# CaptainEven/DenseBox

Measured on AMD Instinct MI355X. Metric: training patches/sec (240x240), higher is better.
Workload: dtype f16; 1 GPU; full training step (fwd + fused dense loss w/ hard-negative mining + bwd + grad all-reduce + SGD) of DenseBoxLMLOC on 240x240 patches; net=DenseBoxLMLOC, batch_per_gpu=64, global_batch=64, patch=240x240, parallelism=dp1, half_neg=11, grad_finite=True

## Files before the change

densebox_amd/_lib.py:

```python
import ctypes as C
import os

_HERE = os.path.dirname(os.path.abspath(__file__))
LIB_PATH = os.environ.get('DBX_LIB') or os.path.join(_HERE, 'csrc', 'libdensebox_hip.so')

F16, BF16, F32 = 0, 1, 2
DTYPE_ID = {'f16': F16, 'bf16': BF16, 'f32': F32}
ESIZE = {F16: 2, BF16: 2, F32: 4}

EPI_BIAS, EPI_RELU, EPI_GATE, EPI_DROPMASK, EPI_ACCUM, EPI_F32_NCHW, EPI_DROPHASH = 1, 2, 4, 8, 16, 32, 64
CONV_WFRAG = 128
K_IGEMM, K_DMA, K_BAND, K_C64, K_C8, K_WS, K_P8 = 1, 2, 3, 4, 5, 6, 7


class View(C.Structure):
    _fields_ = [('ptr', C.c_void_p), ('n', C.c_int32), ('h', C.c_int32), ('w', C.c_int32),
                ('pad', C.c_int32), ('ld', C.c_int32), ('c_off', C.c_int32), ('c', C.c_int32)]


class ConvDesc(C.Structure):
    _fields_ = [('dtype', C.c_int32), ('kh', C.c_int32), ('kw', C.c_int32), ('cpad', C.c_int32),
                ('cin_pad', C.c_int32), ('cout_pad', C.c_int32), ('epilogue', C.c_int32), ('drop_seed', C.c_uint32)]


class ConvPlan(C.Structure):
    _fields_ = [('kernel', C.c_int32), ('tile_m', C.c_int32), ('tile_n', C.c_int32), ('w_frag', C.c_int32),
                ('name', C.c_char * 64)]


class LossDesc(C.Structure):
    _fields_ = [('kind', C.c_int32), ('n', C.c_int32), ('half_neg', C.c_int32),
                ('lambda_loc', C.c_float), ('lambda_det', C.c_float), ('lambda_lm', C.c_float),
                ('use_labels', C.c_int32)]


class LossIO(C.Structure):
    _fields_ = [(k, C.c_void_p) for k in (
        'bbox', 'vertices', 'labels', 'rand_neg', 'lm_rand_neg',
        'score', 'loc', 'lm', 'rf', 'lmloc',
        'd_score', 'd_loc', 'd_lm', 'd_rf', 'd_lmloc',
        'loss', 'mask_cls', 'mask_lm', 'neg_idx', 'lm_neg_idx', 'pos_count')]


class WarpJob(C.Structure):
    _fields_ = [('src', C.c_void_p), ('sh', C.c_int32), ('sw', C.c_int32), ('m9', C.c_double * 9), ('dh', C.c_int32),
                ('dw', C.c_int32), ('x0', C.c_int32), ('y0', C.c_int32), ('oh', C.c_int32), ('ow', C.c_int32),
                ('dst_off', C.c_int64)]


class CropFrame(C.Structure):
    _fields_ = [('src', C.c_void_p), ('sh', C.c_int32), ('sw', C.c_int32)]


class EvalRecord(C.Structure):
    _fields_ = [('score', C.c_double), ('lm_err', C.c_double), ('status', C.c_int32), ('frame', C.c_int32)]


class Track(C.Structure):
    _fields_ = [('box', C.c_double * 4), ('vel', C.c_double * 4), ('score', C.c_double), ('best_score', C.c_double), ('id', C.c_int32),
                ('hits', C.c_int32), ('age', C.c_int32), ('first_frame', C.c_int32), ('last_frame', C.c_int32), ('best_frame', C.c_int32)]


class TrackRecord(C.Structure):
    _fields_ = [('stream', C.c_int32), ('reserved', C.c_int32), ('t', Track)]


class Shot(C.Structure):
    _fields_ = [('key', C.c_double), ('score', C.c_double), ('sharpness', C.c_int64), ('id', C.c_int32), ('frame', C.c_int32),
                ('shots', C.c_int32), ('reserved', C.c_int32)]


class ShotRecord(C.Structure):
    _fields_ = [('stream', C.c_int32), ('slot', C.c_int32), ('shot', Shot)]


class ResizeJob(C.Structure):
    _fields_ = [('src', C.c_void_p), ('sh', C.c_int32), ('sw', C.c_int32), ('cx0', C.c_int32), ('cy0', C.c_int32),
                ('cw', C.c_int32), ('ch', C.c_int32), ('pad_l', C.c_int32), ('pad_t', C.c_int32), ('pad_r', C.c_int32),
                ('pad_b', C.c_int32), ('pad_value', C.c_int32), ('dh', C.c_int32), ('dw', C.c_int32), ('dst_off', C.c_int64)]


class MergeXform(C.Structure):
    _fields_ = [('scale', C.c_double), ('off_x', C.c_double), ('off_y', C.c_double)]


_VP, _I32, _I64, _F, _D = C.c_void_p, C.c_int32, C.c_int64, C.c_float, C.c_double
_PV, _PC = C.POINTER(View), C.POINTER(ConvDesc)

SIGNATURES = {
    'dbx_last_error': (C.c_char_p, []),
    'dbx_version': (C.c_int, []),
    'dbx_device_arch': (C.c_int, [C.c_int]),
    'dbx_conv_packed_elems': (_I64, [_PC]),
    'dbx_conv_forward': (C.c_int, [_PC, _PV, _VP, _VP, _PV, _PV, _VP, _I32, _VP]),
    'dbx_conv_plan': (C.c_int, [_PC, _PV, _PV, C.POINTER(ConvPlan)]),
    'dbx_conv_forward_split': (C.c_int, [_PC, _PV, _VP, _VP, _PV, _PV, _PV, _PV, _I32, _I32, _VP]),
    'dbx_heads_forward_fusable': (C.c_int, [_PC, _PV, _PV, C.POINTER(C.c_int32), _I32]),
    'dbx_heads_forward_fused_scratch_bytes': (_I64, [_I32, _I64]),
    'dbx_heads_forward_fused': (C.c_int, [_PC, _PV, _VP, _VP, _PV, _VP, _VP, C.POINTER(C.c_int32), _I32, _VP, _VP, _VP]),
    'dbx_heads_forward_fused_heads': (C.c_int, [_PC, _PV, _VP, _VP, _PV, _VP, _VP, C.POINTER(C.c_int32), _I32, C.POINTER(C.c_void_p), _VP, _VP]),
    'dbx_dp_unique_id': (C.c_int, [_VP]),
    'dbx_dp_init': (C.c_int, [_VP, _I32, _I32, C.POINTER(C.c_void_p)]),
    'dbx_dp_allreduce_sum_f32': (C.c_int, [_VP, _VP, _I64, _VP]),
    'dbx_dp_destroy': (C.c_int, [_VP]),
    'dbx_conv_dgrad_wgrad1_scratch_bytes': (_I64, []),
    'dbx_conv_dgrad_wgrad1_fusable': (C.c_int, [_PC, _PV, _PV, _PV]),
    'dbx_conv_dgrad_wgrad1': (C.c_int, [_PC, _PV, _VP, _PV, _PV, _I32, _VP, _VP, _VP, _I32, _VP]),
    'dbx_conv_pool_fusable': (C.c_int, [_PC, _PV, _PV]),
    'dbx_conv_forward_pool': (C.c_int, [_PC, _PV, _VP, _VP, _PV, _PV, _I32, _VP]),
    'dbx_conv_forward_pool_idx': (C.c_int, [_PC, _PV, _VP, _VP, _PV, _PV, _I32, _VP, _VP]),
    'dbx_pack_weight': (C.c_int, [_I32, _I32, _VP, _I32, _I32, _I32, _I32, _VP, _I32, _I32, _I32, _I32, _VP]),
    'dbx_fold_heads': (C.c_int, [_VP, _VP, _VP, _VP, _I32, _VP, _VP, _VP]),
    'dbx_fold_refine': (C.c_int, [_VP, _VP, _VP, _VP, _VP, _VP, _I32, _I32, _VP, _VP, _VP, _VP]),
    'dbx_refine_eval': (C.c_int, [_VP, _VP, _I32, _I32, _I32, _VP, _VP, _VP, _VP]),
    'dbx_refine_backward_scratch_bytes': (C.c_int64, [_I32, _I32, _I32]),
    'dbx_refine_backward': (C.c_int, [_VP, _VP, _VP, _I32, _I32, _I32, _VP, _VP, _VP, _VP, _VP, _VP, _I32, _VP, _VP, _VP, _VP, _VP, _VP, _VP, _VP, _VP, _VP, _VP, _VP, _VP, _VP]),
    'dbx_upsample_bilinear_nchw_f32': (C.c_int, [_VP, _I32, _I32, _I32, _VP, _I32, _I32, _VP]),
    'dbx_pack_multi': (C.c_int, [_I32, _VP, _I32, _I64, _VP]),
    'dbx_sgd_pack_step': (C.c_int, [_I32, _VP, _I32, _I64, _VP, _F, _F, _F, _I32, _VP]),
    'dbx_head2_dgrad': (C.c_int, [_I32, _PV, C.POINTER(C.c_void_p), C.POINTER(C.c_int32), _I32, _PV, _VP, _I32, _I32, C.c_uint32, _VP]),
    'dbx_head2_wgrad_scratch_bytes': (_I64, [_I32, _I32]),
    'dbx_head2_wgrad': (C.c_int, [_I32, _PV, _PV, C.POINTER(C.c_int32), _I32, C.POINTER(C.c_void_p), C.POINTER(C.c_void_p), _VP, _VP]),
    'dbx_head2_backward': (C.c_int, [_I32, _PV, _PV, C.POINTER(C.c_void_p), C.POINTER(C.c_int32), _I32, _PV, _VP, _I32, _I32, C.c_uint32,
                                     C.POINTER(C.c_void_p), C.POINTER(C.c_void_p), _VP, _VP]),
    'dbx_head2_backward_up': (C.c_int, [_I32, _PV, _PV, C.POINTER(C.c_void_p), C.POINTER(C.c_int32), _I32, _PV, _VP, _I32, _I32, C.c_uint32,
                                        C.POINTER(C.c_void_p), C.POINTER(C.c_void_p), _VP, _PV, _VP]),
    'dbx_perspective_matrix': (C.c_int, [_VP, _VP, _VP]),
    'dbx_warp_perspective_u8': (C.c_int, [_VP, _I32, _I32, _I32, _VP, _VP, _I32, _I32, _VP]),
    'dbx_warp_batch_workspace_bytes': (_I64, [_I32]),
    'dbx_warp_perspective_batch_u8': (C.c_int, [C.POINTER(WarpJob), _I32, _I32, _VP, _VP, _VP]),
    'dbx_plate_crops_batch': (C.c_int, [_VP, _I32, _I32, _VP, _I64, _I64, _VP, _I32, _I32, _I32, _VP, _VP, _VP, _VP]),
    'dbx_match_gt_batch': (C.c_int, [_VP, _I32, _I64, _VP, _VP, _I32, _I32, _VP, _I32, _VP, _VP, _I32, _D, _VP, _VP, _VP, _VP, _VP, _VP]),
    'dbx_eval_append': (C.c_int, [_VP, _I32, _I64, _VP, _VP, _I32, _I32, _VP, _VP, _VP, _VP, _I64, _VP, _VP]),
    'dbx_track_update_batch': (C.c_int, [_VP, _I32, _I64, _VP, _VP, _I32, _I32, _VP, _VP, _I32, _I32, _I32, _D, _I32, _D, _D, _D, _VP, _VP, _VP,
                                         _VP, _VP, _VP]),
    'dbx_track_append': (C.c_int, [_VP, _VP, _I32, _I32, _I32, _VP, _I64, _VP, _VP]),
    'dbx_crop_sharpness': (C.c_int, [_VP, _I64, _I32, _I32, _I32, _VP, _VP]),
    'dbx_track_gallery_update': (C.c_int, [_VP, _VP, _VP, _VP, _VP, _VP, _VP, _VP, _VP, _VP, _VP, _VP, _VP, _I32, _I32, _I32, _I32, _I32, _I32,
                                           _I32, _I32, _I64, _I32, _D, _I32, _VP]),
    'dbx_resize_batch_workspace_bytes': (_I64, [_I32]),
    'dbx_resize_cubic_batch_u8': (C.c_int, [C.POINTER(ResizeJob), _I32, _I32, _VP, _VP, _VP]),
    'dbx_conv_wgrad_scratch_bytes': (_I64, [_I32, _PV, _PV, _I32, _I32]),
    'dbx_conv_wgrad': (C.c_int, [_I32, _PV, _PV, _I32, _I32, _I32, _I32, _I32, _VP, _VP, _VP, _I32, _VP]),
    'dbx_conv_wgrad_slice': (C.c_int, [_I32, _PV, _PV, _I32, _I32, _I32, _I32, _I32, _VP, _I32, _I32, _VP, _VP, _I32, _VP]),
    'dbx_conv_wgrad_pool_dz_ok': (C.c_int, [_I32, _PV, _PV, _I32, _I32]),
    'dbx_conv_wgrad_pool_dz': (C.c_int, [_I32, _PV, _VP, _I32, _PV, _PV, _I32, _I32, _I32, _I32, _I32, _VP, _VP, _VP, _I32, _I32, _VP]),
    'dbx_head2_backward_up_fused': (C.c_int, [_I32, _PV, _PV]),
    'dbx_heads1_wgrad_gen_ok': (C.c_int, [_I32, _PV, _I32]),
    'dbx_heads1_dgrad_gen': (C.c_int, [_I32, _PV, C.POINTER(C.c_void_p), C.POINTER(C.c_int32), _I32, _I32, C.c_uint32, _VP, _PV, _PV, _VP]),
    'dbx_heads1_wgrad_gen': (C.c_int, [_I32, _PV, _PV, C.POINTER(C.c_void_p), C.POINTER(C.c_int32), _I32, _I32, C.c_uint32, _I32, _VP, _I32, _I32,
                             _VP, _VP, _VP]),
    'dbx_conv_wgrad_plan': (C.c_int, [_I32, _PV, _PV, _I32, _I32, C.c_char_p, _I32, C.POINTER(C.c_int32)]),
    'dbx_nchw_to_framed': (C.c_int, [_I32, _VP, _I32, _PV, _VP]),
    'dbx_u8hwc_to_framed': (C.c_int, [_I32, _VP, _PV, C.POINTER(C.c_float), C.POINTER(C.c_float), _VP]),
    'dbx_nchw_to_framed_ch': (C.c_int, [_I32, _VP, _I32, _PV, _I32, _VP]),
    'dbx_nchw_to_framed_slots': (C.c_int, [_I32, _VP, _VP, _I32, _I32, _PV, _VP]),
    'dbx_framed_to_nchw_f32': (C.c_int, [_I32, _PV, _VP, _VP]),
    'dbx_framed_add_ch': (C.c_int, [_I32, _PV, _I32, _I32, _PV, _I32, _VP]),
    'dbx_maxpool2x2': (C.c_int, [_I32, _PV, _PV, _VP]),
    'dbx_maxpool2x2_bwd': (C.c_int, [_I32, _PV, _PV, _PV, _I32, _I32, _VP]),
    'dbx_maxpool_idx_bytes': (C.c_int64, [_I32, _I32, _I32, _I32]),
    'dbx_maxpool2x2_idx': (C.c_int, [_I32, _PV, _PV, _VP, _VP]),
    'dbx_maxpool2x2_bwd_idx': (C.c_int, [_I32, _VP, _PV, _PV, _I32, _I32, _VP]),
    'dbx_upsample_bilinear': (C.c_int, [_I32, _PV, _PV, _VP]),
    'dbx_upsample_bilinear_bwd': (C.c_int, [_I32, _PV, _PV, _PV, _VP]),
    'dbx_loss_scratch_bytes': (C.c_int64, [_I32]),
    'dbx_loss_forward_backward': (C.c_int, [C.POINTER(LossDesc), C.POINTER(LossIO), _VP, _VP]),
    'dbx_count_positives': (C.c_int, [_VP, _VP, _I32, _VP, _VP]),
    'dbx_init_score_map': (C.c_int, [_VP, _VP, _I32, _VP, _VP]),
    'dbx_init_offset_map': (C.c_int, [_VP, _VP, _I32, _I32, _VP, _VP]),
    'dbx_init_lm_heatmap': (C.c_int, [_VP, _VP, _I32, _I32, _VP, _VP]),
    'dbx_mask_by_sel': (C.c_int, [_VP, _I32, _VP, _I64, _VP, _I32, _VP]),
    'dbx_mask_gray_zone_cls': (C.c_int, [_VP, _VP, _VP, _I32, _VP]),
    'dbx_mask_gray_zone_lm': (C.c_int, [_VP, _I32, _VP, _I64, _VP]),
    'dbx_sgd_step': (C.c_int, [_VP, _VP, _I32, _I64, _F, _F, _F, _I32, _VP]),
    'dbx_grad_guard': (C.c_int, [_VP, _I64, _VP, _I32, _VP]),
    'dbx_sgd_step_guarded': (C.c_int, [_VP, _VP, _I32, _I64, _F, _F, _F, _I32, _VP, _I32, _VP]),
    'dbx_sgd_pack_step_guarded': (C.c_int, [_I32, _VP, _I32, _I64, _VP, _F, _F, _F, _I32, _VP, _I32, _VP]),
    'dbx_detect_scratch_bytes': (_I64, [_I32, _I32, _I32]),
    'dbx_detect': (C.c_int, [_VP, _VP, _VP, _VP, _I32, _I32, _I32, _D, _VP, _I32, _VP, _VP, _VP, _VP]),
    'dbx_detect_batch_scratch_bytes': (_I64, [_I32, _I32, _I32, _I32]),
    'dbx_detect_batch': (C.c_int, [_VP, _VP, _VP, _VP, _I32, _I32, _I32, _I32, _D, _VP, _I32, _VP, _VP, _VP, _VP]),
    'dbx_nms': (C.c_int, [_VP, _I32, _I32, _D, _VP, _VP, _VP]),
    'dbx_detect_thresh_batch_scratch_bytes': (_I64, [_I32, _I32, _I32, _I32]),
    'dbx_detect_thresh_batch': (C.c_int, [_VP, _VP, _VP, _VP, _I32, _I32, _I32, _F, _I32, _D, _VP, _I32, _VP, _VP, _VP, _VP, _VP]),
    'dbx_thresh_rows_batch_scratch_bytes': (_I64, [_I32, _I32, _I32, _I32]),
    'dbx_thresh_rows_batch': (C.c_int, [_VP, _VP, _VP, _VP, _I32, _I32, _I32, _F, _I32, _VP, _I32, _VP, _VP, _VP, _VP]),
    'dbx_nms_large_scratch_bytes': (_I64, [_I32]),
    'dbx_nms_large': (C.c_int, [_VP, _I32, _I32, _D, _VP, _VP, _VP]),
    'dbx_merge_nms_batch_workspace_bytes': (_I64, [_I32, _I32, _I32]),
    'dbx_merge_nms_batch': (C.c_int, [C.POINTER(C.c_void_p), C.POINTER(MergeXform), _I32, _I32, _I32, _I32, _D, _VP, _VP, _VP, _VP]),
    'dbx_merge_nms_thresh_batch_workspace_bytes': (_I64, [_I32, _I32, _I32]),
    'dbx_merge_nms_thresh_batch': (C.c_int, [C.POINTER(C.c_void_p), C.POINTER(C.c_void_p), C.POINTER(MergeXform), _I32, _I32, _I32, _I32, _D,
                                             _VP, _VP, _VP, _VP, _VP]),
}

ABI_VERSION = 13
_lib = None
MISSING = []


def lib():
    global _lib
    if _lib is None:
        if not os.path.exists(LIB_PATH):
            raise RuntimeError('libdensebox_hip.so is not built (%s). Run `python -c "import __graft_entry__ as g; '
                               'g.build()"`; densebox_amd has no fallback path.' % LIB_PATH)
        L = C.CDLL(LIB_PATH)
        for name, (res, args) in SIGNATURES.items():
            try:
                fn = getattr(L, name)
            except AttributeError:
                MISSING.append(name)
                continue
            fn.restype = res
            fn.argtypes = args
        if 'dbx_version' not in MISSING and L.dbx_version() != ABI_VERSION:
            raise RuntimeError('libdensebox_hip.so at %s has ABI version %d, this binding needs %d (struct layouts / scratch '
                               'contracts differ): rebuild it' % (LIB_PATH, L.dbx_version(), ABI_VERSION))
        _lib = L
    return _lib


def check(rc):
    if rc != 0:
        raise RuntimeError('libdensebox_hip: %s (status %d)' % (lib().dbx_last_error().decode(), rc))


def ptr(t):
    return C.c_void_p(t.data_ptr()) if t is not None else None


def stream_ptr():
    import torch
    return C.c_void_p(torch.cuda.current_stream().cuda_stream)
```

densebox_amd/csrc/aux_ops.hip:

```cpp
#include "common.hpp"
#include <mutex>

static thread_local char g_err[512] = "";
void dbx_set_error(const char* fmt, ...) {
    va_list ap;
    va_start(ap, fmt);
    vsnprintf(g_err, sizeof(g_err), fmt, ap);
    va_end(ap);
}
extern "C" const char* dbx_last_error(void) { return g_err; }
extern "C" int dbx_version(void) { return DBX_ABI_VERSION; }
extern "C" int dbx_device_arch(int device) {
    hipDeviceProp_t p;
    if (hipGetDeviceProperties(&p, device) != hipSuccess) { dbx_set_error("hipGetDeviceProperties failed"); return DBX_ERR_HIP; }
    int arch = 0;
    const char* s = p.gcnArchName;
    if (s[0] == 'g' && s[1] == 'f' && s[2] == 'x') arch = (int)strtol(s + 3, nullptr, 16) == 0x950 ? 950 : (int)strtol(s + 3, nullptr, 10);
    return arch;
}

template <typename T> struct Vec { static constexpr int N = 16 / sizeof(T); };

template <typename T> __device__ __forceinline__ void load_vec(const T* p, float (&v)[16 / sizeof(T)]) {
    const u32x4 raw = *(const u32x4*)p;
    const T* e = (const T*)&raw;
#pragma unroll
    for (int i = 0; i < 16 / (int)sizeof(T); ++i) v[i] = to_f32(e[i]);
}
template <typename T> __device__ __forceinline__ void store_vec(T* p, const float (&v)[16 / sizeof(T)]) {
    u32x4 raw;
    T* e = (T*)&raw;
#pragma unroll
    for (int i = 0; i < 16 / (int)sizeof(T); ++i) e[i] = from_f32<T>(v[i]);
    *(u32x4*)p = raw;
}

static inline int grid_for(int64_t work, int block = 256) {
    int64_t b = (work + block - 1) / block;
    return (int)(b < 1 ? 1 : (b > 8192 ? 8192 : b));
}

#define VIEW_VEC_CHECK(T, v, name)                                                                             \
    DBX_REQUIRE(((size_t)(v)->ptr % 16) == 0 && ((v)->ld * sizeof(T)) % 16 == 0 && ((v)->c_off * sizeof(T)) % 16 == 0 && \
                    ((v)->c * sizeof(T)) % 16 == 0, name ": view must be 16-byte aligned/strided")

template <typename T>
__global__ void nchw_to_framed_kernel(const float* __restrict__ x, int csrc, FrameGeo y) {
    constexpr int V = Vec<T>::N;
    const int cg = y.c / V;
    const int64_t total = (int64_t)y.n * y.h * y.w * cg;
    for (int64_t i = blockIdx.x * (int64_t)blockDim.x + threadIdx.x; i < total; i += (int64_t)gridDim.x * blockDim.x) {
        const int px = (int)(i % y.w);
        const int g = (int)((i / y.w) % cg);
        const int py = (int)((i / ((int64_t)y.w * cg)) % y.h);
        const int n = (int)(i / ((int64_t)y.w * cg * y.h));
        float v[V];
#pragma unroll
        for (int j = 0; j < V; ++j) {
            const int c = g * V + j;
            v[j] = c < csrc ? x[(((int64_t)n * csrc + c) * y.h + py) * y.w + px] : 0.f;
        }
        store_vec<T>((T*)y.base + geo_pix(y, n, py, px) + g * V, v);
    }
}
template <typename T> static int nchw_to_framed_t(const float* x, int csrc, const dbx_view* y, hipStream_t s) {
    VIEW_VEC_CHECK(T, y, "nchw_to_framed");
    FrameGeo g = make_geo<T>(y);
    const int64_t total = (int64_t)y->n * y->h * y->w * (y->c / Vec<T>::N);
    hipLaunchKernelGGL(nchw_to_framed_kernel<T>, dim3(grid_for(total)), dim3(256), 0, s, x, csrc, g);
    DBX_LAUNCH_CHECK();
    return DBX_OK;
}
extern "C" int dbx_nchw_to_framed(int32_t dtype, const float* x_nchw, int32_t c_src, const dbx_view* y, void* stream) {
    DBX_DISPATCH_DTYPE(dtype, nchw_to_framed_t, x_nchw, c_src, y, (hipStream_t)stream);
}

struct SlotSrc { const float* x[4]; int k[4]; };
template <typename T>
__global__ void nchw_to_framed_slots_kernel(SlotSrc src, int nslots, int slot, FrameGeo y) {
    constexpr int V = Vec<T>::N;
    const int gps = slot / V, cg = nslots * gps;
    const int64_t total = (int64_t)y.n * y.h * y.w * cg;
    for (int64_t i = blockIdx.x * (int64_t)blockDim.x + threadIdx.x; i < total; i += (int64_t)gridDim.x * blockDim.x) {
        const int px = (int)(i % y.w);
        const int g = (int)((i / y.w) % cg);
        const int py = (int)((i / ((int64_t)y.w * cg)) % y.h);
        const int n = (int)(i / ((int64_t)y.w * cg * y.h));
        const int si = g / gps, c0 = (g % gps) * V;
        const float* x = si == 0 ? src.x[0] : si == 1 ? src.x[1] : si == 2 ? src.x[2] : src.x[3];
        const int k = si == 0 ? src.k[0] : si == 1 ? src.k[1] : si == 2 ? src.k[2] : src.k[3];
        float v[V];
#pragma unroll
        for (int j = 0; j < V; ++j) {
            const int c = c0 + j;
            v[j] = (x && c < k) ? x[(((int64_t)n * k + c) * y.h + py) * y.w + px] : 0.f;
        }
        store_vec<T>((T*)y.base + geo_pix(y, n, py, px) + si * slot + c0, v);
    }
}
template <typename T> static int nchw_to_framed_slots_t(const float* const* xs, const int32_t* ks, int nslots, int slot, const dbx_view* y, hipStream_t s) {
    VIEW_VEC_CHECK(T, y, "nchw_to_framed_slots");
    DBX_REQUIRE(nslots >= 1 && nslots <= 4 && slot % Vec<T>::N == 0 && y->c == nslots * slot, "nchw_to_framed_slots: 1..4 slots of a multiple of the vector width, view of nslots * slot channels");
    SlotSrc src;
    for (int i = 0; i < 4; ++i) {
        src.x[i] = i < nslots ? xs[i] : nullptr; src.k[i] = i < nslots ? ks[i] : 0;
        if (i < nslots) DBX_REQUIRE(ks[i] >= 0 && ks[i] <= slot, "nchw_to_framed_slots: k must fit its slot");
    }
    FrameGeo g = make_geo<T>(y);
    const int64_t total = (int64_t)y->n * y->h * y->w * (y->c / Vec<T>::N);
    hipLaunchKernelGGL(nchw_to_framed_slots_kernel<T>, dim3(grid_for(total)), dim3(256), 0, s, src, nslots, slot, g);
    DBX_LAUNCH_CHECK();
    return DBX_OK;
}
extern "C" int dbx_nchw_to_framed_slots(int32_t dtype, const float* const* x_nchw, const int32_t* k, int32_t nslots, int32_t slot, const dbx_view* y,
                                        void* stream) {
    if (!x_nchw || !k || !y) { dbx_set_error("nchw_to_framed_slots: null argument"); return DBX_ERR_ARG; }
    DBX_DISPATCH_DTYPE(dtype, nchw_to_framed_slots_t, x_nchw, k, nslots, slot, y, (hipStream_t)stream);
}

template <typename T>
__global__ void framed_to_nchw_kernel(FrameGeo x, float* __restrict__ y) {
    const int64_t total = (int64_t)x.n * x.c * x.h * x.w;
    for (int64_t i = blockIdx.x * (int64_t)blockDim.x + threadIdx.x; i < total; i += (int64_t)gridDim.x * blockDim.x) {
        const int px = (int)(i % x.w);
        const int py = (int)((i / x.w) % x.h);
        const int c = (int)((i / ((int64_t)x.w * x.h)) % x.c);
        const int n = (int)(i / ((int64_t)x.w * x.h * x.c));
        y[i] = to_f32(((const T*)x.base)[geo_pix(x, n, py, px) + c]);
    }
}
template <typename T> static int framed_to_nchw_t(const dbx_view* x, float* y, hipStream_t s) {
    FrameGeo g = make_geo<T>(x);
    const int64_t total = (int64_t)x->n * x->c * x->h * x->w;
    hipLaunchKernelGGL(framed_to_nchw_kernel<T>, dim3(grid_for(total)), dim3(256), 0, s, g, y);
    DBX_LAUNCH_CHECK();
    return DBX_OK;
}
extern "C" int dbx_framed_to_nchw_f32(int32_t dtype, const dbx_view* x, float* y_nchw, void* stream) {
    DBX_DISPATCH_DTYPE(dtype, framed_to_nchw_t, x, y_nchw, (hipStream_t)stream);
}

template <typename T> struct IdxWord { typedef unsigned int type; };
template <> struct IdxWord<float> { typedef unsigned short type; };
template <typename T>
__global__ void maxpool_kernel(FrameGeo x, FrameGeo y, unsigned char* __restrict__ idx) {
    constexpr int V = Vec<T>::N;
    const int cg = y.c / V;
    const int64_t total = (int64_t)y.n * y.h * y.w * cg;
    for (int64_t i = blockIdx.x * (int64_t)blockDim.x + threadIdx.x; i < total; i += (int64_t)gridDim.x * blockDim.x) {
        const int g = (int)(i % cg);
        const int px = (int)((i / cg) % y.w);
        const int py = (int)((i / ((int64_t)cg * y.w)) % y.h);
        const int n = (int)(i / ((int64_t)cg * y.w * y.h));
// ... 1049 lines not shown
#pragma unroll
        for (int d = 0; d < D; ++d) {
            const int r = r0 + d;
            float gj[KJ], h[V];
            {
                const T* ge = (const T*)&graw[d];
                const T* he = (const T*)&hraw[d];
#pragma unroll
                for (int j = 0; j < KJ; ++j) gj[j] = to_f32(ge[j]);
#pragma unroll
                for (int i = 0; i < V; ++i) h[i] = to_f32(he[i]);
            }
            fetch(d);
            if (r < R) {
                int y0, y1; float ly0, ly1;
                bilin_coef(oy, sy, dg.h, y0, y1, ly0, ly1);
                while (y0 > cur) {
                    finalize(cur, va);
#pragma unroll
                    for (int i = 0; i < V / 2; ++i) { va[i] = vb[i]; vb[i] = (f32x2){0.f, 0.f}; }
                    ++cur;
                }
                const float wa = (y0 == cur ? ly0 : 0.f) + (y1 == cur ? ly1 : 0.f);
                const float wb = (y0 == cur + 1 ? ly0 : 0.f) + (y1 == cur + 1 ? ly1 : 0.f);
                {
                    f32x2 o2[V / 2];
#pragma unroll
                    for (int i = 0; i < V / 2; ++i) o2[i] = (f32x2){0.f, 0.f};
#pragma unroll
                    for (int j = 0; j < KJ; ++j) {
                        bs[j] += gj[j];
                        const f32x2 g2 = {gj[j], gj[j]};
#pragma unroll
                        for (int i = 0; i < V / 2; ++i) acc[j][i] = g2 * (f32x2){h[2 * i], h[2 * i + 1]} + acc[j][i];
#pragma unroll
                        for (int i = 0; i < V / 2; ++i) o2[i] = g2 * w2[j][i] + o2[i];
                    }
                    float o[V];
#pragma unroll
                    for (int i = 0; i < V / 2; ++i) { o[2 * i] = o2[i].x; o[2 * i + 1] = o2[i].y; }
                    const long long pc0 = ((long long)n * H + oy) * W;
                    if (mask) {
                        unsigned char mb[V];
                        *(u32x2*)mb = *(const u32x2*)(mask + (size_t)pc0 * mask_ld + lo_mask);
#pragma unroll
                        for (int i = 0; i < V; ++i) o[i] = mb[i] ? o[i] : 0.f;
                    } else if (use_hash) {
                        const unsigned kb8 = dbx_drop_hash32(drop_seed, (unsigned)pc0 + (unsigned)px, (unsigned)(hd * 512 + c0) >> 5) >> ((unsigned)c0 & 31u);
#pragma unroll
                        for (int i = 0; i < V; ++i)
                            o[i] = __builtin_bit_cast(float, __builtin_bit_cast(int, o[i]) & ((int)(kb8 << (31 - i)) >> 31));
                    }
                    u32x4 raw;
                    T* oe = (T*)&raw;
#pragma unroll
                    for (int i = 0; i < V; ++i) oe[i] = from_f32<T>(o[i]);
                    if (owner && !nostore) *(u32x4*)((T*)dhid.base + row_of(dhid, n, oy) + lo_dhid) = raw;
                    const f32x2 wa2 = {wa, wa}, wb2 = {wb, wb};
#pragma unroll
                    for (int i = 0; i < V / 2; ++i) {
                        const f32x2 dv = {to_f32(oe[2 * i]), to_f32(oe[2 * i + 1])};
                        va[i] = wa2 * dv + va[i]; vb[i] = wb2 * dv + vb[i];
                    }
                }
                if (++oy == H) {
                    finalize(cur, va);
                    if (cur + 1 < dg.h) finalize(cur + 1, vb);
                    if (pend) flush();
#pragma unroll
                    for (int i = 0; i < V / 2; ++i) va[i] = vb[i] = (f32x2){0.f, 0.f};
                    cur = 0; oy = 0; n += G;
                }
            }
        }
    }
    if (!owner) {
#pragma unroll
        for (int j = 0; j < KJ; ++j) {
            bs[j] = 0.f;
#pragma unroll
            for (int i = 0; i < V / 2; ++i) acc[j][i] = (f32x2){0.f, 0.f};
        }
    }
    const int lane = threadIdx.x & 63, wv = threadIdx.x >> 6;
#pragma unroll
    for (int j = 0; j < KJ; ++j) {
#pragma unroll
        for (int i = 0; i < V; ++i) {
            float a = acc[j][i >> 1][i & 1];
            a += __shfl_xor(a, 8); a += __shfl_xor(a, 16); a += __shfl_xor(a, 32);
            acc[j][i >> 1][i & 1] = a;
        }
        float bsum = bs[j];
        bsum += __shfl_xor(bsum, 8); bsum += __shfl_xor(bsum, 16); bsum += __shfl_xor(bsum, 32);
        bs[j] = bsum;
    }
    __syncthreads();
    float* red = s_v;
    if (lane < LPP) {
#pragma unroll
        for (int j = 0; j < KJ; ++j) {
            *(f32x4*)&red[(wv * 8 + j) * CS + lane * V] = (f32x4){acc[j][0][0], acc[j][0][1], acc[j][1][0], acc[j][1][1]};
            *(f32x4*)&red[(wv * 8 + j) * CS + lane * V + 4] = (f32x4){acc[j][2][0], acc[j][2][1], acc[j][3][0], acc[j][3][1]};
        }
#pragma unroll
        for (int j = KJ; j < 8; ++j) {
            *(f32x4*)&red[(wv * 8 + j) * CS + lane * V] = (f32x4){0.f, 0.f, 0.f, 0.f};
            *(f32x4*)&red[(wv * 8 + j) * CS + lane * V + 4] = (f32x4){0.f, 0.f, 0.f, 0.f};
        }
        if (lane == 0) {
#pragma unroll
            for (int j = 0; j < 8; ++j) red[4 * 8 * CS + wv * 8 + j] = j < KJ ? bs[j < KJ ? j : 0] : 0.f;
        }
    }
    __syncthreads();
    {
        const size_t blk = (size_t)grp * plan.halves + half;
        const int c = threadIdx.x % CS;
#pragma unroll
        for (int jj = 0; jj < 2; ++jj) {
            const int j = threadIdx.x / CS + 4 * jj;
            float o = 0.f;
#pragma unroll
            for (int q = 0; q < 4; ++q) o += red[(q * 8 + j) * CS + c];
            partial[(blk * nhl * 8 + (hd - hd0) * 8 + j) * 512 + cbase + c] = o;
        }
        if (cbase == 0 && threadIdx.x < 8) {
            float bsum = 0.f;
#pragma unroll
            for (int q = 0; q < 4; ++q) bsum += red[4 * 8 * CS + q * 8 + threadIdx.x];
            bpartial[blk * 32 + (hd - hd0) * 8 + threadIdx.x] = bsum;
        }
    }
}
static bool h2u_plan(int W, int ws, float sx, H2UPlan& p) {
    if (W > 64 || ws > 32 || W < 1 || ws < 1) return false;
    int x0[64];
    for (int ox = 0; ox < W; ++ox) { int v = (int)(sx * (float)ox); x0[ox] = v > ws - 1 ? ws - 1 : v; }
    if (W <= 32 && ws <= 16) { p.halves = 1; p.h[0] = p.h[1] = H2UHalf{0, W, 0, W, 0, ws}; return true; }
    const int S = ws / 2;
    if (S < 1 || S > 16 || ws - S > 16) return false;
    int hiL = -1, loR = W;
    for (int ox = 0; ox < W; ++ox) { if (x0[ox] <= S - 1) hiL = ox; if (x0[ox] >= S - 1 && ox < loR) loR = ox; }
    if (hiL + 1 > 32 || W - loR > 32 || loR > hiL + 1) return false;
    const int P = (loR + hiL + 1) / 2;
    p.halves = 2;
    p.h[0] = H2UHalf{0, hiL + 1, 0, P, 0, S};
    p.h[1] = H2UHalf{loR, W - loR, P, W, S, ws - S};
    return true;
}
template <typename T>
static int head2_backward_up_t(const dbx_view* dout, const dbx_view* hid, const float* const* w2, const int32_t* k, int nh, const dbx_view* dhid,
                               const uint8_t* mask, int mask_ld, int use_hash, unsigned drop_seed, float* const* dw, float* const* db,
                               void* scratch, const dbx_view* dg, hipStream_t s) {
    VIEW_VEC_CHECK(T, dg, "head2_backward_up d_g44");
    DBX_REQUIRE(dg->n == hid->n && dg->c == hid->c, "head2_backward_up: d_g44 has the hidden map's batch and channels");
    const float sy = ac_scale(dg->h, hid->h), sx = ac_scale(dg->w, hid->w);
    H2UPlan plan;
    bool fused = sizeof(T) == 2 && sy > 0.f && sy < 1.f && sx > 0.45f && sx < 1.f && hid->c % 64 == 0 && hid->h >= 2 && h2u_plan(hid->w, dg->w, sx, plan);
    if (const char* e = getenv("DBX_HEAD2_UP")) fused = fused && atoi(e) != 0;
    const bool nostore = dhid->ptr == nullptr;
    DBX_REQUIRE(!nostore || (fused && !mask), "head2_backward_up without d_hid: needs the one-pass kernel (dbx_head2_backward_up_fused) and hash / no dropout");
    if (!fused) {
        const int rc = head2_wgrad_t<T>(dout, hid, k, nh, dw, db, scratch, s, w2, dhid, mask, mask_ld, use_hash, drop_seed);
        return rc != DBX_OK ? rc : upsample_bwd_t<T>(dhid, dg, nullptr, s);
    }
    if constexpr (sizeof(T) == 2) {
        VIEW_VEC_CHECK(T, hid, "head2_backward_up hid");
        if (!nostore) VIEW_VEC_CHECK(T, dhid, "head2_backward_up d_hid");
        DBX_REQUIRE(nh >= 1 && nh <= 4 && hid->c == 512 * nh && dout->c % nh == 0 && dout->c / nh >= 8, "head2_backward_up: nh in 1..4, hid of 512*nh channels, d_out of nh slots >= 8 channels");
        DBX_REQUIRE(dout->n == hid->n && dout->h == hid->h && dout->w == hid->w && dhid->n == hid->n && dhid->h == hid->h && dhid->w == hid->w && dhid->c == hid->c,
                    "head2_backward_up: shape mismatch");
        DBX_REQUIRE(((size_t)dout->ptr % 16) == 0 && (dout->ld * sizeof(T)) % 16 == 0 && (dout->c_off * sizeof(T)) % 16 == 0 &&
                        ((dout->c / nh) * sizeof(T)) % 16 == 0, "head2_backward_up: d_out alignment");
        Head2Out o;
        Head2Args ha;
        ha.nh = nh; ha.slot = dout->c / nh;
        for (int i = 0; i < 4; ++i) {
            o.dw[i] = i < nh ? dw[i] : nullptr; o.db[i] = (i < nh && db) ? db[i] : nullptr; o.k[i] = i < nh ? k[i] : 0;
            ha.w2[i] = i < nh ? w2[i] : nullptr; ha.k[i] = i < nh ? k[i] : 0;
            if (i < nh) DBX_REQUIRE(k[i] >= 1 && k[i] <= 8 && dw[i] && w2[i] && ((size_t)w2[i] % 16) == 0, "head2_backward_up: k in 1..8, 16-byte aligned weights");
        }
        constexpr size_t smem = (size_t)2 * H2U_NB * 32 * 64 * 4;
        static_assert(smem >= (4 * 8 * 64 + 32) * 4 && 2 * smem + 4096 <= 160 * 1024, "LDS budget of two workgroups per CU");
        static DbxDevOnce attr_once; int attr_dev = 0;
        if (attr_once.pending(&attr_dev)) {
            DBX_HIP(hipFuncSetAttribute((const void*)head2_backward_up_kernel<T, 1>, hipFuncAttributeMaxDynamicSharedMemorySize, (int)smem));
            DBX_HIP(hipFuncSetAttribute((const void*)head2_backward_up_kernel<T, 2>, hipFuncAttributeMaxDynamicSharedMemorySize, (int)smem));
            DBX_HIP(hipFuncSetAttribute((const void*)head2_backward_up_kernel<T, 4>, hipFuncAttributeMaxDynamicSharedMemorySize, (int)smem));
            DBX_HIP(hipFuncSetAttribute((const void*)head2_backward_up_kernel<T, 8>, hipFuncAttributeMaxDynamicSharedMemorySize, (int)smem));
            attr_once.mark(attr_dev);
        }
        static int split = -1;
        if (split < 0) { const char* e = getenv("DBX_HEAD2_UP_SPLIT"); split = e ? atoi(e) : 1; }
        auto kup = [&](int kk) { return !split ? 8 : kk <= 1 ? 1 : kk <= 2 ? 2 : kk <= 4 ? 4 : 8; };
        float* const pbase = (float*)scratch;
        long long pused = 0;
        int blocks_max = 0;
        for (int h0 = 0; h0 < nh;) {
            int h1 = h0 + 1;
            while (h1 < nh && kup(k[h1]) == kup(k[h0])) ++h1;
            const int nhl = h1 - h0, nsl = nhl * 8, kj = kup(k[h0]);
            int groups = H2U_WGS / (nsl * plan.halves);
            groups = groups < 1 ? 1 : groups > hid->n ? hid->n : groups;
            const int blocks = groups * plan.halves;
            float* partial = pbase + pused;
            float* bpartial = partial + (size_t)blocks * nhl * 8 * 512;
            for (int i = h0; i < h1; ++i) { o.poff[i] = pused; o.boff[i] = pused + (long long)blocks * nhl * 8 * 512; o.nblk[i] = blocks; o.nhl[i] = nhl; o.hl[i] = i - h0; }
            pused += (long long)blocks * (nhl * 8 * 512 + 32);
            blocks_max = blocks > blocks_max ? blocks : blocks_max;
#define H2U_LAUNCH(KJ)                                                                                                              \
            hipLaunchKernelGGL((head2_backward_up_kernel<T, KJ>), dim3(blocks * nsl), dim3(256), smem, s, make_geo<T>(dout), make_geo<T>(hid),    \
                               make_geo<T>(nostore ? hid : dhid), make_geo<T>(dg), h0, nhl, dout->c / nh, ha, partial, bpartial, mask, mask_ld,    \
                               use_hash, drop_seed, sy, sx, plan, nostore ? 1 : 0)
            if (kj == 1) H2U_LAUNCH(1); else if (kj == 2) H2U_LAUNCH(2); else if (kj == 4) H2U_LAUNCH(4); else H2U_LAUNCH(8);
#undef H2U_LAUNCH
            DBX_LAUNCH_CHECK();
            h0 = h1;
        }
        for (int i = nh; i < 4; ++i) { o.poff[i] = 0; o.boff[i] = 0; o.nblk[i] = 0; o.nhl[i] = 1; o.hl[i] = 0; }
        float* partial = pbase; float* bpartial = pbase;
        const int blocks = blocks_max;
        const int total = nh * 8 * 512 + nh * 8;
        hipLaunchKernelGGL(head2_wgrad_reduce_kernel, dim3((total + 63) / 64), dim3(1024), 0, s, partial, bpartial, blocks, nh, o);
        DBX_LAUNCH_CHECK();
    }
    return DBX_OK;
}
template <typename T> static int head2_up_fused_t(const dbx_view* hid, const dbx_view* dg) {
    const float sy = ac_scale(dg->h, hid->h), sx = ac_scale(dg->w, hid->w);
    H2UPlan plan;
    bool fused = sizeof(T) == 2 && sy > 0.f && sy < 1.f && sx > 0.45f && sx < 1.f && hid->c % 64 == 0 && hid->h >= 2 && h2u_plan(hid->w, dg->w, sx, plan);
    if (const char* e = getenv("DBX_HEAD2_UP")) fused = fused && atoi(e) != 0;
    return fused ? 1 : 0;
}
extern "C" int dbx_head2_backward_up_fused(int32_t dtype, const dbx_view* hid, const dbx_view* d_g44) {
    if (!hid || !d_g44) return 0;
    switch (dtype) { case DBX_F16: return head2_up_fused_t<_Float16>(hid, d_g44); case DBX_BF16: return head2_up_fused_t<__bf16>(hid, d_g44); default: return 0; }
}
extern "C" int dbx_head2_backward_up(int32_t dtype, const dbx_view* d_out, const dbx_view* hid, const float* const* w2, const int32_t* k,
                                     int32_t nh, const dbx_view* d_hid, const uint8_t* dropmask, int32_t dropmask_ld, int32_t use_hash,
                                     uint32_t drop_seed, float* const* dw, float* const* db, void* scratch, const dbx_view* d_g44, void* stream) {
    if (!d_out || !hid || !w2 || !k || !d_hid || !dw || !scratch || !d_g44) { dbx_set_error("head2_backward_up: null argument"); return DBX_ERR_ARG; }
    DBX_DISPATCH_DTYPE(dtype, head2_backward_up_t, d_out, hid, w2, k, nh, d_hid, dropmask, dropmask_ld, use_hash, (unsigned)drop_seed, dw, db,
                       scratch, d_g44, (hipStream_t)stream);
}

struct PackJob { const float* src; void* dst; int co, ci, taps, mode; long long ktot; int cin_pad, row_off, k_off, rows_lim; };
template <typename T>
__global__ void pack_multi_kernel(const PackJob* __restrict__ jobs) {
    const PackJob j = jobs[blockIdx.y];
    const int total = j.co * j.ci * j.taps, taps = j.taps, ci = j.ci;
    T* wp = (T*)j.dst;
    const bool fwd = j.mode == 0 || j.mode == 4;
    const int rl = j.mode >= 4 ? (int)j.ktot : j.rows_lim;
    if (sizeof(T) == 2 && j.mode != 2 && (fwd ? ci : j.co) % 8 == 0 && (j.k_off & 7) == 0 && (j.cin_pad & 7) == 0 && taps <= 25) {
        __shared__ float tile[8][32 * 25];
        const int ot = (j.co + 7) / 8, ctn = (ci + 31) / 32, ntiles = ot * ctn, row_f = 32 * taps;
        for (int tl = blockIdx.x; tl < ntiles; tl += gridDim.x) {
            const int o0 = (tl / ctn) * 8, c0 = (tl % ctn) * 32;
            const int cw = min(32, ci - c0), ow = min(8, j.co - o0);
            __syncthreads();
            for (int e = threadIdx.x; e < 8 * row_f; e += blockDim.x) {
                const int r = e / row_f, f = e - r * row_f;
                tile[r][f] = (r < ow && f < cw * taps) ? j.src[((o0 + r) * ci + c0) * taps + f] : 0.f;
            }
            __syncthreads();
            const int nch = fwd ? 8 * taps * 4 : 32 * taps;
            for (int q = threadIdx.x; q < nch; q += blockDim.x) {
                int row, col, tap;
                float v[8];
                if (fwd) {
                    const int k8 = q & 3, t = (q >> 2) % taps, r = (q >> 2) / taps;
                    if (r >= ow || 8 * k8 >= cw) continue;
                    row = j.row_off + o0 + r; col = j.k_off + c0 + 8 * k8; tap = t;
#pragma unroll
                    for (int e = 0; e < 8; ++e) v[e] = tile[r][(8 * k8 + e) * taps + t];
                } else {
                    const int c = q % 32, t = q / 32;
                    if (c >= cw) continue;
                    row = j.row_off + c0 + c; col = j.k_off + o0; tap = taps - 1 - t;
#pragma unroll
                    for (int e = 0; e < 8; ++e) v[e] = tile[e][c * taps + t];
                }
                if (row < 0 || col < 0 || col + 8 > j.cin_pad || (rl > 0 && row >= rl)) continue;
                u32x4 raw;
                T* e8 = (T*)&raw;
#pragma unroll
                for (int e = 0; e < 8; ++e) e8[e] = from_f32<T>(v[e]);
                const long long di = j.mode >= 4 ? (long long)dbx_frag_index(row, tap, col, j.cin_pad, (int)j.ktot, taps)
                                                 : (long long)row * j.ktot + (long long)tap * j.cin_pad + col;
                *(u32x4*)(wp + di) = raw;
            }
        }
        return;
    }
    for (int i = blockIdx.x * blockDim.x + threadIdx.x; i < total; i += gridDim.x * blockDim.x) {
        const float v = j.src[i];
        if (j.mode == 2) { ((float*)j.dst)[j.row_off + i] = v; continue; }
        const int q = i / taps, t = i - q * taps;
        const int o = q / ci, c = q - o * ci;
        {
            const int row = j.row_off + (fwd ? o : c), col = j.k_off + (fwd ? c : o);
            if (row < 0 || col < 0 || col >= j.cin_pad || (rl > 0 && row >= rl)) continue;
        }
        if (j.mode == 0) wp[(long long)(j.row_off + o) * j.ktot + (long long)t * j.cin_pad + j.k_off + c] = from_f32<T>(v);
        else if (j.mode == 1) wp[(long long)(j.row_off + c) * j.ktot + (long long)(taps - 1 - t) * j.cin_pad + j.k_off + o] = from_f32<T>(v);
        else if (j.mode == 4) wp[dbx_frag_index(j.row_off + o, t, j.k_off + c, j.cin_pad, (int)j.ktot, taps)] = from_f32<T>(v);
        else wp[dbx_frag_index(j.row_off + c, taps - 1 - t, j.k_off + o, j.cin_pad, (int)j.ktot, taps)] = from_f32<T>(v);
    }
}
template <typename T> static int pack_multi_t(const void* jobs, int count, long long max_elems, hipStream_t s) {
    int bx = (int)((max_elems + 255) / 256);
    bx = bx < 1 ? 1 : (bx > 256 ? 256 : bx);
    hipLaunchKernelGGL(pack_multi_kernel<T>, dim3(bx, count), dim3(256), 0, s, (const PackJob*)jobs);
    DBX_LAUNCH_CHECK();
    return DBX_OK;
}
extern "C" int dbx_pack_multi(int32_t dtype, const void* jobs, int32_t count, int64_t max_elems, void* stream) {
    DBX_REQUIRE(jobs && count > 0, "pack_multi: empty job table");
    DBX_DISPATCH_DTYPE(dtype, pack_multi_t, jobs, count, (long long)max_elems, (hipStream_t)stream);
}

struct PackDst { void* dst; long long ktot; int mode, cin_pad, row_off, k_off, rows_lim, pad_; };
struct SgdPackJob { float* p; int pidx, co, ci, taps, ndst, tiled; PackDst d[4]; };
template <typename T>
__device__ __forceinline__ void pack_scatter_elem(const PackDst& d, int o, int c, int t, int i, int taps, float v) {
    if (d.mode == 2) { ((float*)d.dst)[d.row_off + i] = v; return; }
    const bool fwd = d.mode == 0 || d.mode == 4;
    const int rl = d.mode >= 4 ? (int)d.ktot : d.rows_lim;
    const int row = d.row_off + (fwd ? o : c), col = d.k_off + (fwd ? c : o), tap = fwd ? t : taps - 1 - t;
    if (row < 0 || col < 0 || col >= d.cin_pad || (rl > 0 && row >= rl)) return;
    T* wp = (T*)d.dst;
    if (d.mode >= 4) wp[dbx_frag_index(row, tap, col, d.cin_pad, (int)d.ktot, taps)] = from_f32<T>(v);
    else wp[(long long)row * d.ktot + (long long)tap * d.cin_pad + col] = from_f32<T>(v);
}
template <typename T>
__global__ __launch_bounds__(256) void sgd_pack_kernel(const SgdPackJob* __restrict__ jobs, float* const* __restrict__ ptrs, float lr, float mu,
                                                       float wd, int first, int* __restrict__ guard, int step_id) {
    if (guard && guard[0] == step_id) {
        if (blockIdx.x == 0 && blockIdx.y == 0 && threadIdx.x == 0) atomicAdd(guard + 1, 1);
        return;
    }
    const SgdPackJob& j = jobs[blockIdx.y];
    float* p = j.p;
    const int pidx = j.pidx, taps = j.taps, ci = j.ci, co = j.co, ndst = j.ndst;
    const float* g = pidx >= 0 ? ptrs[3 * pidx + 1] : nullptr;
    float* b = pidx >= 0 ? ptrs[3 * pidx + 2] : nullptr;
    const int total = co * ci * taps;
    if (j.tiled && sizeof(T) == 2) {
        __shared__ float tile[8][32 * 25];
        const int CW = taps == 1 ? 256 : 32, nk8 = CW / 8;
        const int ot = (co + 7) / 8, ctn = (ci + CW - 1) / CW, ntiles = ot * ctn, row_f = CW * taps;
        constexpr int U = 3;
        for (int tl = blockIdx.x; tl < ntiles; tl += gridDim.x) {
            const int o0 = (tl / ctn) * 8, c0 = (tl % ctn) * CW;
            const int cw = min(CW, ci - c0), ow = min(8, co - o0);
            __syncthreads();
            int r = 0, f = threadIdx.x;
            while (f >= row_f) { f -= row_f; ++r; }
            for (int e = threadIdx.x; e < 8 * row_f; e += U * 256) {
                float pv[U], gv[U], bv[U];
                int ii[U], rr[U], ff[U];
#pragma unroll
                for (int u = 0; u < U; ++u) {
                    rr[u] = r; ff[u] = f;
                    const bool ok = r < ow && f < cw * taps;
                    ii[u] = ok ? ((o0 + r) * ci + c0) * taps + f : -1;
                    pv[u] = ok ? p[ii[u]] : 0.f;
                    if (g && ok) { gv[u] = g[ii[u]]; bv[u] = first ? 0.f : b[ii[u]]; }
                    f += 256;
                    while (f >= row_f) { f -= row_f; ++r; }
                }
#pragma unroll
                for (int u = 0; u < U; ++u) {
                    if (g && ii[u] >= 0) {
                        float bb = bv[u];
                        pv[u] = dbx_sgd_update(pv[u], gv[u], &bb, lr, mu, wd, first);
                        b[ii[u]] = bb; p[ii[u]] = pv[u];
                    }
                    if (rr[u] < 8) tile[rr[u]][ff[u]] = pv[u];
                }
            }
            __syncthreads();
            for (int di = 0; di < ndst; ++di) {
                const PackDst& d = j.d[di];
                T* wp = (T*)d.dst;
                const bool fwd = d.mode == 0 || d.mode == 4;
                const int rl = d.mode >= 4 ? (int)d.ktot : d.rows_lim;
                const int nch = fwd ? 8 * taps * nk8 : CW * taps;
                for (int q = threadIdx.x; q < nch; q += blockDim.x) {
                    int row, col, tap;
                    float v[8];
                    if (fwd) {
                        const int k8 = q % nk8, q2 = q / nk8, t = q2 % taps, r2 = q2 / taps;
                        if (r2 >= ow || 8 * k8 >= cw) continue;
                        row = d.row_off + o0 + r2; col = d.k_off + c0 + 8 * k8; tap = t;
#pragma unroll
// ... 240 lines not shown
```

densebox_amd/csrc/loss.hip:

```cpp
#include "common.hpp"

#define HWD 60
#define NPIX 3600
#define LOSS_THREADS 1024

__device__ __forceinline__ int norm_idx(int v) {
    if (v < 0) { v += HWD; if (v < 0) v = 0; }
    else if (v > HWD) v = HWD;
    return v;
}
struct Span { int a, b; };
__device__ __forceinline__ Span py_slice(int start, int stop) {
    Span s; s.a = norm_idx(start); s.b = norm_idx(stop); if (s.b < s.a) s.b = s.a; return s;
}
__device__ __forceinline__ void rect_axis(float c0, float c2, double border, int& org, int& end) {
    const double centre = (double)(c0 + c2) * 0.5;
    const float w = c2 - c0;
    const float rw = 0.3f * w;
    const float half = rw * 0.5f;
    if (border == 0.0) {
        org = (int)(centre - (double)half + 0.5);
        end = (int)((double)org + (double)rw + 0.5);
    } else {
        org = (int)(centre - (double)half - border + 0.5);
// ... 160 lines not shown
        }
        __syncthreads();
        for (int i = tid; i < NPIX; i += LOSS_THREADS) {
            const int y = i / HWD, x = i - y * HWD;
            if (in_span(box.coy, y) && in_span(box.cox, x)) mask[i] = 1;
        }
        __syncthreads();
    }

    int lmx[4] = {0, 0, 0, 0}, lmy[4] = {0, 0, 0, 0};
    if (kind != 0) {
        const float* vt = io.vertices + 8 * n;
        const int clamp = a.d.use_labels;
        for (int j = 0; j < 4; ++j) { lmx[j] = lm_coord(vt[2 * j], clamp); lmy[j] = lm_coord(vt[2 * j + 1], clamp); }
        for (int j = 0; j < 4; ++j) {
            const float* lm = io.lm + ((size_t)n * 4 + j) * NPIX;
            const int pidx = lmy[j] * HWD + lmx[j];
            for (int i = tid; i < NPIX; i += LOSS_THREADS) {
                const float gt = (valid && i == pidx) ? 1.f : 0.f;
                const float d = lm[i] - gt;
                negl[i] = d * d * (1.f - gt);
                lmask[j][i] = gt != 0.f;
            }
            __syncthreads();
            const int hard = block_argmax(negl, red_v, red_i);
            if (tid == 0) {
                const long long r = io.lm_rand_neg[((size_t)j * N + n)];
                lmask[j][hard] = 1;
                if (r >= 0 && r < NPIX) lmask[j][(int)r] = 1;
                if (io.lm_neg_idx) { io.lm_neg_idx[((size_t)j * N + n) * 2] = hard; io.lm_neg_idx[((size_t)j * N + n) * 2 + 1] = r; }
            }
            __syncthreads();
            if (valid) {
                const Span sy = py_slice(lmy[j] - 2, lmy[j] + 3), sx = py_slice(lmx[j] - 2, lmx[j] + 3);
                for (int i = tid; i < 25; i += LOSS_THREADS) {
                    const int y = sy.a + i / 5, x = sx.a + i % 5;
                    if (y < sy.b && x < sx.b) lmask[j][y * HWD + x] = 0;
                }
                __syncthreads();
                if (tid == 0) lmask[j][pidx] = 1;
                __syncthreads();
            }
        }
    }

    unsigned char* mb = a.maskbuf + (size_t)n * 5 * NPIX;
    for (int i = tid; i < NPIX; i += LOSS_THREADS) {
        mb[i] = mask[i];
        if (kind != 0) {
#pragma unroll
            for (int j = 0; j < 4; ++j) mb[(1 + j) * NPIX + i] = lmask[j][i];
        }
    }
}

__global__ __launch_bounds__(LOSS_APPLY_THREADS) void loss_apply_kernel(const LossArgs a) {
    __shared__ double red_d[LOSS_APPLY_THREADS / 64];
    const int n = blockIdx.y, tid = threadIdx.x, i = blockIdx.x * LOSS_APPLY_THREADS + tid;
    const int kind = a.d.kind;
    const dbx_loss_io& io = a.io;
    const float* bb = io.bbox + 4 * n;
    const int valid = (a.d.use_labels && io.labels) ? (io.labels[n] != 0.f) : 1;
    const Box box = make_box(bb, valid);
    const float* score = io.score + (size_t)n * NPIX;
    const unsigned char* mb = a.maskbuf + (size_t)n * 5 * NPIX;
    int lmx[4] = {0, 0, 0, 0}, lmy[4] = {0, 0, 0, 0};
    if (kind != 0) {
        const float* vt = io.vertices + 8 * n;
        const int clamp = a.d.use_labels;
        for (int j = 0; j < 4; ++j) { lmx[j] = lm_coord(vt[2 * j], clamp); lmy[j] = lm_coord(vt[2 * j + 1], clamp); }
    }
    const float l_loc = a.d.lambda_loc, l_det = (kind == 0) ? 1.f : a.d.lambda_det, l_lm = a.d.lambda_lm;
    double s_cls = 0, s_loc = 0, s_lm = 0, s_lmloc = 0, s_rf = 0;
    if (i < NPIX) {
        const int y = i / HWD, x = i - y * HWD;
        const float m = (float)mb[i];
        const float gt = (valid && in_span(box.py, y) && in_span(box.px, x)) ? 1.f : 0.f;
        if (io.mask_cls) io.mask_cls[(size_t)n * NPIX + i] = m;
        {
            const float d = score[i] - gt;
            s_cls += (double)(m * (d * d));
            if (io.d_score) io.d_score[(size_t)n * NPIX + i] = 2.f * l_det * m * d;
        }
        const float mg = m * gt;
        const float fx = (float)x, fy = (float)y;
#pragma unroll
        for (int c = 0; c < 4; ++c) {
            const float tgt = valid ? ((c & 1) ? fy : fx) - bb[c] : 0.f;
            const size_t o = ((size_t)n * 4 + c) * NPIX + i;
            const float d = io.loc[o] - tgt;
            s_loc += (double)(mg * (d * d));
            if (io.d_loc) io.d_loc[o] = 2.f * l_det * l_loc * mg * d;
        }
        if (kind != 0) {
            const float d = io.rf[(size_t)n * NPIX + i] - gt;
            s_rf += (double)(m * (d * d));
            if (io.d_rf) io.d_rf[(size_t)n * NPIX + i] = 2.f * m * d;
#pragma unroll
            for (int j = 0; j < 4; ++j) {
                const float ml = (float)mb[(1 + j) * NPIX + i];
                const float hg = (valid && i == lmy[j] * HWD + lmx[j]) ? 1.f : 0.f;
                const size_t o = ((size_t)n * 4 + j) * NPIX + i;
                const float dl = io.lm[o] - hg;
                s_lm += (double)(ml * (dl * dl));
                if (io.d_lm) io.d_lm[o] = 2.f * l_lm * ml * dl;
                if (io.mask_lm) io.mask_lm[o] = ml;
            }
            if (kind == 2) {
                const float* vt = io.vertices + 8 * n;
#pragma unroll
                for (int c = 0; c < 8; ++c) {
                    const float tgt = valid ? ((c & 1) ? fy : fx) - vt[c] : 0.f;
                    const size_t o = ((size_t)n * 8 + c) * NPIX + i;
                    const float d = io.lmloc[o] - tgt;
                    s_lmloc += (double)(mg * (d * d));
                    if (io.d_lmloc) io.d_lmloc[o] = 2.f * mg * d;
                }
            }
        }
    }
    double mine = (double)l_det * (s_cls + (double)l_loc * s_loc) + (double)l_lm * s_lm + s_lmloc + s_rf;
#pragma unroll
    for (int off = 32; off > 0; off >>= 1) mine += __shfl_down(mine, off);
    if ((tid & 63) == 0) red_d[tid >> 6] = mine;
    __syncthreads();
    if (tid == 0) {
        double t = 0.0;
        for (int w = 0; w < LOSS_APPLY_THREADS / 64; ++w) t += red_d[w];
        a.partial[(size_t)n * LOSS_APPLY_BLOCKS + blockIdx.x] = t;
    }
}

__global__ __launch_bounds__(256) void loss_finish_kernel(const double* partial, int n, int per, float* loss) {
    __shared__ double psum[256];
    double run = 0.0;
    for (int base = 0; base < n; base += 256) {
        const int p = base + threadIdx.x;
        double t = 0.0;
        if (p < n) for (int i = 0; i < per; ++i) t += partial[(size_t)p * per + i];
        psum[threadIdx.x] = t;
        __syncthreads();
        if (threadIdx.x == 0) {
            const int cnt = n - base < 256 ? n - base : 256;
            for (int i = 0; i < cnt; ++i) run += psum[i];
        }
        __syncthreads();
    }
    if (threadIdx.x == 0) loss[0] = (float)run;
}

extern "C" int64_t dbx_loss_scratch_bytes(int32_t n) {
    return (int64_t)n * LOSS_APPLY_BLOCKS * 8 + (int64_t)n * 5 * NPIX + 64;
}
extern "C" int dbx_loss_forward_backward(const dbx_loss_desc* d, const dbx_loss_io* io, void* scratch, void* stream) {
    DBX_REQUIRE(d && io && scratch, "loss: null argument");
    DBX_REQUIRE(d->kind >= 0 && d->kind <= 2 && d->n > 0, "loss: bad kind/n");
    DBX_REQUIRE(d->half_neg >= 0 && d->half_neg <= NPIX, "loss: half_neg out of range");
    DBX_REQUIRE(io->bbox && io->score && io->loc && io->loss && (d->half_neg == 0 || io->rand_neg), "loss: missing tensors");
    if (d->kind != 0) DBX_REQUIRE(io->vertices && io->lm && io->rf && io->lm_rand_neg, "loss: landmark tensors missing");
    if (d->kind == 2) DBX_REQUIRE(io->lmloc != nullptr, "loss: lm_loc missing");
    LossArgs a; a.d = *d; a.io = *io; a.partial = (double*)scratch;
    a.maskbuf = (unsigned char*)scratch + (size_t)d->n * LOSS_APPLY_BLOCKS * sizeof(double);
    hipLaunchKernelGGL(loss_kernel, dim3(d->n), dim3(LOSS_THREADS), 0, (hipStream_t)stream, a);
    DBX_LAUNCH_CHECK();
    hipLaunchKernelGGL(loss_apply_kernel, dim3(LOSS_APPLY_BLOCKS, d->n), dim3(LOSS_APPLY_THREADS), 0, (hipStream_t)stream, a);
    DBX_LAUNCH_CHECK();
    hipLaunchKernelGGL(loss_finish_kernel, dim3(1), dim3(256), 0, (hipStream_t)stream, (const double*)scratch, d->n, LOSS_APPLY_BLOCKS, io->loss);
    DBX_LAUNCH_CHECK();
    return DBX_OK;
}

__global__ void count_positives_kernel(const float* bbox, const float* labels, int n, int* out) {
    const int i = blockIdx.x * blockDim.x + threadIdx.x;
    if (i >= n) return;
    const int valid = labels ? labels[i] != 0.f : 1;
    const Box b = make_box(bbox + 4 * i, valid);
    out[i] = valid ? (b.py.b - b.py.a) * (b.px.b - b.px.a) : 0;
}
extern "C" int dbx_count_positives(const float* bbox, const float* labels, int32_t n, int32_t* out, void* stream) {
    hipLaunchKernelGGL(count_positives_kernel, dim3((n + 63) / 64), dim3(64), 0, (hipStream_t)stream, bbox, labels, n, out);
    DBX_LAUNCH_CHECK();
    return DBX_OK;
}

__global__ void init_score_map_kernel(const float* bbox, const float* labels, float* out) {
    const int n = blockIdx.x;
    const int valid = labels ? labels[n] != 0.f : 1;
    const Box b = make_box(bbox + 4 * n, valid);
    for (int i = threadIdx.x; i < NPIX; i += blockDim.x) {
        const int y = i / HWD, x = i - y * HWD;
        out[(size_t)n * NPIX + i] = (valid && in_span(b.py, y) && in_span(b.px, x)) ? 1.f : 0.f;
    }
}
extern "C" int dbx_init_score_map(const float* bbox, const float* labels, int32_t n, float* out, void* stream) {
    hipLaunchKernelGGL(init_score_map_kernel, dim3(n), dim3(256), 0, (hipStream_t)stream, bbox, labels, out);
    DBX_LAUNCH_CHECK();
    return DBX_OK;
}

__global__ void init_offset_map_kernel(const float* coords, const float* labels, int c, float* out) {
    const int n = blockIdx.x;
    const int valid = labels ? labels[n] != 0.f : 1;
    for (int i = threadIdx.x; i < c * NPIX; i += blockDim.x) {
        const int ch = i / NPIX, p = i - ch * NPIX;
        const int y = p / HWD, x = p - y * HWD;
        out[(size_t)n * c * NPIX + i] = valid ? ((ch & 1) ? (float)y : (float)x) - coords[n * c + ch] : 0.f;
    }
}
extern "C" int dbx_init_offset_map(const float* coords, const float* labels, int32_t n, int32_t c, float* out, void* stream) {
    hipLaunchKernelGGL(init_offset_map_kernel, dim3(n), dim3(256), 0, (hipStream_t)stream, coords, labels, c, out);
    DBX_LAUNCH_CHECK();
    return DBX_OK;
}

__global__ void init_lm_heatmap_kernel(const float* vert, const float* labels, int clamp, float* out, int* err) {
    const int n = blockIdx.x;
    const int valid = labels ? labels[n] != 0.f : 1;
    for (int i = threadIdx.x; i < 4 * NPIX; i += blockDim.x) out[(size_t)n * 4 * NPIX + i] = 0.f;
    __syncthreads();
    if (threadIdx.x < 4 && valid) {
        const int j = threadIdx.x;
        int x = lm_coord(vert[8 * n + 2 * j], clamp), y = lm_coord(vert[8 * n + 2 * j + 1], clamp);
        if (x >= HWD || y >= HWD) { if (err) atomicAdd(err, 1); x = min(x, HWD - 1); y = min(y, HWD - 1); }
        out[((size_t)n * 4 + j) * NPIX + y * HWD + x] = 1.f;
    }
}
extern "C" int dbx_init_lm_heatmap(const float* vertices, const float* labels, int32_t n, int32_t clamp, float* out, void* stream) {
    hipLaunchKernelGGL(init_lm_heatmap_kernel, dim3(n), dim3(256), 0, (hipStream_t)stream, vertices, labels, clamp, out, (int*)nullptr);
    DBX_LAUNCH_CHECK();
    return DBX_OK;
}

__global__ void mask_by_sel_kernel(float* mask, int n, const long long* pos, long long npos, const long long* neg, int nneg) {
    const long long total = npos + (long long)n * nneg;
    for (long long i = blockIdx.x * (long long)blockDim.x + threadIdx.x; i < total; i += (long long)gridDim.x * blockDim.x) {
        if (i < npos) {
            const long long* p = pos + 4 * i;
            mask[((size_t)p[0] + p[1]) * NPIX + p[2] * HWD + p[3]] = 1.f;
        } else {
            const long long j = i - npos;
            const long long id = neg[j];
            if (id >= 0 && id < NPIX) mask[(size_t)(j / nneg) * NPIX + id] = 1.f;
        }
    }
}
extern "C" int dbx_mask_by_sel(float* mask, int32_t n, const int64_t* pos_idx, int64_t n_pos, const int64_t* neg_idx,
                               int32_t n_neg, void* stream) {
    const long long total = n_pos + (long long)n * n_neg;
    if (total == 0) return DBX_OK;
    hipLaunchKernelGGL(mask_by_sel_kernel, dim3((unsigned)((total + 255) / 256)), dim3(256), 0, (hipStream_t)stream, mask, n,
                       (const long long*)pos_idx, (long long)n_pos, (const long long*)neg_idx, n_neg);
    DBX_LAUNCH_CHECK();
    return DBX_OK;
}

__global__ void mask_gray_zone_cls_kernel(float* mask, const float* bbox, const float* labels) {
    const int n = blockIdx.x;
    const int valid = labels ? labels[n] != 0.f : 1;
    if (!valid) return;
    const Box b = make_box(bbox + 4 * n, valid);
    for (int i = threadIdx.x; i < NPIX; i += blockDim.x) {
        const int y = i / HWD, x = i - y * HWD;
        float v = mask[(size_t)n * NPIX + i];
        if (in_span(b.gzy, y) && in_span(b.gzx, x)) v = 0.f;
        if (in_span(b.coy, y) && in_span(b.cox, x)) v = 1.f;
        mask[(size_t)n * NPIX + i] = v;
    }
}
extern "C" int dbx_mask_gray_zone_cls(float* mask, const float* bbox, const float* labels, int32_t n, void* stream) {
    hipLaunchKernelGGL(mask_gray_zone_cls_kernel, dim3(n), dim3(256), 0, (hipStream_t)stream, mask, bbox, labels);
    DBX_LAUNCH_CHECK();
    return DBX_OK;
}

__global__ void mask_gray_zone_lm_kernel(float* mask, const long long* pos, long long npos) {
    const long long p = blockIdx.x;
    if (p >= npos) return;
    const long long n = pos[4 * p];
    const int y = (int)pos[4 * p + 2], x = (int)pos[4 * p + 3];
    const Span sy = py_slice(y - 2, y + 3), sx = py_slice(x - 2, x + 3);
    const int i = threadIdx.x;
    if (i < 25) {
        const int yy = sy.a + i / 5, xx = sx.a + i % 5;
        if (yy < sy.b && xx < sx.b) mask[(size_t)n * NPIX + yy * HWD + xx] = 0.f;
    }
    __syncthreads();
    if (i == 0) mask[(size_t)n * NPIX + y * HWD + x] = 1.f;
}
extern "C" int dbx_mask_gray_zone_lm(float* mask, int32_t n, const int64_t* pos_idx, int64_t n_pos, void* stream) {
    if (n_pos == 0) return DBX_OK;
    hipLaunchKernelGGL(mask_gray_zone_lm_kernel, dim3((unsigned)n_pos), dim3(64), 0, (hipStream_t)stream, mask,
                       (const long long*)pos_idx, (long long)n_pos);
    DBX_LAUNCH_CHECK();
    return DBX_OK;
}
```

densebox_amd/dist.py:

```python
import contextlib
import json
import os
import sys
import threading
from datetime import timedelta

import torch
import torch.distributed as dist


def rendezvous_timeout_s():
    return float(os.environ.get('DBX_DIST_RENDEZVOUS_S', '120'))


def dist_timeout_s():
    return float(os.environ.get('DBX_DIST_TIMEOUT_S', '1800'))


def rccl_info():
    env = {k: v for k, v in os.environ.items()
           if k.startswith(('NCCL_', 'RCCL_', 'HSA_ENABLE_IPC', 'MASTER_', 'DBX_DIST_')) or k in ('RANK', 'WORLD_SIZE', 'LOCAL_RANK')}
    info = {'backend': dist.get_backend() if dist.is_initialized() else None,
            'world': dist.get_world_size() if dist.is_initialized() else int(os.environ.get('WORLD_SIZE', '1')),
            'timeout_s': dist_timeout_s(), 'rendezvous_timeout_s': rendezvous_timeout_s(), 'env': env,
# ... 77 lines not shown
        self.bucket_elems = max(1, bucket_bytes // 4)
        self._ready_hi = 0
        self._sent_hi = 0
        self._works = []

    def grad_view(self, name):
        return self.views[name]

    def region(self, names):
        lo, hi = self.range[names[0]][0], self.range[names[-1]][1]
        assert hi - lo == sum(self.range[n][1] - self.range[n][0] for n in names), 'parameters are not adjacent'
        return self.flat[lo:hi]

    in_step = False

    def begin(self):
        self._ready_hi = self._sent_hi = 0
        self._works = []

    def ready(self, names):
        if not self.in_step:
            return
        for n in names:
            self._ready_hi = max(self._ready_hi, self.range[n][1])
        if self.collective and self._ready_hi - self._sent_hi >= self.bucket_elems:
            self._send(self._ready_hi)

    def _send(self, hi):
        if hi > self._sent_hi:
            self._works.append(dist.all_reduce(self.flat[self._sent_hi:hi], op=dist.ReduceOp.SUM, group=self.group,
                                               async_op=True))
            self._sent_hi = hi

    def finish(self):
        if self.collective:
            self._send(self.flat.numel())
            for w in self._works:
                w.wait()
        self._works = []


class DataParallel:

    def __init__(self, net, optimizer, bucket_bytes=8 << 20, always_reduce=False):
        self.net, self.opt = net, optimizer
        self.world = dist.get_world_size() if dist.is_initialized() else 1
        self.rank = dist.get_rank() if dist.is_initialized() else 0
        self.ctl = None
        self.collective = self.world > 1 or (always_reduce and dist.is_initialized())
        if self.collective:
            for p in net.parameters():
                dist.broadcast(p.data, src=0)
            self.ctl = dist.new_group(backend='gloo', timeout=timedelta(seconds=dist_timeout_s())) if dist.get_backend() != 'gloo' \
                else dist.group.WORLD
        eng = net.engine()
        self.reducer = GradReducer(net.named_parameters(), eng.grad_order(), bucket_bytes, always_reduce=always_reduce)
        eng.grad_sink = self.reducer
        self._pf = None
        self.guard_f16 = os.environ.get('DBX_F16_GUARD', '1') != '0' and hasattr(optimizer, 'enable_guard')

    def close(self):
        eng = self.net.engine()
        if eng.grad_sink is self.reducer:
            eng.grad_sink = None

    def prefetch_positive_num(self, bbox, labels=None):
        from . import labels as LB
        if self._pf is not None:
            self._consume_prefetch()
        p = int(LB.positive_count(bbox, labels).sum())
        if self.collective:
            t = torch.tensor([p], dtype=torch.int64)
            self._pf = (p, t, dist.all_reduce(t, op=dist.ReduceOp.SUM, group=self.ctl, async_op=True))
        else:
            self._pf = (p, None, None)

    def drain_prefetch(self):
        if self._pf is not None:
            self._consume_prefetch()

    def _consume_prefetch(self):
        p, t, w = self._pf
        self._pf = None
        if w is not None:
            w.wait()
            return p, int(t.item())
        return p, p

    def global_positive_num(self, bbox, labels=None):
        from . import labels as LB
        p = int(LB.positive_count(bbox, labels).sum())
        if self._pf is not None:
            local, total = self._consume_prefetch()
            if local != p:
                raise RuntimeError('prefetch_positive_num() was given another batch than this step (local positives %d != %d)' % (local, p))
            return total
        if self.collective:
            t = torch.tensor([p], dtype=torch.int64)
            dist.all_reduce(t, op=dist.ReduceOp.SUM, group=self.ctl)
            p = int(t.item())
        return p

    def skipped_steps(self):
        return self.opt.skipped_steps() if hasattr(self.opt, 'skipped_steps') else 0

    def _stage(self, dev, items):
        import numpy as np
        host = []
        for t, dt in items:
            if t is None or (torch.is_tensor(t) and t.is_cuda):
                host.append(None)
            else:
                host.append(torch.as_tensor(np.ascontiguousarray(t) if isinstance(t, np.ndarray) else t).to(dt).contiguous())
        nbytes = sum((h.numel() * h.element_size() + 15) // 16 * 16 for h in host if h is not None)
        if nbytes == 0:
            return [t for t, _ in items]
        st = self.__dict__.get('_stage_buf')
        if st is None or st[0].numel() < nbytes:
            st = (torch.empty(2 * nbytes, dtype=torch.uint8).pin_memory(), torch.empty(2 * nbytes, dtype=torch.uint8, device=dev),
                  torch.cuda.Event())
            self._stage_buf = st
        pin, dbuf, ev = st
        ev.synchronize()
        out, off = [], 0
        for (t, dt), h in zip(items, host):
            if h is None:
                out.append(t); continue
            nb = h.numel() * h.element_size()
            pin[off:off + nb].view(dt).view(h.shape).copy_(h)
            out.append(dbuf[off:off + nb].view(dt).view(h.shape))
            off += (nb + 15) // 16 * 16
        dbuf[:off].copy_(pin[:off], non_blocking=True)
        ev.record()
        return out

    def step(self, x, bbox, vertices=None, labels=None, rand_neg_indices=None, lm_rand_neg_indices=None,
             positive_num_global=None, **loss_kw):
        net = self.net
        n_global = x.size(0) * self.world
        if positive_num_global is None:
            positive_num_global = self.global_positive_num(bbox, labels if net.KIND == 'DenseBoxLMLOC' else None)
        if x.is_cuda:
            import numpy as np
            from . import labels as LB
            n = x.size(0)
            rs = loss_kw.get('rng') or np.random
            _, half = LB.neg_counts(int(positive_num_global), n_global)
            if rand_neg_indices is None:
                rand_neg_indices = np.stack([rs.choice(3600, half, replace=False) for _ in range(n)]) if half else \
                    np.zeros((n, 0), np.int64)
            if net.KIND != 'DenseBox' and lm_rand_neg_indices is None:
                lm_rand_neg_indices = np.stack([np.stack([rs.choice(3600, 1, replace=False) for _ in range(n)])
                                                for _ in range(4)])
            bbox, vertices, labels, rand_neg_indices, lm_rand_neg_indices = self._stage(
                x.device, [(bbox, torch.float32), (vertices, torch.float32), (labels, torch.float32),
                           (rand_neg_indices, torch.int64), (lm_rand_neg_indices, torch.int64)])
        if self.guard_f16:
            self.opt.enable_guard(self.reducer.flat, on=net.resolved_dtype(True) == 'f16')
        self.opt.zero_grad(set_to_none=True)
        self.reducer.begin()
        net.engine().sample_offset = self.rank * x.size(0)
        self.reducer.in_step = True
        try:
            outs = net(x)
            loss = net.loss(outs, bbox, vertices, labels, rand_neg_indices, lm_rand_neg_indices,
                            batch_global=n_global, positive_num_global=positive_num_global, **loss_kw)
            direct = getattr(loss, '_dbx_direct', None)
            if direct is not None and all(t.requires_grad for t in direct[0]):
                torch.autograd.backward(direct[0], direct[1])
            else:
                loss.backward()
        finally:
            self.reducer.in_step = False
        self.reducer.finish()
        for name, p in net.named_parameters():
            p.grad = self.reducer.views.get(name)
        self.opt.step()
        return loss
```

densebox_amd/engine.py:

```python
import ctypes as C
import os
import weakref

import torch

from . import _lib
from ._lib import View, ConvDesc, check, ptr, stream_ptr

_BACKBONE = [('conv1_1_1', 3, 64), ('conv1_2_1', 64, 64), ('conv2_1_1', 64, 128), ('conv2_2_1', 128, 128),
             ('conv3_1_1', 128, 256), ('conv3_2_1', 256, 256), ('conv3_4_1', 256, 256),
             ('conv4_1_1', 256, 512), ('conv4_2_1', 512, 512), ('conv4_3_1', 512, 512), ('conv4_4_1', 512, 512)]

_HEADS = {
    'DenseBox': [('det', 1), ('loc', 4)],
    'DenseBoxLM': [('det', 1), ('loc', 4), ('landmark', 4)],
    'DenseBoxLMLOC': [('det', 1), ('loc', 4), ('landmark', 4), ('lmloc', 8)],
}


_FWD_IO = {'conv1_1_1': ('x0', 'a11'), 'conv1_2_1': ('a11', 'a12'), 'conv2_1_1': ('p1', 'a21'), 'conv2_2_1': ('a21', 'a22'),
           'conv3_1_1': ('p2', 'a31'), 'conv3_2_1': ('a31', 'a32'), 'conv3_4_1': ('a32', 'c34'), 'conv4_1_1': ('p3', 'a41'),
           'conv4_2_1': ('a41', 'a42'), 'conv4_3_1': ('a42', 'a43'), 'conv4_4_1': ('a43', 'a44')}
_BWD_IO = {'conv4_4_1': ('d_a44', 'd_a43'), 'conv4_3_1': ('d_a43', 'd_a42'), 'conv4_2_1': ('d_a42', 'd_a41'),
           'conv4_1_1': ('d_a41', 'd_p3'), 'conv3_4_1': ('d_c34', 'd_a32'), 'conv3_2_1': ('d_a32', 'd_a31'),
           'conv3_1_1': ('d_a31', 'd_p2'), 'conv2_2_1': ('d_a22', 'd_a21'), 'conv2_1_1': ('d_a21', 'd_p1'),
           'conv1_2_1': ('d_a12', 'd_a11')}
_CH = {s: (ci, co) for s, ci, co in [('conv1_1_1', 3, 64), ('conv1_2_1', 64, 64), ('conv2_1_1', 64, 128), ('conv2_2_1', 128, 128),
                                     ('conv3_1_1', 128, 256), ('conv3_2_1', 256, 256), ('conv3_4_1', 256, 256),
                                     ('conv4_1_1', 256, 512), ('conv4_2_1', 512, 512), ('conv4_3_1', 512, 512),
                                     ('conv4_4_1', 512, 512)]}


def _align(x, a=256):
    return (x + a - 1) // a * a


class Buf:

    def __init__(self, name, n, h, w, c, pad, dtype_id):
        self.name, self.n, self.h, self.w, self.c, self.pad = name, n, h, w, c, pad
        self.dtype_id = dtype_id
        self.es = _lib.ESIZE[dtype_id]
        self.hp, self.wp = h + 2 * pad, w + 2 * pad
        self.bytes = n * self.hp * self.wp * c * self.es
        self.guard = _align(max(4 * (self.wp + 2), 576 + 4 * self.wp) * c * self.es)
        self.base = None

    def view(self, c_off=0, c=None):
        return View(C.c_void_p(self.base), self.n, self.h, self.w, self.pad, self.c, c_off,
                    self.c - c_off if c is None else c)


class Plan:

    @staticmethod
    def env_flags():
        return tuple(os.environ.get(k, '1') != '0' for k in ('DBX_LIN_BWD', 'DBX_REFINE_LINEAR', 'DBX_POOL_IDX', 'DBX_HEADS_GEN')) + \
            (os.environ.get('DBX_F32_LIN', '0') == '1',)

    def __init__(self, kind, n, h, w, dtype_id, device, train):
        self.kind, self.n, self.h, self.w, self.dtype_id, self.train = kind, n, h, w, dtype_id, train
        self.flags = Plan.env_flags()
        lin_bwd, lin_refine, use_idx, heads_gen, f32_lin = self.flags
        lin_bwd = lin_bwd and (dtype_id != _lib.F32 or f32_lin)
        es = _lib.ESIZE[dtype_id]
        self.cin0 = 16 // es
        self.rdt = dtype_id
        self.crf = 8 if _lib.ESIZE[self.rdt] == 2 else 32
        nh = len(_HEADS[kind])
        h2, w2, h4, w4, h8, w8 = h // 2, w // 2, h // 4, w // 4, h // 8, w // 8
        self.h4, self.w4 = h4, w4
        B = {}

        def add(name, hh, ww, c, pad=1, dt=None):
            B[name] = Buf(name, n, hh, ww, c, pad, dtype_id if dt is None else dt)
        add('x0', h, w, self.cin0)
        self.a12_alias = es == 2 and h % 2 == 0 and w % 2 == 0 and (not train or use_idx)
        add('a11', h, w, 64)
        if not self.a12_alias:
            add('a12', h, w, 64)
        add('p1', h2, w2, 64)
        add('a21', h2, w2, 128); add('a22', h2, w2, 128); add('p2', h4, w4, 128)
        add('a31', h4, w4, 256); add('a32', h4, w4, 256)
        add('fusion', h4, w4, 768)
        add('p3', h8, w8, 256)
        add('a41', h8, w8, 512); add('a42', h8, w8, 512); add('a43', h8, w8, 512); add('a44', h8, w8, 512)
        add('hid', h4, w4, 512 * nh, pad=0)
        rf_convs = kind != 'DenseBox' and train and not lin_refine
        if rf_convs:
            add('rf_in', h4, w4, self.crf, pad=0, dt=self.rdt)
            add('rf_p', h8, w8, self.crf, pad=1, dt=self.rdt)
            add('rf_1', h8 - 2, w8 - 2, 64, pad=2, dt=self.rdt)
            add('rf_2', h8 - 6, w8 - 6, 64, pad=0, dt=self.rdt)
            add('rf_u', h4, w4, 64, pad=0, dt=self.rdt)
        if train:
            for nm in ('a11', 'a21', 'a22', 'a31', 'a32', 'a41', 'a42', 'a43', 'a44'):
                add('d_' + nm, B[nm].h, B[nm].w, B[nm].c)
            add('d_a12', h, w, 64)
            add('d_c34', h4, w4, 256)
            if not lin_bwd:
                add('d_ups', h4, w4, 512, pad=0)
            add('d_p1', h2, w2, 64, pad=0); add('d_p2', h4, w4, 128, pad=0); add('d_p3', h8, w8, 256, pad=0)
            add('d_g44', h8, w8, 512 * nh, pad=1)
            add('d_out', h4, w4, self.crf * nh, pad=0)
            L = _lib.lib()
            gen_fits = n * h4 * w4 < (1 << 24) and n * h4 * w4 * self.crf * nh * es < (1 << 31) and self.crf <= 8
            if dtype_id == _lib.F32:
                self.heads_gen = bool(heads_gen and lin_bwd)
            else:
                self.heads_gen = bool(heads_gen and lin_bwd and gen_fits and
                                      L.dbx_head2_backward_up_fused(dtype_id, C.byref(B['hid'].view()), C.byref(B['d_g44'].view())) and
                                      L.dbx_heads1_wgrad_gen_ok(dtype_id, C.byref(B['fusion'].view(512, 256)), nh))
            if not self.heads_gen or dtype_id == _lib.F32:
                add('d_hid', h4, w4, 512 * nh, pad=1)
            if rf_convs:
                add('d_rfo', h4, w4, self.crf, pad=0)
                add('d_rf_u', h4, w4, 64, pad=0)
                add('d_rf_2', h8 - 6, w8 - 6, 64, pad=4)
                add('d_rf_1', h8 - 2, w8 - 2, 64, pad=2)
                add('d_rf_p', h8, w8, self.crf, pad=0)
                add('d_rf_in', h4, w4, self.crf, pad=0)
        off = 0
        for b in B.values():
            off += b.guard
            b.off = off
            off += _align(b.bytes) + b.guard
        self.total = off
        if not train:
            self.heads_gen = False
        self.drop_active = self.drop_hash = False
        self.frag = {}
        self.drop_seed = 0
        self.mask_buf = None
        self.ws = torch.zeros(off, dtype=torch.uint8, device=device)
        self.pool_idx = None
        if train and os.environ.get('DBX_POOL_IDX', '1') != '0':
            self.pool_idx = {k: torch.empty(n * (hh // 2) * (ww // 2) * (c // 2) + 16, dtype=torch.uint8, device=device)
                             for k, (hh, ww, c) in {'a12': (h, w, 64), 'a22': (h2, w2, 128), 'fusion': (h4, w4, 256)}.items()}
        base = self.ws.data_ptr()
        assert base % 256 == 0
        for b in B.values():
            b.base = base + b.off
        if self.a12_alias:
            B['a12'] = B['a11']
        self.B = B


_PARAM_ENGINE = {}


def register_params(engine, params):
    if len(_PARAM_ENGINE) > 4096:
        for k in [k for k, (rp, re_) in _PARAM_ENGINE.items() if rp() is None or re_() is None]:
            del _PARAM_ENGINE[k]
    re_ = weakref.ref(engine)
    for p in params:
        ent = _PARAM_ENGINE.get(id(p))
        if ent is None or ent[0]() is not p or ent[1]() is not engine:
            _PARAM_ENGINE[id(p)] = (weakref.ref(p), re_)


def engine_of(params):
    eng = None
    for p in params:
        ent = _PARAM_ENGINE.get(id(p))
        if ent is None or ent[0]() is not p:
            return None
        e = ent[1]()
        if e is None or (eng is not None and e is not eng):
            return None
        eng = e
    return eng


class Engine:
    def __init__(self, net):
        self.net = net
        self.kind = net.KIND
        self.L = _lib.lib()
        self.plans = {}
        self.wcache = {}
        self.bias_cache = {}
        self.last_plan = None
        self.grad_sink = None
        self.profile = None
        self._defer = None
        self._defer_keep = []
        self._table_keys = set()
        self._tables = {}
        self._wsig = None
        self._plans_conv = {}
        self.act_hook = None

    def grad_order(self):
        heads = _HEADS[self.kind]
        names = []
        if self.kind != 'DenseBox':
            for s_ in ('conv6_3_det', 'conv6_2_det', 'conv6_1_det'):
                names += [s_ + '.weight', s_ + '.bias']
        for s_, _ in heads:
            names += ['conv5_2_%s.weight' % s_, 'conv5_2_%s.bias' % s_]
        names += ['conv5_1_%s.weight' % s_ for s_, _ in heads] + ['conv5_1_%s.bias' % s_ for s_, _ in heads]
        for s_, _, _ in reversed(_BACKBONE):
            names += [s_ + '.weight', s_ + '.bias']
        return names

    def _param(self, name):
        mod, attr = name.rsplit('.', 1)
        return getattr(getattr(self.net, mod), attr)

    def _packed(self, key, builder, versions):
        ent = self.wcache.get(key)
        if ent is not None and (ent[0] == versions or key in self._table_keys):
            return ent[1]
        t = builder(ent[1] if ent is not None else None)
        self.wcache[key] = (versions, t)
        return t

    def _pack(self, dt, mode, w, rows_pad, cin_pad, kh, kw, out=None, row_off=0, k_off=0):
        d = ConvDesc(dt, kh, kw, 0, cin_pad, rows_pad, 0, 0)
        elems = self.L.dbx_conv_packed_elems(C.byref(d))
        if out is None:
            out = torch.zeros(elems * _lib.ESIZE[dt], dtype=torch.uint8, device=w.device)
        co, ci = w.shape[0], w.shape[1]
        if self._defer is not None:
            es = _lib.ESIZE[dt]
            ktot = (kh * kw * cin_pad * es + 127) // 128 * 128 // es
            self._defer.append((w.data_ptr(), out.data_ptr(), co, ci, kh * kw, mode, rows_pad if mode >= 4 else ktot, cin_pad,
                                row_off, k_off, rows_pad))
            self._defer_keep.append(out)
            return out
        check(self.L.dbx_pack_weight(dt, mode, ptr(w.detach()), co, ci, kh, kw, ptr(out), rows_pad, cin_pad,
                                     row_off, k_off, stream_ptr()))
        return out

    def _bias(self, names, pad_to):
        ps = [self._param(n + '.bias') for n in names]
        key = tuple(names)
        ver = tuple((p._version, p.data_ptr()) for p in ps)
        ent = self.bias_cache.get(key)
        if ent is not None and (ent[0] == ver or key in self._table_keys):
            return ent[1]
        b = ent[1] if ent is not None else torch.zeros(pad_to, dtype=torch.float32, device=ps[0].device)
        o = 0
        for p in ps:
            if self._defer is not None:
                self._defer.append((p.data_ptr(), b.data_ptr(), p.numel(), 1, 1, 2, 0, 0, o, 0, 0))
            else:
                b[o:o + p.numel()].copy_(p.detach())
            o += p.numel()
        if self._defer is not None:
            self._defer_keep.append(b)
        self.bias_cache[key] = (ver, b)
        return b

    def _w_fwd(self, dt, stem, cin_pad, cout_pad, frag=False):
        w = self._param(stem + '.weight')
        mode = 4 if frag else 0
        return self._packed((stem, mode, dt),
                            lambda old: self._pack(dt, mode, w, cout_pad, cin_pad, w.shape[2], w.shape[3], out=old),
                            (w._version, w.data_ptr()))

    def conv_plan(self, dt, x, y, kh, kw, cpad, cin_pad, cout_pad, epi):
        key = (dt, x.n, x.h, x.w, x.pad, x.ld, x.c_off, x.c, y.pad, y.ld, y.c_off, y.c, kh, kw, cpad, cin_pad, cout_pad,
               epi & ~_lib.CONV_WFRAG)
        ent = self._plans_conv.get(key)
        if ent is None:
            d = ConvDesc(dt, kh, kw, cpad, cin_pad, cout_pad, epi & ~_lib.CONV_WFRAG, 0)
            out = _lib.ConvPlan()
            check(self.L.dbx_conv_plan(C.byref(d), C.byref(x), C.byref(y), C.byref(out)))
            ent = (out.kernel, out.name.decode(), bool(out.w_frag))
            self._plans_conv[key] = ent
        return ent

    def _w_heads1(self, dt, frag=False):
        heads = _HEADS[self.kind]
        ws = [self._param('conv5_1_%s.weight' % s) for s, _ in heads]
        mode = 4 if frag else 0

        def build(out):
            for i, w in enumerate(ws):
                out = self._pack(dt, mode, w, 512 * len(ws), 768, 1, 1, out=out, row_off=512 * i)
# ... 458 lines not shown
            else:
                self._conv(dt, B['fusion'].view(), yv, wp, bf, 1, 1, 0, 768, 64, _lib.EPI_BIAS | _lib.EPI_F32_NCHW)
            o = 0
            for stem, k in heads:
                outs[stem] = big[:, o:o + k].contiguous()
                o += k
        else:
            epi = _lib.EPI_BIAS
            dm = None
            P.drop_active = bool(self._dropout_p() > 0.0)
            P.drop_hash = P.drop_active and self.net.dropout_masks is None
            if P.drop_hash:
                P.drop_seed = self._next_drop_seed()
                epi |= _lib.EPI_DROPHASH
            elif P.drop_active:
                dm = self._fill_dropout(P, heads)
                epi |= _lib.EPI_DROPMASK
            hfrag = (epi & _lib.EPI_DROPMASK) == 0 and self._frag_heads(P, dt, 'f')
            ktot = sum(k for _, k in heads)
            big = None
            b1 = self._bias(['conv5_1_' + s_ for s_, _ in heads], 512 * nh)
            b2 = self._bias(['conv5_2_' + s_ for s_, _ in heads], 64)
            fk = self._heads_fused(P, dt) if (P.drop_hash and not (epi & _lib.EPI_DROPMASK)) else 0
            if fk == 1 and not hfrag:
                fk = 0
            if fk:
                need = L.dbx_heads_forward_fused_scratch_bytes(nh, n * h4 * w4)
                if getattr(self, '_hf_scratch', None) is None or self._hf_scratch.numel() < need:
                    self._hf_scratch = torch.empty(int(need), dtype=torch.uint8, device=dev)
                d = ConvDesc(dt, 1, 1, 0, 768, 512 * nh, epi | (_lib.CONV_WFRAG if fk == 1 else 0), P.drop_seed)
                prof = self.profile
                if prof is not None:
                    ev0, ev1 = torch.cuda.Event(enable_timing=True), torch.cuda.Event(enable_timing=True)
                    ev0.record()
                for stem, k in heads:
                    outs[stem] = torch.empty((n, k, h4, w4), dtype=torch.float32, device=dev)
                check(L.dbx_heads_forward_fused_heads(C.byref(d), C.byref(B['fusion'].view()), ptr(self._w_heads1(dt, frag=fk == 1)), ptr(b1),
                                                      C.byref(B['hid'].view()), ptr(self._w_heads2_frag(dt) if fk == 1 else self._w_heads2_rows0(dt)), ptr(b2),
                                                      (C.c_int32 * nh)(*[k for _, k in heads]), nh,
                                                      (C.c_void_p * nh)(*[outs[stem].data_ptr() for stem, _ in heads]), ptr(self._hf_scratch), s))
                if prof is not None:
                    ev1.record()
                    prof.append({'kernel': ('conv3x3_ws_kernel<%s,1,1,2>' if fk == 1 else 'conv3x3_p8_kernel<%s,1,1>') % ('f16', 'bf16', 'f32')[dt],
                                 'flops': 2.0 * n * h4 * w4 * (768 * 512 * nh + 512 * ktot), 'start': ev0, 'end': ev1})
            else:
                self._conv(dt, B['fusion'].view(), B['hid'].view(), self._w_heads1(dt, frag=hfrag), b1, 1, 1, 0, 768, 512 * nh,
                           epi | (_lib.CONV_WFRAG if hfrag else 0),
                           dropmask=dm, dm_ld=512 * nh, drop_seed=P.drop_seed if P.drop_hash else 0)
                big = torch.empty((n, ktot, h4, w4), dtype=torch.float32, device=dev)
                yv = View(C.c_void_p(big.data_ptr()), n, h4, w4, 0, ktot, 0, ktot)
                self._conv(dt, B['hid'].view(), yv, self._w_heads2(dt), b2, 1, 1, 0,
                           512 * nh, 64, _lib.EPI_BIAS | _lib.EPI_F32_NCHW, alg_ci=512)
            o = 0
            for stem, k in heads:
                if big is not None:
                    outs[stem] = big[:, o:o + k].contiguous()
                o += k
        lin_rf = os.environ.get('DBX_REFINE_LINEAR', '1') != '0'
        P.refine_fwd = None
        if kind != 'DenseBox' and (not train or lin_rf):
            wf7, bf7, vf7 = self._w_refine_folded()
            lmk, det = outs['landmark'], outs['det']
            if not lmk.is_contiguous():
                lmk = lmk.contiguous()
            if not det.is_contiguous():
                det = det.contiguous()
            small = torch.empty((n, 1, h4 // 2 - 6, w4 // 2 - 6), dtype=torch.float32, device=dev)
            check(L.dbx_refine_eval(ptr(lmk), ptr(det), n, h4, w4, ptr(wf7), ptr(bf7), ptr(small), s))
            o = torch.empty((n, 1, h4, w4), dtype=torch.float32, device=dev)
            check(L.dbx_upsample_bilinear_nchw_f32(ptr(small), n, h4 // 2 - 6, w4 // 2 - 6, ptr(o), h4, w4, s))
            outs['refine'] = o
            if train:
                P.refine_fwd = (lmk, det, wf7, vf7)
        elif kind != 'DenseBox':
            rdt = P.rdt
            saved, self._defer = self._defer, None
            w61, w62, w63 = (self._w_fwd(rdt, 'conv6_1_det', P.crf, 64), self._w_fwd(rdt, 'conv6_2_det', 64, 64),
                             self._w_fwd(rdt, 'conv6_3_det', 64, 64))
            self._defer = saved
            rin = B['rf_in'].view()
            check(L.dbx_nchw_to_framed_ch(rdt, ptr(outs['landmark']), 4, C.byref(rin), 0, s))
            check(L.dbx_nchw_to_framed_ch(rdt, ptr(outs['det']), 1, C.byref(rin), 4, s))
            check(L.dbx_maxpool2x2(rdt, C.byref(rin), C.byref(B['rf_p'].view()), s))
            self._conv(rdt, B['rf_p'].view(), B['rf_1'].view(), w61,
                       self._bias(['conv6_1_det'], 64), 3, 3, 0, P.crf, 64, _lib.EPI_BIAS, alg_ci=5)
            self._conv(rdt, B['rf_1'].view(), B['rf_2'].view(), w62,
                       self._bias(['conv6_2_det'], 64), 5, 5, 0, 64, 64, _lib.EPI_BIAS)
            check(L.dbx_upsample_bilinear(rdt, C.byref(B['rf_2'].view()), C.byref(B['rf_u'].view()), s))
            o = torch.empty((n, 1, h4, w4), dtype=torch.float32, device=dev)
            yv = View(C.c_void_p(o.data_ptr()), n, h4, w4, 0, 1, 0, 1)
            self._conv(rdt, B['rf_u'].view(), yv, w63,
                       self._bias(['conv6_3_det'], 64), 1, 1, 0, 64, 64, _lib.EPI_BIAS | _lib.EPI_F32_NCHW)
            outs['refine'] = o
        return outs

    def _dropout_p(self):
        drops = [m for m in self.net.modules() if isinstance(m, torch.nn.Dropout)]
        p = drops[0].p if drops else 0.0
        if p not in (0.0, 0.5):
            raise RuntimeError('densebox_amd: the head Dropout supports p=0.5 (reference) or p=0, got %r' % p)
        return p

    def _fill_dropout(self, P, heads):
        nh = len(heads)
        inj = self.net.dropout_masks
        dev = P.ws.device
        m = torch.empty((P.n, P.h4, P.w4, nh, 512), dtype=torch.uint8, device=dev)
        for i, (stem, _) in enumerate(heads):
            m[:, :, :, i, :] = inj[stem].to(dev).permute(0, 2, 3, 1).to(torch.uint8)
        P.mask_buf = m
        return m.data_ptr()

    def read_activation(self, name, c_off=0, c=None):
        P = self.last_plan
        b = P.B[name]
        v = b.view(c_off, c)
        out = torch.empty((b.n, v.c, b.h, b.w), dtype=torch.float32, device=P.ws.device)
        check(self.L.dbx_framed_to_nchw_f32(P.dtype_id, C.byref(v), ptr(out), stream_ptr()))
        return out

    def _w_bwd(self, dt, stem, rows_pad, cin_pad, frag=False):
        w = self._param(stem + '.weight')
        mode = 5 if frag else 1
        return self._packed((stem, mode, dt),
                            lambda old: self._pack(dt, mode, w, rows_pad, cin_pad, w.shape[2], w.shape[3], out=old),
                            (w._version, w.data_ptr()))

    def _w_heads1_bwd(self, dt, frag=False):
        heads = _HEADS[self.kind]
        ws = [self._param('conv5_1_%s.weight' % s) for s, _ in heads]
        mode = 5 if frag else 1

        def build(out):
            for i, w in enumerate(ws):
                out = self._pack(dt, mode, w, 768, 512 * len(ws), 1, 1, out=out, k_off=512 * i)
            return out
        return self._packed(('heads1', mode, dt), build, tuple((w._version, w.data_ptr()) for w in ws))

    def _w_heads1_bwd_part(self, dt, part, frag=False):
        heads = _HEADS[self.kind]
        ws = [self._param('conv5_1_%s.weight' % s) for s, _ in heads]
        mode = 5 if frag else 1
        rows, roff = (512, 0) if part == 'a' else (256, -512)

        def build(out):
            for i, w in enumerate(ws):
                out = self._pack(dt, mode, w, rows, 512 * len(ws), 1, 1, out=out, row_off=roff, k_off=512 * i)
            return out
        return self._packed(('heads1_' + part, mode, dt), build, tuple((w._version, w.data_ptr()) for w in ws))

    def _lin_bwd(self, dt):
        return (dt != _lib.F32 or os.environ.get('DBX_F32_LIN', '0') == '1') and os.environ.get('DBX_LIN_BWD', '1') != '0'

    def _d_hid(self, P):
        b = P.B.get('d_hid')
        if b is None:
            hb = P.B['hid']
            b = Buf('d_hid', hb.n, hb.h, hb.w, hb.c, 1, hb.dtype_id)
            P._d_hid_store = torch.zeros(2 * b.guard + _align(b.bytes) + 256, dtype=torch.uint8, device=P.ws.device)
            b.base = _align(P._d_hid_store.data_ptr() + b.guard)
            P.B['d_hid'] = b
        return b

    def _wgrad(self, dt, dz, x, kh, kw, cpad, co, ci, dw, db, accumulate=0, ci_total=None, ci_off=0, gen=None, pool=None):
        need = self.L.dbx_conv_wgrad_scratch_bytes(dt, C.byref(dz), C.byref(x), kh, kw)
        if getattr(self, '_wg_scratch', None) is None or self._wg_scratch.numel() < need:
            self._wg_scratch = torch.empty(int(need * 1.25) + 1024, dtype=torch.uint8, device=dw.device)
        prof = self.profile
        if prof is not None:
            ev0, ev1 = torch.cuda.Event(enable_timing=True), torch.cuda.Event(enable_timing=True)
            ev0.record()
        if pool is not None:
            dyv, nib, nch, write_dz = pool
            check(self.L.dbx_conv_wgrad_pool_dz(dt, C.byref(dyv), ptr(nib), nch, C.byref(dz), C.byref(x), kh, kw, cpad, co, ci, ptr(dw), ptr(db),
                                                ptr(self._wg_scratch), accumulate, write_dz, stream_ptr()))
        elif gen is not None:
            dov, w2p, ks, nh, use_hash, seed = gen
            check(self.L.dbx_heads1_wgrad_gen(dt, C.byref(dov), C.byref(x), w2p, ks, nh, use_hash, seed, ci, ptr(dw), ci_total, ci_off, ptr(db),
                                              ptr(self._wg_scratch), stream_ptr()))
        elif ci_total is None:
            check(self.L.dbx_conv_wgrad(dt, C.byref(dz), C.byref(x), kh, kw, cpad, co, ci, ptr(dw), ptr(db),
                                        ptr(self._wg_scratch), accumulate, stream_ptr()))
        else:
            check(self.L.dbx_conv_wgrad_slice(dt, C.byref(dz), C.byref(x), kh, kw, cpad, co, ci, ptr(dw), ci_total, ci_off, ptr(db),
                                              ptr(self._wg_scratch), accumulate, stream_ptr()))
        if prof is not None:
            ev1.record()
            buf = C.create_string_buffer(64)
            check(self.L.dbx_conv_wgrad_plan(dt, C.byref(dz), C.byref(x), kh, kw, buf, 64, None))
            name = buf.value.decode()
            if gen is not None:
                name = name.replace('>', ',gen>')
            if pool is not None:
                name = name.replace('>', ',pool+dz>' if pool[3] else ',pool>')
            prof.append({'kernel': name, 'flops': 2.0 * dz.n * dz.h * dz.w * kh * kw * ci * co, 'start': ev0, 'end': ev1})

    def backward_raw(self, grad_outs):
        L, kind = self.L, self.kind
        P = self.last_plan
        assert P is not None and P.train, 'backward needs a preceding training-mode forward'
        B, dt, n = P.B, P.dtype_id, P.n
        s = stream_ptr()
        dev = P.ws.device
        heads = _HEADS[kind]
        nh = len(heads)
        h4, w4 = P.h4, P.w4
        G = {}

        sink = self.grad_sink

        def new_grad(name):
            p = self._param(name)
            g = sink.grad_view(name) if sink is not None else torch.empty_like(p, dtype=torch.float32)
            G[name] = g
            return g

        def gout(name, k):
            g = grad_outs.get(name)
            if g is None:
                return torch.zeros((n, k, h4, w4), dtype=torch.float32, device=dev)
            return g.to(torch.float32).contiguous()

        main = torch.cuda.current_stream()
        side = None
        multi = sink is not None and getattr(sink, 'world', 1) > 1
        if self.profile is None and not multi and os.environ.get('DBX_SIDE_STREAM', '0') == '1':
            if getattr(self, '_side', None) is None:
                self._side = torch.cuda.Stream(device=dev)
            side = self._side

        def on_side(fn):
            if side is None:
                return fn()
            ev = torch.cuda.Event()
            ev.record(main)
            side.wait_event(ev)
            with torch.cuda.stream(side):
                return fn()

        def conv_bwd(stem, dz, x, kh, kw, cpad, co, ci):
            dw, db = new_grad(stem + '.weight'), new_grad(stem + '.bias')
            pool = None
            if stem == 'conv1_2_1' and pool12:
                pool = (B['d_p1'].view(), P.pool_idx['a12'], 64, 1 if pool12 == 1 else 0)

            def run():
                self._wgrad(dt, dz, x, kh, kw, cpad, co, ci, dw, db, pool=pool)
                if sink is not None:
                    sink.ready([stem + '.weight', stem + '.bias'])
            on_side(run)

        def dgrad(stem, src, dst, kh, kw, cpad, rows_pad, cin_pad, gate=None, epi=0, dropmask=None):
            frag = stem in _BWD_IO and kh == 3 and self._frag(P, dt, stem, 'b')
            wp = self._w_bwd(dt, stem, rows_pad, cin_pad, frag=frag)
            e = epi | (_lib.EPI_GATE if gate is not None else 0) | (_lib.CONV_WFRAG if frag else 0)
            self._conv(dt, src, dst, wp, None, kh, kw, cpad, cin_pad, rows_pad, e, gate=gate, dropmask=dropmask,
                       dm_ld=512 * nh)

        override = {}
        if kind != 'DenseBox' and P.refine_fwd is not None:
            lmk, det, wf7, vf7 = P.refine_fwd
            pn = ['conv6_1_det.weight', 'conv6_1_det.bias', 'conv6_2_det.weight', 'conv6_2_det.bias', 'conv6_3_det.weight', 'conv6_3_det.bias']
            ps = [self._param(nm).detach() for nm in pn]
            gs = [new_grad(nm) for nm in pn]

            def f32c(t):
                return None if t is None else t.to(torch.float32).contiguous()
            g_lm, g_det = f32c(grad_outs.get('landmark')), f32c(grad_outs.get('det'))
            o_lm = torch.empty((n, 4, h4, w4), dtype=torch.float32, device=dev)
            o_det = torch.empty((n, 1, h4, w4), dtype=torch.float32, device=dev)
            need = L.dbx_refine_backward_scratch_bytes(n, h4, w4)
            if getattr(self, '_rf_scratch', None) is None or self._rf_scratch.numel() < need:
                self._rf_scratch = torch.empty(int(need), dtype=torch.uint8, device=dev)
            d_rf = gout('refine', 1)
            check(L.dbx_refine_backward(ptr(d_rf), ptr(lmk), ptr(det), n, h4, w4, *[ptr(p) for p in ps], ps[0].shape[0], ptr(wf7), ptr(vf7),
                                        ptr(g_lm), ptr(g_det), ptr(o_lm), ptr(o_det), *[ptr(g_) for g_ in gs], ptr(self._rf_scratch), s))
            if sink is not None:
                sink.ready(pn)
            override = {'landmark': o_lm, 'det': o_det}
        elif kind != 'DenseBox' and os.environ.get('DBX_REFINE_LINEAR', '1') != '0':
            raise RuntimeError('densebox_amd: backward of the refine branch without its forward state (no training-mode forward on this plan)')
        elif kind != 'DenseBox':
            d_rfo = B['d_rfo'].view()
            check(L.dbx_nchw_to_framed(dt, ptr(gout('refine', 1)), 1, C.byref(d_rfo), s))
            conv_bwd('conv6_3_det', d_rfo, B['rf_u'].view(), 1, 1, 0, 1, 64)
            dgrad('conv6_3_det', d_rfo, B['d_rf_u'].view(), 1, 1, 0, 64, P.crf)
            check(L.dbx_upsample_bilinear_bwd(dt, C.byref(B['d_rf_u'].view()), C.byref(B['d_rf_2'].view()), None, s))
            conv_bwd('conv6_2_det', B['d_rf_2'].view(), B['rf_1'].view(), 5, 5, 0, 64, 64)
            dgrad('conv6_2_det', B['d_rf_2'].view(), B['d_rf_1'].view(), 5, 5, 4, 64, 64)
            conv_bwd('conv6_1_det', B['d_rf_1'].view(), B['rf_p'].view(), 3, 3, 0, 64, 5)
            dgrad('conv6_1_det', B['d_rf_1'].view(), B['d_rf_p'].view(), 3, 3, 2, 64, 64)
            check(L.dbx_maxpool2x2_bwd(dt, C.byref(B['rf_in'].view()), C.byref(B['d_rf_p'].view()),
                                       C.byref(B['d_rf_in'].view()), 0, 0, s))

        slot = {}
        srcs = []
        for i, (stem, k) in enumerate(heads):
            slot[stem] = B['d_out'].view(P.crf * i, P.crf)
            src = override.get(stem)
            srcs.append(src if src is not None else gout(stem, k))
        if override or kind == 'DenseBox':
            check(L.dbx_nchw_to_framed_slots(dt, (C.c_void_p * nh)(*[t.data_ptr() for t in srcs]), (C.c_int32 * nh)(*[k for _, k in heads]), nh, P.crf,
                                             C.byref(B['d_out'].view()), s))
        else:
            for (stem, k), t in zip(heads, srcs):
                check(L.dbx_nchw_to_framed(dt, ptr(t), k, C.byref(slot[stem]), s))
        if kind != 'DenseBox' and not override:
            check(L.dbx_framed_add_ch(dt, C.byref(B['d_rf_in'].view()), 0, 4, C.byref(slot['landmark']), 0, s))
            check(L.dbx_framed_add_ch(dt, C.byref(B['d_rf_in'].view()), 4, 1, C.byref(slot['det']), 0, s))

        hv = B['hid'].view()
        need = L.dbx_head2_wgrad_scratch_bytes(nh, hv.n * hv.h)
        if getattr(self, '_h2_scratch', None) is None or self._h2_scratch.numel() < need:
            self._h2_scratch = torch.empty(int(need), dtype=torch.uint8, device=dev)
        dw2 = [new_grad('conv5_2_%s.weight' % st) for st, _ in heads]
        db2 = [new_grad('conv5_2_%s.bias' % st) for st, _ in heads]
        prof = self.profile
        if prof is not None:
            ev0, ev1 = torch.cuda.Event(enable_timing=True), torch.cuda.Event(enable_timing=True)
            ev0.record()
        w2s = [self._param('conv5_2_%s.weight' % st).detach() for st, _ in heads]
        ks = (C.c_int32 * nh)(*[k for _, k in heads])
        h2_names = ['conv5_2_%s.weight' % st for st, _ in heads] + ['conv5_2_%s.bias' % st for st, _ in heads]
        mask_p = C.c_void_p(P.mask_buf.data_ptr()) if (P.drop_active and not P.drop_hash) else None
        hash_on, hash_seed = (1 if P.drop_hash else 0), (P.drop_seed if P.drop_hash else 0)
        lin = self._lin_bwd(dt)
        up_done = False
        gen = bool(getattr(P, 'heads_gen', False) and lin and side is None and mask_p is None)
        if gen and dt != _lib.F32:
            dhid_v = View(None, hv.n, hv.h, hv.w, 1, 512 * nh, 0, 512 * nh)
        else:
            dhid_v = self._d_hid(P).view()
        w2p = (C.c_void_p * nh)(*[w.data_ptr() for w in w2s])
        if side is not None:
            def run_h2():
                check(L.dbx_head2_wgrad(dt, C.byref(B['d_out'].view()), C.byref(hv), ks, nh,
                                        (C.c_void_p * nh)(*[t.data_ptr() for t in dw2]), (C.c_void_p * nh)(*[t.data_ptr() for t in db2]),
                                        ptr(self._h2_scratch), stream_ptr()))
                if sink is not None:
                    sink.ready(h2_names)
            on_side(run_h2)
            check(L.dbx_head2_dgrad(dt, C.byref(B['d_out'].view()), (C.c_void_p * nh)(*[w.data_ptr() for w in w2s]), ks, nh,
                                    C.byref(dhid_v), mask_p, 512 * nh, hash_on, hash_seed, s))
        elif lin:
            check(L.dbx_head2_backward_up(dt, C.byref(B['d_out'].view()), C.byref(hv), (C.c_void_p * nh)(*[w.data_ptr() for w in w2s]), ks, nh,
                                          C.byref(dhid_v), mask_p, 512 * nh, hash_on, hash_seed,
                                          (C.c_void_p * nh)(*[t.data_ptr() for t in dw2]), (C.c_void_p * nh)(*[t.data_ptr() for t in db2]),
                                          ptr(self._h2_scratch), C.byref(B['d_g44'].view()), s))
            up_done = True
            if gen and dt == _lib.F32:
                bh = P.B['d_hid']
                P.ws[bh.off:bh.off + bh.bytes].view(torch.float32).fill_(float('nan'))
        else:
            check(L.dbx_head2_backward(dt, C.byref(B['d_out'].view()), C.byref(hv), (C.c_void_p * nh)(*[w.data_ptr() for w in w2s]), ks, nh,
                                       C.byref(dhid_v), mask_p, 512 * nh, hash_on, hash_seed,
                                       (C.c_void_p * nh)(*[t.data_ptr() for t in dw2]), (C.c_void_p * nh)(*[t.data_ptr() for t in db2]),
                                       ptr(self._h2_scratch), s))
            if sink is not None:
                sink.ready(h2_names)
        if prof is not None:
            ev1.record()
            prof.append({'kernel': ('head2_backward_up_kernel<%s>' if up_done else 'head2_wgrad_kernel<%s>') % ('f16', 'bf16', 'f32')[dt],
                         'flops': 2.0 * hv.n * hv.h * hv.w * 512 * sum(k for _, k in heads) * (1 if side is not None else 2), 'start': ev0, 'end': ev1})
        w1n = ['conv5_1_%s.weight' % st for st, _ in heads]
        b1n = ['conv5_1_%s.bias' % st for st, _ in heads]
        if sink is not None:
            dw1, db1 = sink.region(w1n).view(512 * nh, 768, 1, 1), sink.region(b1n)
        else:
            dw1 = torch.empty((512 * nh, 768, 1, 1), dtype=torch.float32, device=dev)
            db1 = torch.empty((512 * nh,), dtype=torch.float32, device=dev)
        c34 = B['fusion'].view(512, 256)
        if lin and not up_done:
            check(L.dbx_upsample_bilinear_bwd(dt, C.byref(dhid_v), C.byref(B['d_g44'].view()), None, s))

        def run_h1():
            if lin:
                self._wgrad(dt, B['d_g44'].view(), B['a44'].view(), 1, 1, 0, 512 * nh, 512, dw1, None, ci_total=768, ci_off=0)
                if gen:
                    self._wgrad(dt, dhid_v, c34, 1, 1, 0, 512 * nh, 256, dw1, db1, ci_total=768, ci_off=512,
                                gen=(B['d_out'].view(), w2p, ks, nh, hash_on, hash_seed))
                else:
                    self._wgrad(dt, dhid_v, c34, 1, 1, 0, 512 * nh, 256, dw1, db1, ci_total=768, ci_off=512)
            else:
                self._wgrad(dt, dhid_v, B['fusion'].view(), 1, 1, 0, 512 * nh, 768, dw1, db1)
            if sink is not None:
                sink.ready(w1n + b1n)
        on_side(run_h1)
        for i, (stem, _) in enumerate(heads):
            G['conv5_1_%s.weight' % stem] = dw1[512 * i:512 * (i + 1)]
            G['conv5_1_%s.bias' % stem] = db1[512 * i:512 * (i + 1)]
        row_bytes = 512 * nh * _lib.ESIZE[dt]
        if lin:
            fa, fc = self._frag_heads(P, dt, 'ba'), self._frag_heads(P, dt, 'bc')
            self._conv(dt, B['d_g44'].view(), B['d_a44'].view(), self._w_heads1_bwd_part(dt, 'a', frag=fa), None, 1, 1, 0, 512 * nh, 512,
                       _lib.EPI_GATE | (_lib.CONV_WFRAG if fa else 0), gate=B['a44'].view())
            if gen:
                if prof is not None:
                    ev0, ev1 = torch.cuda.Event(enable_timing=True), torch.cuda.Event(enable_timing=True)
                    ev0.record()
                check(L.dbx_heads1_dgrad_gen(dt, C.byref(B['d_out'].view()), w2p, ks, nh, hash_on, hash_seed,
                                             ptr(self._w_heads1_bwd_part(dt, 'c', frag=dt != _lib.F32)), C.byref(B['d_c34'].view()), C.byref(c34), s))
                if prof is not None:
                    ev1.record()
                    prof.append({'kernel': 'heads1_dgrad_gen_kernel<%s>' % ('f16', 'bf16', 'f32')[dt],
                                 'flops': 2.0 * hv.n * hv.h * hv.w * 512 * nh * (256 + 8), 'start': ev0, 'end': ev1})
            else:
                if fc and getattr(P, 'heads_gen', False):
                    fc = self.conv_plan(dt, dhid_v, B['d_c34'].view(), 1, 1, 0, 512 * nh, 256, _lib.EPI_GATE)[2]
                self._conv(dt, dhid_v, B['d_c34'].view(), self._w_heads1_bwd_part(dt, 'c', frag=fc), None, 1, 1, 0, 512 * nh, 256,
                           _lib.EPI_GATE | (_lib.CONV_WFRAG if fc else 0), gate=c34)
        elif dt != _lib.F32:
            bfrag = self._frag_heads(P, dt, 'b')
            w1t = self._w_heads1_bwd(dt, frag=bfrag)
            d = ConvDesc(dt, 1, 1, 0, 512 * nh, 768, _lib.CONV_WFRAG if bfrag else 0, 0)
            prof = self.profile
            if prof is not None:
                ev0, ev1 = torch.cuda.Event(enable_timing=True), torch.cuda.Event(enable_timing=True)
                ev0.record()
            check(L.dbx_conv_forward_split(C.byref(d), C.byref(dhid_v), ptr(w1t), None, C.byref(B['d_ups'].view()), None,
                                           C.byref(B['d_c34'].view()), C.byref(c34), 512, _lib.EPI_GATE, s))
            if prof is not None:
                ev1.record()
                hv = dhid_v
                dv = B['d_ups'].view()
                both = View(dv.ptr, dv.n, dv.h, dv.w, dv.pad, 768, 0, 768)
                prof.append({'kernel': self.conv_plan(dt, hv, both, 1, 1, 0, 512 * nh, 768, 0)[1] if bfrag else
                             'conv_igemm_dma_kernel<%s,256,256>' % ('f16', 'bf16', 'f32')[dt],
                             'flops': 2.0 * hv.n * hv.h * hv.w * 512 * nh * 768, 'start': ev0, 'end': ev1})
        else:
            w1t = self._w_heads1_bwd(dt, frag=False)
            self._conv(dt, dhid_v, B['d_ups'].view(), w1t, None, 1, 1, 0, 512 * nh, 512, 0)
            self._conv(dt, dhid_v, B['d_c34'].view(), w1t[512 * row_bytes:], None, 1, 1, 0, 512 * nh, 256,
                       _lib.EPI_GATE, gate=c34)
        if not lin:
            check(L.dbx_upsample_bilinear_bwd(dt, C.byref(B['d_ups'].view()), C.byref(B['d_a44'].view()),
                                              C.byref(B['a44'].view()), s))

        chain = [
            ('conv4_4_1', 'd_a44', 'a43', 512, 512, 'd_a43', 'a43'),
            ('conv4_3_1', 'd_a43', 'a42', 512, 512, 'd_a42', 'a42'),
            ('conv4_2_1', 'd_a42', 'a41', 512, 512, 'd_a41', 'a41'),
            ('conv4_1_1', 'd_a41', 'p3', 256, 512, 'd_p3', None),
            ('pool', 'fusion', 'd_p3', 'd_c34', 1),
            ('conv3_4_1', 'd_c34', 'a32', 256, 256, 'd_a32', 'a32'),
            ('conv3_2_1', 'd_a32', 'a31', 256, 256, 'd_a31', 'a31'),
            ('conv3_1_1', 'd_a31', 'p2', 128, 256, 'd_p2', None),
            ('pool', 'a22', 'd_p2', 'd_a22', 0),
            ('conv2_2_1', 'd_a22', 'a21', 128, 128, 'd_a21', 'a21'),
            ('conv2_1_1', 'd_a21', 'p1', 64, 128, 'd_p1', None),
            ('pool', 'a12', 'd_p1', 'd_a12', 0),
            ('conv1_2_1', 'd_a12', 'a11', 64, 64, 'd_a11', 'a11'),
            ('conv1_1_1', 'd_a11', 'x0', 3, 64, None, None),
        ]
        fused11 = False
        pool12 = 0
        if P.pool_idx is not None and os.environ.get('DBX_POOL_WGRAD', '1') != '0' and \
                L.dbx_conv_wgrad_pool_dz_ok(dt, C.byref(B['d_a12'].view()), C.byref(B['a11'].view()), 3, 3):
            pool12 = 2 if (os.environ.get('DBX_POOL_WGRAD') == '2' or side is not None) else 1
        for item in chain:
            if item[0] == 'conv1_1_1' and fused11:
                continue
            if item[0] == 'conv1_2_1':
                stem, dzn, xn, cin, cout, dxn, gaten = item
                d12 = ConvDesc(dt, 3, 3, 1, 64, 64, _lib.EPI_GATE, 0)
                dzv, gv, x0v = B[dzn].view(), B[gaten].view(), B['x0'].view()
                if side is None and os.environ.get('DBX_FUSE_WG1', '1') != '0' and L.dbx_conv_dgrad_wgrad1_fusable(C.byref(d12), C.byref(dzv), C.byref(gv), C.byref(x0v)):
                    conv_bwd(stem, dzv, B[xn].view(), 3, 3, 1, cout, cin)
                    need = L.dbx_conv_dgrad_wgrad1_scratch_bytes()
                    if getattr(self, '_wg1_scratch', None) is None or self._wg1_scratch.numel() < need:
                        self._wg1_scratch = torch.empty(int(need), dtype=torch.uint8, device=dev)
                    dw1, db1 = new_grad('conv1_1_1.weight'), new_grad('conv1_1_1.bias')
                    if prof is not None:
                        ev0, ev1 = torch.cuda.Event(enable_timing=True), torch.cuda.Event(enable_timing=True)
                        ev0.record()
                    check(L.dbx_conv_dgrad_wgrad1(C.byref(d12), C.byref(dzv), ptr(self._w_bwd(dt, stem, 64, 64, frag=False)),
                                                  C.byref(gv), C.byref(x0v), 3, ptr(dw1), ptr(db1), ptr(self._wg1_scratch), 0, s))
                    if prof is not None:
                        ev1.record()
                        prof.append({'kernel': self.conv_plan(dt, dzv, B[dxn].view(), 3, 3, 1, 64, 64, _lib.EPI_GATE)[1],
                                     'flops': 2.0 * dzv.n * dzv.h * dzv.w * 9 * 64 * (64 + 3), 'start': ev0, 'end': ev1})
                    if sink is not None:
                        sink.ready(['conv1_1_1.weight', 'conv1_1_1.bias'])
                    fused11 = True
                    continue
            if item[0] == 'pool':
                _, xname, dyname, dxname, acc = item
                if xname == 'a12' and pool12 == 1:
                    continue
                if P.pool_idx is not None:
                    check(L.dbx_maxpool2x2_bwd_idx(dt, ptr(P.pool_idx[xname]), C.byref(B[dyname].view()), C.byref(B[dxname].view()),
                                                   acc, 1, s))
                    continue
                xv = c34 if xname == 'fusion' else B[xname].view()
                check(L.dbx_maxpool2x2_bwd(dt, C.byref(xv), C.byref(B[dyname].view()), C.byref(B[dxname].view()),
                                           acc, 1, s))
                continue
            stem, dzn, xn, cin, cout, dxn, gaten = item
            conv_bwd(stem, B[dzn].view(), B[xn].view(), 3, 3, 1, cout, cin)
            if dxn is not None:
                dgrad(stem, B[dzn].view(), B[dxn].view(), 3, 3, 1, max(64, cin), cout,
                      gate=B[gaten].view() if gaten else None)
        if side is not None:
            main.wait_stream(side)
        return G
```

densebox_amd/labels.py:

```python
import ctypes as C

import numpy as np
import torch

from . import _lib
from ._lib import check, ptr, stream_ptr

HW = 60


def _dev(t, device=None, dtype=torch.float32):
    if t is None:
        return None
    t = torch.as_tensor(t)
    if not t.is_cuda:
        t = t.to(device or 'cuda')
    return t.to(dtype).contiguous()


def init_score_map(bbox, batch_size=None, ratio=0.3, labels=None):
    assert ratio == 0.3, 'the kernels hard-code the reference ratio 0.3'
    bbox = _dev(bbox)
    n = bbox.size(0)
    assert batch_size is None or batch_size == n
    out = torch.empty((n, 1, HW, HW), dtype=torch.float32, device=bbox.device)
    lab = _dev(labels, bbox.device)
    check(_lib.lib().dbx_init_score_map(ptr(bbox), ptr(lab), n, ptr(out), stream_ptr()))
    return out


def init_score(bboxes, labels, ratio=0.3):
    assert bboxes.size(0) == labels.size(0) and tuple(labels.shape) == (labels.size(0), 1)
    return init_score_map(bboxes, ratio=ratio, labels=labels)


def _offset(coords, c, labels):
    coords = _dev(coords)
    n = coords.size(0)
    assert tuple(coords.shape) == (n, c)
    out = torch.empty((n, c, HW, HW), dtype=torch.float32, device=coords.device)
    lab = _dev(labels, coords.device)
    check(_lib.lib().dbx_init_offset_map(ptr(coords), ptr(lab), n, c, ptr(out), stream_ptr()))
    return out


def init_loc_map(bboxes, batch_size=None):
    return _offset(bboxes, 4, None)


def init_loc(bboxes, labels):
    return _offset(bboxes, 4, labels)


def init_lm_locmap(vertices, batch_size=None):
    return _offset(vertices, 8, None)


def init_lm_locmap_pn(vertices, labels):
    return _offset(vertices, 8, labels)


def _heat(vertices, labels, clamp):
    v = _dev(vertices)
    n = v.size(0)
    assert tuple(v.shape) == (n, 8)
    out = torch.empty((n, 4, HW, HW), dtype=torch.float32, device=v.device)
    lab = _dev(labels, v.device)
    check(_lib.lib().dbx_init_lm_heatmap(ptr(v), ptr(lab), n, clamp, ptr(out), stream_ptr()))
    return out


def init_lm_heatmap(vertices, batch_size=None):
    v = torch.as_tensor(vertices).float()
    if bool(((v + 0.5).to(torch.int64) >= HW).any()):
        raise IndexError('landmark index 60 is out of bounds for dimension with size 60')
    return _heat(vertices, None, 0)


def init_lm_heatmap_pn(vertices, labels):
    return _heat(vertices, labels, 1)


def mask_by_sel(loss_mask, pos_indices, neg_indices):
    assert tuple(loss_mask.shape) == (loss_mask.size(0), 1, HW, HW) and loss_mask.is_cuda and loss_mask.is_contiguous()
    pos = _dev(pos_indices, loss_mask.device, torch.int64)
    neg = _dev(neg_indices, loss_mask.device, torch.int64)
    check(_lib.lib().dbx_mask_by_sel(ptr(loss_mask), loss_mask.size(0), ptr(pos), pos.size(0), ptr(neg),
                                     neg.size(1) if neg.dim() == 2 else 0, stream_ptr()))


def mask_gray_zone_cls(loss_mask, bboxes, ratio=0.3, gray_border=2.0):
    assert ratio == 0.3 and gray_border == 2.0
    assert loss_mask.is_cuda and loss_mask.is_contiguous() and tuple(loss_mask.shape[1:]) == (1, HW, HW)
    bb = _dev(bboxes, loss_mask.device)
    check(_lib.lib().dbx_mask_gray_zone_cls(ptr(loss_mask), ptr(bb), None, loss_mask.size(0), stream_ptr()))


def mask_gray_zone_cls_pn(loss_mask, bboxes, labels, ratio=0.3, gray_border=2.0):
    assert ratio == 0.3 and gray_border == 2.0
    assert loss_mask.is_cuda and loss_mask.is_contiguous() and tuple(loss_mask.shape[1:]) == (1, HW, HW)
    bb, lab = _dev(bboxes, loss_mask.device), _dev(labels, loss_mask.device)
    check(_lib.lib().dbx_mask_gray_zone_cls(ptr(loss_mask), ptr(bb), ptr(lab), loss_mask.size(0), stream_ptr()))


def mask_gray_zone_lm(loss_mask, pos_indices, lm_id=0, gray_border=2.0):
    assert lm_id in (0, 1, 2, 3)
    assert loss_mask.is_cuda and loss_mask.is_contiguous() and tuple(loss_mask.shape[1:]) == (1, HW, HW)
    pos = _dev(pos_indices, loss_mask.device, torch.int64)
    check(_lib.lib().dbx_mask_gray_zone_lm(ptr(loss_mask), loss_mask.size(0), ptr(pos), pos.size(0), stream_ptr()))


def gen_neg_loss(loss_orig, map_gt):
    assert loss_orig.size() == map_gt.size()
    return loss_orig * (1.0 - map_gt)


def positive_count(bbox, labels=None):
    b = np.asarray(torch.as_tensor(bbox).detach().cpu(), np.float32)
    n = b.shape[0]
    lab = None if labels is None else np.asarray(torch.as_tensor(labels).detach().cpu(), np.float32).reshape(n)
    out = np.zeros(n, np.int64)
    for i in range(n):
        if lab is not None and lab[i] == 0.0:
            continue
        ext = []
        for c0, c2 in ((b[i, 0], b[i, 2]), (b[i, 1], b[i, 3])):
            centre = float(np.float32(c0 + c2)) * 0.5
            rw = np.float32(np.float32(0.3) * np.float32(c2 - c0))
            org = int(centre - float(np.float32(rw * np.float32(0.5))) + 0.5)
            end = int(float(org) + float(rw) + 0.5)
            lo, hi = org, end + 1
            lo = max(lo + HW, 0) if lo < 0 else min(lo, HW)
            hi = max(hi + HW, 0) if hi < 0 else min(hi, HW)
            ext.append(max(0, hi - lo))
        out[i] = ext[0] * ext[1]
    return out


def neg_counts(positive_num, batch):
    neg_num = int(float(positive_num) / float(batch) + 0.5)
    return neg_num, int(neg_num * 0.5 + 0.5)
```

densebox_amd/loss.py:

```python
import ctypes as C

import numpy as np
import torch

from . import _lib, labels as LB
from ._lib import LossDesc, LossIO, check, ptr, stream_ptr

_KIND_ID = {'DenseBox': 0, 'DenseBoxLM': 1, 'DenseBoxLMLOC': 2}


class _LossFn(torch.autograd.Function):
    @staticmethod
    def forward(ctx, loss, n_out, *outs_and_grads):
        outs, grads = outs_and_grads[:n_out], outs_and_grads[n_out:]
        ctx.grads = grads
        return loss.clone()

    @staticmethod
    def backward(ctx, g):
        return (None, None) + tuple(d * g for d in ctx.grads) + (None,) * len(ctx.grads)


def densebox_loss(kind, outputs, bbox, vertices=None, labels=None, rand_neg_indices=None, lm_rand_neg_indices=None,
                  lambda_loc=3.0, lambda_det=1.0, lambda_lm=0.5, batch_global=None, positive_num_global=None,
                  return_debug=False, rng=None):
    kid = _KIND_ID[kind]
    if kind == 'DenseBox':
        score, loc = outputs
        lm = rf = lmloc = None
    elif kind == 'DenseBoxLM':
        score, loc, lm, rf = outputs
        lmloc = None
    else:
        score, rf, loc, lm, lmloc = outputs
    dev = score.device
    n = score.size(0)
    assert tuple(score.shape[1:]) == (1, 60, 60), 'the dense loss is defined on the 60x60 training grid'
    use_labels = kind == 'DenseBoxLMLOC'
    P = int(LB.positive_count(bbox, labels if use_labels else None).sum()) if positive_num_global is None \
        else int(positive_num_global)
    _, half = LB.neg_counts(P, n if batch_global is None else batch_global)
    rs = rng if rng is not None else np.random
    if rand_neg_indices is None:
        rand_neg_indices = np.stack([rs.choice(3600, half, replace=False) for _ in range(n)]) if half else \
            np.zeros((n, 0), np.int64)
    if kid != 0 and lm_rand_neg_indices is None:
        lm_rand_neg_indices = np.stack([np.stack([rs.choice(3600, 1, replace=False) for _ in range(n)])
                                        for _ in range(4)])
    rn = LB._dev(rand_neg_indices, dev, torch.int64).reshape(n, half)
    lrn = LB._dev(lm_rand_neg_indices, dev, torch.int64).reshape(4, n, 1) if kid != 0 else None
    bb = LB._dev(bbox, dev)
    vt = LB._dev(vertices, dev) if kid != 0 else None
    lb = LB._dev(labels, dev) if use_labels else None

    def c32(t):
        return None if t is None else t.detach().to(torch.float32).contiguous()
    o = [c32(t) for t in (score, loc, lm, rf, lmloc)]
    g = [None if t is None else torch.empty_like(t) for t in o]
    loss = torch.empty(1, dtype=torch.float32, device=dev)
    scratch = torch.empty((_lib.lib().dbx_loss_scratch_bytes(n) + 7) // 8, dtype=torch.float64, device=dev)
    dbg = {}
    if return_debug:
        dbg['mask_cls'] = torch.empty((n, 1, 60, 60), dtype=torch.float32, device=dev)
        dbg['neg_idx'] = torch.empty((n, 2 * half), dtype=torch.int64, device=dev)
        dbg['pos_count'] = torch.empty(n, dtype=torch.int32, device=dev)
        if kid != 0:
            dbg['mask_lm'] = torch.empty((n, 4, 60, 60), dtype=torch.float32, device=dev)
            dbg['lm_neg_idx'] = torch.empty((4, n, 2), dtype=torch.int64, device=dev)
    d = LossDesc(kid, n, half, lambda_loc, lambda_det, lambda_lm, 1 if use_labels else 0)
    io = LossIO()
    for name, t in (('bbox', bb), ('vertices', vt), ('labels', lb), ('rand_neg', rn), ('lm_rand_neg', lrn),
                    ('score', o[0]), ('loc', o[1]), ('lm', o[2]), ('rf', o[3]), ('lmloc', o[4]),
                    ('d_score', g[0]), ('d_loc', g[1]), ('d_lm', g[2]), ('d_rf', g[3]), ('d_lmloc', g[4]),
                    ('loss', loss), ('mask_cls', dbg.get('mask_cls')), ('mask_lm', dbg.get('mask_lm')),
                    ('neg_idx', dbg.get('neg_idx')), ('lm_neg_idx', dbg.get('lm_neg_idx')),
                    ('pos_count', dbg.get('pos_count'))):
        setattr(io, name, t.data_ptr() if t is not None else None)
    check(_lib.lib().dbx_loss_forward_backward(C.byref(d), C.byref(io), ptr(scratch), stream_ptr()))
    live = [(t, gg) for t, gg in zip((score, loc, lm, rf, lmloc), g) if t is not None]
    out = _LossFn.apply(loss[0], len(live), *[t for t, _ in live], *[gg for _, gg in live])
    out._dbx_direct = ([t for t, _ in live], [gg for _, gg in live])
    if return_debug:
        dbg['half'] = half
        dbg['grads'] = {k: gg for k, gg in zip(('score', 'loc', 'lm', 'rf', 'lmloc'), g) if gg is not None}
        return out, dbg
    return out
```

include/densebox_hip.h:

```cpp
#ifndef DENSEBOX_HIP_H
#define DENSEBOX_HIP_H

#include <stdint.h>

#ifdef __cplusplus
extern "C" {
#endif

enum dbx_status {
    DBX_OK = 0,
    DBX_ERR_ARG = -1,
    DBX_ERR_HIP = -2,
    DBX_ERR_DTYPE = -3
};

enum dbx_dtype { DBX_F16 = 0, DBX_BF16 = 1, DBX_F32 = 2 };

const char* dbx_last_error(void);
#define DBX_ABI_VERSION 13
int dbx_version(void);
int dbx_device_arch(int device);

typedef struct dbx_view {
    void*   ptr;
    int32_t n, h, w;
    int32_t pad;
    int32_t ld;
    int32_t c_off;
    int32_t c;
} dbx_view;

enum dbx_epilogue {
    DBX_EPI_BIAS     = 1,
    DBX_EPI_RELU     = 2,
    DBX_EPI_GATE     = 4,
    DBX_EPI_DROPMASK = 8,
    DBX_EPI_ACCUM    = 16,
    DBX_EPI_F32_NCHW = 32,
    DBX_EPI_DROPHASH = 64,
    DBX_CONV_WFRAG   = 128
};

typedef struct dbx_conv_desc {
    int32_t dtype;
    int32_t kh, kw;
    int32_t cpad;
    int32_t cin_pad;
    int32_t cout_pad;
    int32_t epilogue;
    uint32_t drop_seed;
} dbx_conv_desc;

int64_t dbx_conv_packed_elems(const dbx_conv_desc* d);
int dbx_conv_forward(const dbx_conv_desc* d, const dbx_view* x, const void* w_packed, const float* bias,
                     const dbx_view* y, const dbx_view* gate, const uint8_t* dropmask, int32_t dropmask_ld,
                     void* stream);
enum dbx_conv_kernel { DBX_K_IGEMM = 1, DBX_K_DMA = 2, DBX_K_BAND = 3, DBX_K_C64 = 4, DBX_K_C8 = 5, DBX_K_WS = 6, DBX_K_P8 = 7 };
typedef struct dbx_conv_plan_t {
    int32_t kernel;
    int32_t tile_m, tile_n;
    int32_t w_frag;
    char    name[64];
} dbx_conv_plan_t;
int dbx_conv_plan(const dbx_conv_desc* d, const dbx_view* x, const dbx_view* y, dbx_conv_plan_t* out);

int dbx_heads_forward_fusable(const dbx_conv_desc* d, const dbx_view* x, const dbx_view* hid, const int32_t* k, int32_t nh);
int64_t dbx_heads_forward_fused_scratch_bytes(int32_t nh, int64_t pixels);
int dbx_heads_forward_fused(const dbx_conv_desc* d, const dbx_view* x, const void* w1_frag, const float* bias1, const dbx_view* hid,
                            const void* w2_frag, const float* bias2, const int32_t* k, int32_t nh, float* out_nchw, void* scratch,
                            void* stream);
int dbx_heads_forward_fused_heads(const dbx_conv_desc* d, const dbx_view* x, const void* w1_frag, const float* bias1, const dbx_view* hid,
                                  const void* w2_frag, const float* bias2, const int32_t* k, int32_t nh, float* const* outs, void* scratch,
                                  void* stream);

int dbx_conv_forward_split(const dbx_conv_desc* d, const dbx_view* x, const void* w_packed, const float* bias,
                           const dbx_view* y, const dbx_view* gate, const dbx_view* y2, const dbx_view* gate2,
                           int32_t split_c, int32_t epilogue2, void* stream);

int dbx_conv_pool_fusable(const dbx_conv_desc* d, const dbx_view* x, const dbx_view* y);
int dbx_conv_forward_pool(const dbx_conv_desc* d, const dbx_view* x, const void* w_packed, const float* bias,
                          const dbx_view* y, const dbx_view* ypool, int32_t write_full, void* stream);
int dbx_conv_forward_pool_idx(const dbx_conv_desc* d, const dbx_view* x, const void* w_packed, const float* bias,
                              const dbx_view* y, const dbx_view* ypool, int32_t write_full, void* idx, void* stream);

int dbx_pack_weight(int32_t dtype, int32_t mode, const float* w_oihw, int32_t co, int32_t ci, int32_t kh, int32_t kw,
                    void* w_packed, int32_t rows_pad, int32_t cin_pad, int32_t row_off, int32_t k_off, void* stream);

int dbx_pack_multi(int32_t dtype, const void* jobs, int32_t count, int64_t max_elems, void* stream);

int dbx_sgd_pack_step(int32_t dtype, const void* jobs, int32_t count, int64_t max_elems, float* const* ptrs, float lr, float momentum,
                      float weight_decay, int32_t first_step, void* stream);

int dbx_head2_dgrad(int32_t dtype, const dbx_view* d_out, const float* const* w2, const int32_t* k, int32_t nh,
                    const dbx_view* d_hid, const uint8_t* dropmask, int32_t dropmask_ld, int32_t use_hash, uint32_t drop_seed,
                    void* stream);
int64_t dbx_head2_wgrad_scratch_bytes(int32_t nh, int32_t rows);
int dbx_head2_wgrad(int32_t dtype, const dbx_view* d_out, const dbx_view* hid, const int32_t* k, int32_t nh,
                    float* const* dw, float* const* db, void* scratch, void* stream);
int dbx_head2_backward(int32_t dtype, const dbx_view* d_out, const dbx_view* hid, const float* const* w2, const int32_t* k,
                       int32_t nh, const dbx_view* d_hid, const uint8_t* dropmask, int32_t dropmask_ld, int32_t use_hash,
                       uint32_t drop_seed, float* const* dw, float* const* db, void* scratch, void* stream);
int dbx_head2_backward_up(int32_t dtype, const dbx_view* d_out, const dbx_view* hid, const float* const* w2, const int32_t* k,
                          int32_t nh, const dbx_view* d_hid, const uint8_t* dropmask, int32_t dropmask_ld, int32_t use_hash,
                          uint32_t drop_seed, float* const* dw, float* const* db, void* scratch, const dbx_view* d_g44, void* stream);
int dbx_conv_wgrad_pool_dz_ok(int32_t dtype, const dbx_view* dz, const dbx_view* x, int32_t kh, int32_t kw);
int dbx_conv_wgrad_pool_dz(int32_t dtype, const dbx_view* dy, const void* idx, int32_t idx_channels, const dbx_view* dz, const dbx_view* x,
                           int32_t kh, int32_t kw, int32_t cpad, int32_t co, int32_t ci, float* dw_oihw, float* db, void* scratch,
                           int32_t accumulate, int32_t write_dz, void* stream);
int dbx_head2_backward_up_fused(int32_t dtype, const dbx_view* hid, const dbx_view* d_g44);
int dbx_heads1_wgrad_gen_ok(int32_t dtype, const dbx_view* x, int32_t nh);
int dbx_heads1_wgrad_gen(int32_t dtype, const dbx_view* d_out, const dbx_view* x, const float* const* w2, const int32_t* k, int32_t nh,
                         int32_t use_hash, uint32_t drop_seed, int32_t ci, float* dw_oihw, int32_t dw_ci_total, int32_t dw_ci_off,
                         float* db, void* scratch, void* stream);
int dbx_heads1_dgrad_gen(int32_t dtype, const dbx_view* d_out, const float* const* w2, const int32_t* k, int32_t nh, int32_t use_hash,
                         uint32_t drop_seed, const void* w1t_frag, const dbx_view* y, const dbx_view* gate, void* stream);

int dbx_fold_heads(const float* w2, const float* b2, const float* w1, const float* b1, int32_t k, float* w_out,
                   float* b_out, void* stream);
int dbx_fold_refine(const float* w1, const float* b1, const float* w2, const float* b2, const float* w3, const float* b3,
                    int32_t ci, int32_t cm, float* w_out, float* b_out, float* v_out, void* stream);
int dbx_refine_eval(const float* landmark_nchw, const float* score_nchw, int32_t n, int32_t h, int32_t w, const float* w_fold,
                    const float* b_fold, float* out_small, void* stream);
int dbx_upsample_bilinear_nchw_f32(const float* x, int32_t planes, int32_t hi, int32_t wi, float* y, int32_t ho, int32_t wo,
                                   void* stream);
int64_t dbx_refine_backward_scratch_bytes(int32_t n, int32_t h, int32_t w);
int dbx_refine_backward(const float* d_refine, const float* landmark, const float* score, int32_t n, int32_t h, int32_t w,
                        const float* w1, const float* b1, const float* w2, const float* b2, const float* w3, const float* b3,
                        int32_t cm, const float* w_fold, const float* v_fold, const float* g_landmark, const float* g_score, float* out_landmark,
                        float* out_score, float* dw1, float* db1, float* dw2, float* db2, float* dw3, float* db3, void* scratch,
                        void* stream);

int64_t dbx_conv_wgrad_scratch_bytes(int32_t dtype, const dbx_view* dz, const dbx_view* x, int32_t kh, int32_t kw);
int dbx_conv_wgrad(int32_t dtype, const dbx_view* dz, const dbx_view* x, int32_t kh, int32_t kw, int32_t cpad,
                   int32_t co, int32_t ci, float* dw_oihw, float* db, void* scratch, int32_t accumulate, void* stream);
int dbx_conv_wgrad_slice(int32_t dtype, const dbx_view* dz, const dbx_view* x, int32_t kh, int32_t kw, int32_t cpad,
                         int32_t co, int32_t ci, float* dw_oihw, int32_t dw_ci_total, int32_t dw_ci_off, float* db, void* scratch,
                         int32_t accumulate, void* stream);
int dbx_conv_wgrad_plan(int32_t dtype, const dbx_view* dz, const dbx_view* x, int32_t kh, int32_t kw, char* name, int32_t name_len,
                        int32_t* splits);

int64_t dbx_conv_dgrad_wgrad1_scratch_bytes(void);
int dbx_conv_dgrad_wgrad1_fusable(const dbx_conv_desc* d, const dbx_view* dz, const dbx_view* gate, const dbx_view* x0);
int dbx_conv_dgrad_wgrad1(const dbx_conv_desc* d, const dbx_view* dz, const void* w_packed, const dbx_view* gate, const dbx_view* x0,
                          int32_t ci, float* dw_oihw, float* db, void* scratch, int32_t accumulate, void* stream);

int dbx_nchw_to_framed(int32_t dtype, const float* x_nchw, int32_t c_src, const dbx_view* y, void* stream);
int dbx_u8hwc_to_framed(int32_t dtype, const uint8_t* x_nhwc, const dbx_view* y, const float* mean3, const float* std3,
                        void* stream);
int dbx_nchw_to_framed_ch(int32_t dtype, const float* x_nchw, int32_t c_src, const dbx_view* y, int32_t c_dst_off,
                          void* stream);
int dbx_nchw_to_framed_slots(int32_t dtype, const float* const* x_nchw, const int32_t* k, int32_t nslots, int32_t slot,
                             const dbx_view* y, void* stream);
int dbx_framed_to_nchw_f32(int32_t dtype, const dbx_view* x, float* y_nchw, void* stream);
int dbx_framed_add_ch(int32_t dtype, const dbx_view* src, int32_t c_src_off, int32_t n_ch, const dbx_view* dst,
                      int32_t c_dst_off, void* stream);
int dbx_maxpool2x2(int32_t dtype, const dbx_view* x, const dbx_view* y, void* stream);
int dbx_maxpool2x2_bwd(int32_t dtype, const dbx_view* x, const dbx_view* dy, const dbx_view* dx,
                       int32_t accumulate, int32_t relu_gate, void* stream);
int64_t dbx_maxpool_idx_bytes(int32_t n, int32_t h, int32_t w, int32_t c);
int dbx_maxpool2x2_idx(int32_t dtype, const dbx_view* x, const dbx_view* y, void* idx, void* stream);
int dbx_maxpool2x2_bwd_idx(int32_t dtype, const void* idx, const dbx_view* dy, const dbx_view* dx,
                           int32_t accumulate, int32_t relu_gate, void* stream);
int dbx_upsample_bilinear(int32_t dtype, const dbx_view* x, const dbx_view* y, void* stream);
int dbx_upsample_bilinear_bwd(int32_t dtype, const dbx_view* dy, const dbx_view* dx, const dbx_view* gate, void* stream);

typedef struct dbx_loss_desc {
    int32_t kind;
    int32_t n;
    int32_t half_neg;
    float   lambda_loc, lambda_det, lambda_lm;
    int32_t use_labels;
} dbx_loss_desc;

typedef struct dbx_loss_io {
    const float* bbox;
    const float* vertices;
    const float* labels;
    const int64_t* rand_neg;
    const int64_t* lm_rand_neg;
    const float* score;  const float* loc;  const float* lm;  const float* rf;  const float* lmloc;
    float* d_score; float* d_loc; float* d_lm; float* d_rf; float* d_lmloc;
    float* loss;
    float* mask_cls;
    float* mask_lm;
    int64_t* neg_idx;
    int64_t* lm_neg_idx;
    int32_t* pos_count;
} dbx_loss_io;

int64_t dbx_loss_scratch_bytes(int32_t n);
int dbx_loss_forward_backward(const dbx_loss_desc* d, const dbx_loss_io* io, void* scratch, void* stream);
int dbx_count_positives(const float* bbox, const float* labels, int32_t n, int32_t* count_per_sample, void* stream);

int dbx_init_score_map(const float* bbox, const float* labels, int32_t n, float* out, void* stream);
int dbx_init_offset_map(const float* coords, const float* labels, int32_t n, int32_t c, float* out, void* stream);
int dbx_init_lm_heatmap(const float* vertices, const float* labels, int32_t n, int32_t clamp, float* out, void* stream);
int dbx_mask_by_sel(float* mask, int32_t n, const int64_t* pos_idx, int64_t n_pos, const int64_t* neg_idx, int32_t n_neg, void* stream);
int dbx_mask_gray_zone_cls(float* mask, const float* bbox, const float* labels, int32_t n, void* stream);
int dbx_mask_gray_zone_lm(float* mask, int32_t n, const int64_t* pos_idx, int64_t n_pos, void* stream);

int dbx_sgd_step(float* const* ptrs, const int64_t* sizes, int32_t count, int64_t max_size,
                 float lr, float momentum, float weight_decay, int32_t first_step, void* stream);
int dbx_grad_guard(const float* grads, int64_t n, int32_t* guard, int32_t step_id, void* stream);
int dbx_sgd_step_guarded(float* const* ptrs, const int64_t* sizes, int32_t count, int64_t max_size, float lr, float momentum,
                         float weight_decay, int32_t first_step, int32_t* guard, int32_t step_id, void* stream);
int dbx_sgd_pack_step_guarded(int32_t dtype, const void* jobs, int32_t count, int64_t max_elems, float* const* ptrs, float lr, float momentum,
                              float weight_decay, int32_t first_step, int32_t* guard, int32_t step_id, void* stream);

int dbx_detect(const float* score, const float* loc, const float* lm_heat, const float* lm_loc,
               int32_t rows, int32_t cols, int32_t K, double nms_thresh,
               double* dets, int32_t det_cols, int64_t* topk_idx, int32_t* keep, void* scratch, void* stream);
int64_t dbx_detect_scratch_bytes(int32_t rows, int32_t cols, int32_t K);
int64_t dbx_detect_batch_scratch_bytes(int32_t batch, int32_t rows, int32_t cols, int32_t K);
int dbx_detect_batch(const float* score, const float* loc, const float* lm_heat, const float* lm_loc,
                     int32_t batch, int32_t rows, int32_t cols, int32_t K, double nms_thresh,
                     double* dets, int32_t det_cols, int64_t* topk_idx, int32_t* keep, void* scratch, void* stream);
int dbx_nms(const double* dets, int32_t n, int32_t det_cols, double nms_thresh, int32_t* keep, void* scratch, void* stream);

int64_t dbx_detect_thresh_batch_scratch_bytes(int32_t batch, int32_t rows, int32_t cols, int32_t max_dets);
int dbx_detect_thresh_batch(const float* score, const float* loc, const float* lm_heat, const float* lm_loc,
                            int32_t batch, int32_t rows, int32_t cols, float score_thresh, int32_t max_dets, double nms_thresh,
                            double* dets, int32_t det_cols, int64_t* topk_idx, int32_t* keep, int32_t* counts, void* scratch,
                            void* stream);
int64_t dbx_thresh_rows_batch_scratch_bytes(int32_t batch, int32_t rows, int32_t cols, int32_t max_dets);
int dbx_thresh_rows_batch(const float* score, const float* loc, const float* lm_heat, const float* lm_loc,
                          int32_t batch, int32_t rows, int32_t cols, float score_thresh, int32_t max_dets,
                          double* dets, int32_t det_cols, int64_t* topk_idx, int32_t* counts, void* scratch, void* stream);
int64_t dbx_nms_large_scratch_bytes(int32_t n);
int dbx_nms_large(const double* dets, int32_t n, int32_t det_cols, double nms_thresh, int32_t* keep, void* scratch, void* stream);

typedef struct dbx_merge_xform { double scale, off_x, off_y; } dbx_merge_xform;
int64_t dbx_merge_nms_batch_workspace_bytes(int32_t levels, int32_t batch, int32_t K);
int dbx_merge_nms_batch(const double* const* level_dets, const dbx_merge_xform* xform, int32_t levels, int32_t batch, int32_t K,
                        int32_t det_cols, double nms_thresh, double* out_dets, int32_t* out_keep, void* workspace, void* stream);

int64_t dbx_merge_nms_thresh_batch_workspace_bytes(int32_t levels, int32_t batch, int32_t max_dets);
int dbx_merge_nms_thresh_batch(const double* const* level_dets, const int32_t* const* level_counts, const dbx_merge_xform* xform,
                               int32_t levels, int32_t batch, int32_t max_dets, int32_t det_cols, double nms_thresh,
                               double* out_dets, int32_t* out_keep, int32_t* out_counts, void* workspace, void* stream);

int dbx_perspective_matrix(const float* src_xy, const float* dst_xy, double* m9);
int dbx_warp_perspective_u8(const uint8_t* src, int32_t sh, int32_t sw, int32_t c, const double* m9, uint8_t* dst,
                            int32_t dh, int32_t dw, void* stream);
typedef struct dbx_warp_job {
    const uint8_t* src;
    int32_t sh, sw;
    double m9[9];
    int32_t dh, dw;
    int32_t x0, y0, oh, ow;
    int64_t dst_off;
} dbx_warp_job;
int64_t dbx_warp_batch_workspace_bytes(int32_t njobs);
int dbx_warp_perspective_batch_u8(const dbx_warp_job* jobs, int32_t njobs, int32_t c, uint8_t* dst, void* workspace, void* stream);

typedef struct dbx_crop_frame {
    const uint8_t* src;
    int32_t sh, sw;
} dbx_crop_frame;
int dbx_plate_crops_batch(const dbx_crop_frame* frames, int32_t nframes, int32_t c, const double* quads, int64_t row_stride,
                          int64_t frame_stride, const int32_t* sel, int32_t slots, int32_t ow, int32_t oh, uint8_t* dst, int32_t* ok,
                          double* m9_out, void* stream);

typedef struct dbx_eval_record {
    double  score;
    double  lm_err;
    int32_t status;
    int32_t frame;
} dbx_eval_record;
int dbx_match_gt_batch(const double* dets, int32_t det_cols, int64_t det_rows, const int32_t* keep, const int32_t* prefix,
                       int32_t batch, int32_t slots, const double* gt, int32_t gt_cols, const int32_t* gt_counts,
                       const uint8_t* gt_ignore, int32_t max_gt, double iou_thresh, int32_t* status, int32_t* gt_index,
                       double* iou, double* lm_err, int32_t* tally, void* stream);
int dbx_eval_append(const double* dets, int32_t det_cols, int64_t det_rows, const int32_t* keep, const int32_t* prefix,
                    int32_t batch, int32_t slots, const int32_t* status, const double* lm_err, const int32_t* tally,
                    dbx_eval_record* records, int64_t capacity, int64_t* state, void* stream);

typedef struct dbx_track {
    double  box[4];
    double  vel[4];
    double  score;
    double  best_score;
    int32_t id;
    int32_t hits;
    int32_t age;
    int32_t first_frame;
    int32_t last_frame;
    int32_t best_frame;
} dbx_track;
typedef struct dbx_track_record {
    int32_t   stream;
    int32_t   reserved;
    dbx_track t;
} dbx_track_record;
int dbx_track_update_batch(const double* dets, int32_t det_cols, int64_t det_rows, const int32_t* keep, const int32_t* prefix,
                           int32_t batch, int32_t slots, int32_t* headers, dbx_track* tracks, int32_t streams, int32_t stream0,
                           int32_t max_tracks, double iou_thresh, int32_t max_age, double alpha, double beta, double birth_score,
                           int32_t* track_id, int32_t* track_slot, int32_t* track_hits, dbx_track* retired, int32_t* tally, void* stream);
int dbx_track_append(const dbx_track* retired, const int32_t* tally, int32_t batch, int32_t max_tracks, int32_t stream0,
                     dbx_track_record* records, int64_t capacity, int64_t* state, void* stream);

typedef struct dbx_shot {
    double  key;
    double  score;
    int64_t sharpness;
    int32_t id;
    int32_t frame;
    int32_t shots;
    int32_t reserved;
} dbx_shot;
typedef struct dbx_shot_record {
    int32_t  stream;
    int32_t  slot;
    dbx_shot shot;
} dbx_shot_record;
int dbx_crop_sharpness(const uint8_t* crops, int64_t n, int32_t oh, int32_t ow, int32_t c, int64_t* out, void* stream);
int dbx_track_gallery_update(const dbx_track* tracks, const int32_t* headers, const int32_t* track_slot, const uint8_t* crops,
                             const int32_t* ok, const dbx_track* retired, const int32_t* tally, const int64_t* append_state,
                             dbx_shot* shots, uint8_t* shot_crops, dbx_shot_record* arena, uint8_t* arena_crops, int64_t* gstate,
                             int32_t batch, int32_t slots, int32_t streams, int32_t stream0, int32_t max_tracks, int32_t oh, int32_t ow,
                             int32_t c, int64_t capacity, int32_t policy, double min_score, int32_t commit, void* stream);

typedef struct dbx_resize_job {
    const uint8_t* src;
    int32_t sh, sw;
    int32_t cx0, cy0, cw, ch;
    int32_t pad_l, pad_t, pad_r, pad_b;
    int32_t pad_value;
    int32_t dh, dw;
    int64_t dst_off;
} dbx_resize_job;
int64_t dbx_resize_batch_workspace_bytes(int32_t njobs);
int dbx_resize_cubic_batch_u8(const dbx_resize_job* jobs, int32_t njobs, int32_t c, uint8_t* dst, void* workspace, void* stream);

int dbx_dp_unique_id(void* id128);
int dbx_dp_init(const void* id128, int32_t rank, int32_t world, void** comm);
int dbx_dp_allreduce_sum_f32(void* comm, float* buf, int64_t n, void* stream);
int dbx_dp_destroy(void* comm);

#ifdef __cplusplus
}
#endif
#endif
```

Measured before the change: 7323 patches/s.

## Exploit sparse loss masks to skip dense head backward for confined heads

After the fused loss, the code builds a compacted list of pixels whose classification mask is nonzero, sized by a host-computed bound from the bounding boxes. Heads whose gradients are confined to those pixels (loc and lmloc) then get their weight gradients and upstream gradient computed by new sparse chain and tree kernels over only the listed rows. Other heads keep the dense one-pass kernel. This cuts wasted FLOPs and memory traffic on mostly-zero gradient maps, at the cost of extra kernels, a host-side bound computation, and a fixed row cap that can overflow.

```diff
diff --git a/densebox_amd/_lib.py b/densebox_amd/_lib.py
--- a/densebox_amd/_lib.py
+++ b/densebox_amd/_lib.py
@@ -150,6 +150,15 @@
     'dbx_heads1_dgrad_gen': (C.c_int, [_I32, _PV, C.POINTER(C.c_void_p), C.POINTER(C.c_int32), _I32, _I32, C.c_uint32, _VP, _PV, _PV, _VP]),
     'dbx_heads1_wgrad_gen': (C.c_int, [_I32, _PV, _PV, C.POINTER(C.c_void_p), C.POINTER(C.c_int32), _I32, _I32, C.c_uint32, _I32, _VP, _I32, _I32,
                              _VP, _VP, _VP]),
+    'dbx_heads_sparse_rows_bytes': (_I64, [_I32, _I32, _I32]),
+    'dbx_heads_sparse_rows': (C.c_int, [_VP, _I32, _I32, _I32, _I32, _I32, _VP, _VP, _VP]),
+    'dbx_heads_sparse_rows_read': (C.c_int, [_VP, _I32, _I32, _I32, C.POINTER(C.c_int32), C.POINTER(C.c_int32), _VP, _VP, _VP]),
+    'dbx_heads_sparse_work_bytes': (_I64, [_I32, _I32, _I32, _I32]),
+    'dbx_heads_sparse_ok': (C.c_int, [_I32, _PV, _PV]),
+    'dbx_heads_sparse_head2': (C.c_int, [_I32, _PV, _PV, C.POINTER(C.c_void_p), C.POINTER(C.c_int32), _I32, C.c_uint32, _I32, C.c_uint32, _I32,
+                                         _VP, _VP, _PV, _VP]),
+    'dbx_head2_backward_up_heads': (C.c_int, [_I32, _PV, _PV, C.POINTER(C.c_void_p), C.POINTER(C.c_int32), _I32, C.c_uint32, _PV, _I32,
+                                              C.c_uint32, C.POINTER(C.c_void_p), C.POINTER(C.c_void_p), _VP, _PV, _VP, _I32, _VP, _VP]),
     'dbx_conv_wgrad_plan': (C.c_int, [_I32, _PV, _PV, _I32, _I32, C.c_char_p, _I32, C.POINTER(C.c_int32)]),
     'dbx_nchw_to_framed': (C.c_int, [_I32, _VP, _I32, _PV, _VP]),
     'dbx_u8hwc_to_framed': (C.c_int, [_I32, _VP, _PV, C.POINTER(C.c_float), C.POINTER(C.c_float), _VP]),
@@ -165,6 +174,7 @@
     'dbx_upsample_bilinear': (C.c_int, [_I32, _PV, _PV, _VP]),
     'dbx_upsample_bilinear_bwd': (C.c_int, [_I32, _PV, _PV, _PV, _VP]),
     'dbx_loss_scratch_bytes': (C.c_int64, [_I32]),
+    'dbx_loss_mask_offset': (C.c_int64, [_I32]),
     'dbx_loss_forward_backward': (C.c_int, [C.POINTER(LossDesc), C.POINTER(LossIO), _VP, _VP]),
     'dbx_count_positives': (C.c_int, [_VP, _VP, _I32, _VP, _VP]),
     'dbx_init_score_map': (C.c_int, [_VP, _VP, _I32, _VP, _VP]),
diff --git a/densebox_amd/csrc/aux_ops.hip b/densebox_amd/csrc/aux_ops.hip
--- a/densebox_amd/csrc/aux_ops.hip
+++ b/densebox_amd/csrc/aux_ops.hip
@@ -1,4 +1,5 @@
 #include "common.hpp"
+#include "heads_sparse.hpp"
 #include <mutex>
 
 static thread_local char g_err[512] = "";
@@ -1354,7 +1355,8 @@
 template <typename T>
 static int head2_backward_up_t(const dbx_view* dout, const dbx_view* hid, const float* const* w2, const int32_t* k, int nh, const dbx_view* dhid,
                                const uint8_t* mask, int mask_ld, int use_hash, unsigned drop_seed, float* const* dw, float* const* db,
-                               void* scratch, const dbx_view* dg, hipStream_t s) {
+                               void* scratch, const dbx_view* dg, hipStream_t s, unsigned head_mask = 0xfu, const void* rows = nullptr,
+                               int cap = 0, void* work = nullptr) {
     VIEW_VEC_CHECK(T, dg, "head2_backward_up d_g44");
     DBX_REQUIRE(dg->n == hid->n && dg->c == hid->c, "head2_backward_up: d_g44 has the hidden map's batch and channels");
     const float sy = ac_scale(dg->h, hid->h), sx = ac_scale(dg->w, hid->w);
@@ -1363,6 +1365,9 @@
     if (const char* e = getenv("DBX_HEAD2_UP")) fused = fused && atoi(e) != 0;
     const bool nostore = dhid->ptr == nullptr;
     DBX_REQUIRE(!nostore || (fused && !mask), "head2_backward_up without d_hid: needs the one-pass kernel (dbx_head2_backward_up_fused) and hash / no dropout");
+    const unsigned all_heads = (1u << nh) - 1u;
+    head_mask &= all_heads;
+    DBX_REQUIRE(head_mask == all_heads || (fused && nostore), "head2_backward_up_heads: a subset of the heads needs the one-pass kernel without a d_hid");
     if (!fused) {
         const int rc = head2_wgrad_t<T>(dout, hid, k, nh, dw, db, scratch, s, w2, dhid, mask, mask_ld, use_hash, drop_seed);
         return rc != DBX_OK ? rc : upsample_bwd_t<T>(dhid, dg, nullptr, s);
@@ -1402,22 +1407,56 @@
         for (int h0 = 0; h0 < nh;) {
             int h1 = h0 + 1;
             while (h1 < nh && kup(k[h1]) == kup(k[h0])) ++h1;
-            const int nhl = h1 - h0, nsl = nhl * 8, kj = kup(k[h0]);
-            int groups = H2U_WGS / (nsl * plan.halves);
+            const int kj = kup(k[h0]);
+            int groups = H2U_WGS / ((h1 - h0) * 8 * plan.halves);
             groups = groups < 1 ? 1 : groups > hid->n ? hid->n : groups;
             const int blocks = groups * plan.halves;
-            float* partial = pbase + pused;
-            float* bpartial = partial + (size_t)blocks * nhl * 8 * 512;
-            for (int i = h0; i < h1; ++i) { o.poff[i] = pused; o.boff[i] = pused + (long long)blocks * nhl * 8 * 512; o.nblk[i] = blocks; o.nhl[i] = nhl; o.hl[i] = i - h0; }
-            pused += (long long)blocks * (nhl * 8 * 512 + 32);
             blocks_max = blocks > blocks_max ? blocks : blocks_max;
+            for (int p0 = h0; p0 < h1;) {
+                const bool in = (head_mask >> p0) & 1u;
+                int p1 = p0 + 1;
+                if (in) while (p1 < h1 && ((head_mask >> p1) & 1u)) ++p1;
+                const int nhl = p1 - p0, nsl = nhl * 8;
+                if (!in && !rows) {
+                    o.poff[p0] = 0; o.boff[p0] = 0; o.nblk[p0] = 0; o.nhl[p0] = 1; o.hl[p0] = 0; o.k[p0] = 0;
+                    p0 = p1;
+                    continue;
+                }
+                float* partial = pbase + pused;
+                float* bpartial = partial + (size_t)blocks * nhl * 8 * 512;
+                for (int i = p0; i < p1; ++i) { o.poff[i] = pused; o.boff[i] = pused + (long long)blocks * nhl * 8 * 512; o.nblk[i] = blocks; o.nhl[i] = nhl; o.hl[i] = i - p0; }
+                pused += (long long)blocks * (nhl * 8 * 512 + 32);
+                DBX_REQUIRE(pused * 4 <= dbx_head2_wgrad_scratch_bytes(nh, hid->n * hid->h), "head2_backward_up: scratch too small for the pieces");
+                if (in) {
 #define H2U_LAUNCH(KJ)                                                                                                              \
-            hipLaunchKernelGGL((head2_backward_up_kernel<T, KJ>), dim3(blocks * nsl), dim3(256), smem, s, make_geo<T>(dout), make_geo<T>(hid),    \
-                               make_geo<T>(nostore ? hid : dhid), make_geo<T>(dg), h0, nhl, dout->c / nh, ha, partial, bpartial, mask, mask_ld,    \
-                               use_hash, drop_seed, sy, sx, plan, nostore ? 1 : 0)
-            if (kj == 1) H2U_LAUNCH(1); else if (kj == 2) H2U_LAUNCH(2); else if (kj == 4) H2U_LAUNCH(4); else H2U_LAUNCH(8);
+                    hipLaunchKernelGGL((head2_backward_up_kernel<T, KJ>), dim3(blocks * nsl), dim3(256), smem, s, make_geo<T>(dout), make_geo<T>(hid),    \
+                                       make_geo<T>(nostore ? hid : dhid), make_geo<T>(dg), p0, nhl, dout->c / nh, ha, partial, bpartial, mask, mask_ld,    \
+                                       use_hash, drop_seed, sy, sx, plan, nostore ? 1 : 0)
+                    if (kj == 1) H2U_LAUNCH(1); else if (kj == 2) H2U_LAUNCH(2); else if (kj == 4) H2U_LAUNCH(4); else H2U_LAUNCH(8);
 #undef H2U_LAUNCH
-            DBX_LAUNCH_CHECK();
+                    DBX_LAUNCH_CHECK();
+                } else {
+                    int ordinal = 0;
+                    for (int i = 0; i < p0; ++i) ordinal += !((head_mask >> i) & 1u);
+                    DBX_REQUIRE(work && ordinal < hsp::SPARSE_MAX && hid->h <= 64 && groups <= hsp::GMAX && hid->h * hid->w <= hsp::NPIX_MAX,
+                                "head2_backward_up_heads: a sparse head needs a work buffer and maps dbx_heads_sparse_ok() takes; at most two of them");
+                    const hsp::Rows R = hsp::rows_of((void*)rows, hid->n, (long long)hid->n * hid->h * hid->w, cap);
+                    const hsp::Chains ch = hsp::chains_of(work, cap, hid->c, hid->w, ordinal);
+                    HspChainArgs ca;
+                    ca.dout = make_geo<T>(dout); ca.hid = make_geo<T>(hid); ca.rowid = R.rowid;
+                    ca.H = hid->h; ca.W = hid->w; ca.n = hid->n; ca.G = groups; ca.hd = p0; ca.slot = dout->c / nh;
+                    ca.acc = ch.acc; ca.bacc = ch.bacc; ca.flag = ch.flag;
+                    hipLaunchKernelGGL(hsp_chain_kernel<T>, dim3(groups * hid->w), dim3(64), 0, s, ca);
+                    DBX_LAUNCH_CHECK();
+                    HspTreeArgs ta;
+                    ta.acc = ch.acc; ta.bacc = ch.bacc; ta.flag = ch.flag; ta.W = hid->w; ta.halves = plan.halves;
+                    for (int q = 0; q < 2; ++q) ta.h[q] = HspTreeHalf{plan.h[q].px_lo, plan.h[q].px_n, plan.h[q].own_lo, plan.h[q].own_hi};
+                    ta.partial = partial; ta.bpartial = bpartial;
+                    hipLaunchKernelGGL(hsp_tree_kernel, dim3(blocks, (4096 + 8 + 255) / 256), dim3(256), 0, s, ta);
+                    DBX_LAUNCH_CHECK();
+                }
+                p0 = p1;
+            }
             h0 = h1;
         }
         for (int i = nh; i < 4; ++i) { o.poff[i] = 0; o.boff[i] = 0; o.nblk[i] = 0; o.nhl[i] = 1; o.hl[i] = 0; }
@@ -1446,6 +1485,14 @@
     if (!d_out || !hid || !w2 || !k || !d_hid || !dw || !scratch || !d_g44) { dbx_set_error("head2_backward_up: null argument"); return DBX_ERR_ARG; }
     DBX_DISPATCH_DTYPE(dtype, head2_backward_up_t, d_out, hid, w2, k, nh, d_hid, dropmask, dropmask_ld, use_hash, (unsigned)drop_seed, dw, db,
                        scratch, d_g44, (hipStream_t)stream);
+}
+extern "C" int dbx_head2_backward_up_heads(int32_t dtype, const dbx_view* d_out, const dbx_view* hid, const float* const* w2, const int32_t* k,
+                                           int32_t nh, uint32_t head_mask, const dbx_view* d_hid, int32_t use_hash, uint32_t drop_seed,
+                                           float* const* dw, float* const* db, void* scratch, const dbx_view* d_g44, const void* rows,
+                                           int32_t cap, void* work, void* stream) {
+    if (!d_out || !hid || !w2 || !k || !d_hid || !dw || !scratch || !d_g44) { dbx_set_error("head2_backward_up_heads: null argument"); return DBX_ERR_ARG; }
+    DBX_DISPATCH_DTYPE(dtype, head2_backward_up_t, d_out, hid, w2, k, nh, d_hid, (const uint8_t*)nullptr, 0, use_hash, (unsigned)drop_seed, dw, db,
+                       scratch, d_g44, (hipStream_t)stream, (unsigned)head_mask, rows, (int)cap, work);
 }
 
 struct PackJob { const float* src; void* dst; int co, ci, taps, mode; long long ktot; int cin_pad, row_off, k_off, rows_lim; };
diff --git a/densebox_amd/csrc/heads_sparse.hip b/densebox_amd/csrc/heads_sparse.hip
--- /dev/null
+++ b/densebox_amd/csrc/heads_sparse.hip
@@ -0,0 +1,333 @@
+#include "heads_sparse.hpp"
+
+__device__ __forceinline__ int hsp_union4(const unsigned char* mb, int npix, int planes, int i0, int (&bit)[4]) {
+    int c = 0;
+#pragma unroll
+    for (int e = 0; e < 4; ++e) {
+        const int i = i0 + e;
+        int u = 0;
+        if (i < npix)
+            for (int p = 0; p < planes; ++p) u |= mb[(size_t)p * npix + i];
+        bit[e] = u != 0;
+        c += bit[e];
+    }
+    return c;
+}
+__global__ __launch_bounds__(1024) void hsp_count_kernel(const unsigned char* maskbuf, int npix, int planes, int stride, int* pcount) {
+    __shared__ int red[16];
+    int bit[4];
+    int c = hsp_union4(maskbuf + (size_t)blockIdx.x * stride, npix, planes, threadIdx.x * 4, bit);
+#pragma unroll
+    for (int off = 32; off > 0; off >>= 1) c += __shfl_down(c, off);
+    if ((threadIdx.x & 63) == 0) red[threadIdx.x >> 6] = c;
+    __syncthreads();
+    if (threadIdx.x == 0) {
+        int t = 0;
+        for (int w = 0; w < 16; ++w) t += red[w];
+        pcount[blockIdx.x] = t;
+    }
+}
+__global__ __launch_bounds__(1024) void hsp_list_kernel(const unsigned char* maskbuf, int npix, int planes, int stride, int n, int cap,
+                                                        const int* pcount, int* hdr, int* rowid, int* list, int* overflow) {
+    __shared__ int red[16], wsum[16], s_base;
+    const int tid = threadIdx.x, lane = tid & 63, wv = tid >> 6, patch = blockIdx.x;
+    {
+        int c = 0;
+        for (int p = tid; p < patch; p += 1024) c += pcount[p];
+#pragma unroll
+        for (int off = 32; off > 0; off >>= 1) c += __shfl_down(c, off);
+        if (lane == 0) red[wv] = c;
+        __syncthreads();
+        if (tid == 0) {
+            int t = 0;
+            for (int w = 0; w < 16; ++w) t += red[w];
+            s_base = t;
+            if (patch == n - 1) {
+                const int total = t + pcount[patch];
+                hdr[0] = total < cap ? total : cap;
+                hdr[2] = total;
+                if (total > cap && overflow) overflow[0] += 1;
+            }
+        }
+        __syncthreads();
+    }
+    int bit[4];
+    const int mine = hsp_union4(maskbuf + (size_t)patch * stride, npix, planes, tid * 4, bit);
+    int incl = mine;
+#pragma unroll
+    for (int off = 1; off < 64; off <<= 1) { const int o = __shfl_up(incl, off); if (lane >= off) incl += o; }
+    if (lane == 63) wsum[wv] = incl;
+    __syncthreads();
+    int pos = s_base + incl - mine;
+    for (int w = 0; w < wv; ++w) pos += wsum[w];
+#pragma unroll
+    for (int e = 0; e < 4; ++e) {
+        const int i = tid * 4 + e;
+        if (i >= npix) break;
+        const int m = patch * npix + i;
+        int rid = -1;
+        if (bit[e]) {
+            if (pos < cap) { rid = pos; list[pos] = m; }
+            ++pos;
+        }
+        rowid[m] = rid;
+    }
+}
+
+extern "C" int64_t dbx_heads_sparse_rows_bytes(int32_t n, int32_t npix, int32_t cap) {
+    if (n < 0 || npix < 0 || cap < 0) return 0;
+    return (int64_t)(hsp::HDR * 4 + hsp::align16((size_t)n * 4) + hsp::align16((size_t)n * npix * 4) + hsp::align16((size_t)cap * 4) + 64);
+}
+extern "C" int dbx_heads_sparse_rows(const void* maskbuf, int32_t n, int32_t npix, int32_t planes, int32_t plane_stride, int32_t cap,
+                                     void* rows, void* overflow, void* stream) {
+    DBX_REQUIRE(maskbuf && rows, "heads_sparse_rows: null argument");
+    DBX_REQUIRE(n >= 1 && npix >= 1 && npix <= hsp::NPIX_MAX && planes >= 1 && plane_stride >= planes && cap >= 0 &&
+                    (long long)n * npix < (1ll << 31),
+                "heads_sparse_rows: n >= 1, 1 <= npix <= 4096, planes >= 1, cap >= 0");
+    const hsp::Rows r = hsp::rows_of(rows, n, (long long)n * npix, cap);
+    const int stride = plane_stride * npix;
+    hipLaunchKernelGGL(hsp_count_kernel, dim3(n), dim3(1024), 0, (hipStream_t)stream, (const unsigned char*)maskbuf, npix, planes, stride, r.pcount);
+    DBX_LAUNCH_CHECK();
+    hipLaunchKernelGGL(hsp_list_kernel, dim3(n), dim3(1024), 0, (hipStream_t)stream, (const unsigned char*)maskbuf, npix, planes, stride, n, cap,
+                       (const int*)r.pcount, r.hdr, r.rowid, r.list, (int*)overflow);
+    DBX_LAUNCH_CHECK();
+    return DBX_OK;
+}
+extern "C" int dbx_heads_sparse_rows_read(const void* rows, int32_t n, int32_t npix, int32_t cap, int32_t* count, int32_t* total,
+                                          int32_t* list_out, int32_t* rowid_out, void* stream) {
+    DBX_REQUIRE(rows && count && total, "heads_sparse_rows_read: null argument");
+    const hsp::Rows r = hsp::rows_of((void*)rows, n, (long long)n * npix, cap);
+    int hdr[hsp::HDR];
+    DBX_HIP(hipMemcpyAsync(hdr, r.hdr, sizeof(hdr), hipMemcpyDeviceToHost, (hipStream_t)stream));
+    if (list_out && cap > 0) DBX_HIP(hipMemcpyAsync(list_out, r.list, (size_t)cap * 4, hipMemcpyDeviceToHost, (hipStream_t)stream));
+    if (rowid_out) DBX_HIP(hipMemcpyAsync(rowid_out, r.rowid, (size_t)n * npix * 4, hipMemcpyDeviceToHost, (hipStream_t)stream));
+    DBX_HIP(hipStreamSynchronize((hipStream_t)stream));
+    *count = hdr[0]; *total = hdr[2];
+    return DBX_OK;
+}
+
+struct HspHeads { int n; int hd[4]; };
+__device__ __forceinline__ int hsp_head(const HspHeads& hs, int i) {
+    int h = hs.hd[0];
+#pragma unroll
+    for (int q = 1; q < 4; ++q)
+        if (i == q) h = hs.hd[q];
+    return h;
+}
+struct HspGenArgs {
+    FrameGeo dout;
+    const float* w2[4]; int k[4];
+    int slot, use_hash; unsigned seed;
+    int hw, w;
+    int hc, cap;
+    HspHeads heads;
+};
+template <typename T>
+__global__ __launch_bounds__(256) void hsp_gen_kernel(const HspGenArgs a, const int* __restrict__ hdr, const int* __restrict__ list,
+                                                     T* __restrict__ dhid) {
+    int count = hdr[0]; count = count < a.cap ? count : a.cap;
+    const int r0 = blockIdx.x * 32, hd = hsp_head(a.heads, blockIdx.y);
+    if (r0 >= count) return;
+    const int rg = threadIdx.x >> 6, ct = threadIdx.x & 63, c0 = ct * 8;
+    const float* wp = a.w2[0]; int k = a.k[0];
+#pragma unroll
+    for (int hh = 1; hh < 4; ++hh)
+        if (hd == hh) { wp = a.w2[hh]; k = a.k[hh]; }
+    const float sc = a.use_hash ? 2.f : 1.f;
+    float w[8][8];
+#pragma unroll
+    for (int j = 0; j < 8; ++j)
+#pragma unroll
+        for (int i = 0; i < 8; ++i) w[j][i] = j < k ? to_f32(from_f32<T>(wp[(size_t)(j < k ? j : 0) * 512 + c0 + i])) * sc : 0.f;
+    for (int rr = 0; rr < 8; ++rr) {
+        const int r = r0 + rg * 8 + rr;
+        if (r >= count) break;
+        const int m = list[r];
+        const int img = m / a.hw, rem = m - img * a.hw, y = rem / a.w, x = rem - y * a.w;
+        const u32x4 graw = *(const u32x4*)((const T*)a.dout.base + geo_pix(a.dout, img, y, x) + hd * a.slot);
+        const T* ge = (const T*)&graw;
+        float o[8];
+#pragma unroll
+        for (int i = 0; i < 8; ++i) o[i] = 0.f;
+#pragma unroll
+        for (int j = 0; j < 8; ++j) {
+            const float g = to_f32(ge[j]);
+#pragma unroll
+            for (int i = 0; i < 8; ++i) o[i] = fmaf(g, w[j][i], o[i]);
+        }
+        if (a.use_hash) {
+            const unsigned kb8 = dbx_drop_hash32(a.seed, (unsigned)m, (unsigned)(hd * 512 + c0) >> 5) >> ((unsigned)c0 & 31u);
+#pragma unroll
+            for (int i = 0; i < 8; ++i) o[i] = (kb8 >> i) & 1u ? o[i] : 0.f;
+        }
+        u32x4 raw;
+        T* oe = (T*)&raw;
+#pragma unroll
+        for (int i = 0; i < 8; ++i) oe[i] = from_f32<T>(o[i]);
+        *(u32x4*)(dhid + (size_t)r * a.hc + hd * 512 + c0) = raw;
+    }
+}
+
+__device__ __forceinline__ void hsp_bilin(int d, float scale, int in, int& i0, int& i1, float& l0, float& l1) {
+#pragma clang fp contract(off)
+    const float src = scale * (float)d;
+    i0 = (int)src;
+    if (i0 > in - 1) i0 = in - 1;
+    i1 = i0 + (i0 < in - 1 ? 1 : 0);
+    l1 = src - (float)i0;
+    l0 = 1.f - l1;
+}
+template <typename T>
+__global__ __launch_bounds__(256) void hsp_dg44_kernel(FrameGeo dg, int H, int W, float sy, float sx, int hc, const int* __restrict__ rowid,
+                                                      const T* __restrict__ dhid, HspHeads heads) {
+    __shared__ int s_rid[32][64];
+    __shared__ float s_wy[8], s_wx[32][8];
+    __shared__ int s_cnt[32];
+    __shared__ unsigned char s_tq[32][32];
+    const int iy = blockIdx.x % dg.h, img = blockIdx.x / dg.h;
+    int oylo = (int)((float)(iy - 1) / sy) - 1;
+    oylo = oylo < 0 ? 0 : oylo;
+    auto oxlo_of = [&](int ix) { const int v = (int)((float)(ix - 1) / sx) - 1; return v < 0 ? 0 : v; };
+    for (int e = threadIdx.x; e < 8 + dg.w * 8; e += 256) {
+        const bool isx = e >= 8;
+        const int ix = isx ? (e - 8) >> 3 : 0, t = e & 7;
+        const int o = (isx ? oxlo_of(ix) : oylo) + t, lim = isx ? W : H, in = isx ? dg.w : dg.h, i = isx ? ix : iy;
+        float wgt = 0.f;
+        if (o < lim) {
+            int i0, i1; float l0, l1;
+            hsp_bilin(o, isx ? sx : sy, in, i0, i1, l0, l1);
+            if (isx) wgt = i0 == i ? (i1 == i0 ? l0 + l1 : l0) : (i0 == i - 1 && i1 != i0 ? l1 : 0.f);
+            else wgt = (i0 == i ? l0 : 0.f) + (i1 == i ? l1 : 0.f);
+        }
+        if (isx) s_wx[ix][t] = wgt; else s_wy[t] = wgt;
+    }
+    __syncthreads();
+    for (int e = threadIdx.x; e < dg.w * 64; e += 256) {
+        const int ix = e >> 6, q = e & 63, ax = q >> 3, ay = q & 7;
+        const int oy = oylo + ay, ox = oxlo_of(ix) + ax;
+        int rid = -1;
+        if (oy < H && ox < W && s_wy[ay] != 0.f && s_wx[ix][ax] != 0.f) rid = rowid[(img * H + oy) * W + ox];
+        s_rid[ix][q] = rid;
+    }
+    __syncthreads();
+    if (threadIdx.x < dg.w) {
+        int cnt = 0;
+        for (int q = 0; q < 64; ++q)
+            if (s_rid[threadIdx.x][q] >= 0 && cnt < 32) s_tq[threadIdx.x][cnt++] = (unsigned char)q;
+        s_cnt[threadIdx.x] = cnt;
+    }
+    __syncthreads();
+    const int per = heads.n * 64;
+    T* const row = (T*)dg.base + geo_pix(dg, img, iy, 0);
+    for (int item = threadIdx.x; item < dg.w * per; item += 256) {
+        const int ix = item / per, ci = item - ix * per;
+        const int c0 = hsp_head(heads, ci >> 6) * 512 + (ci & 63) * 8;
+        float c[8], v[8];
+#pragma unroll
+        for (int i = 0; i < 8; ++i) c[i] = v[i] = 0.f;
+        const int cnt = s_cnt[ix];
+        int cur = -1;
+        for (int t = 0; t < cnt; t += 4) {
+            u32x4 raw[4];
+            int qq[4];
+#pragma unroll
+            for (int u = 0; u < 4; ++u) {
+                qq[u] = s_tq[ix][t + u < cnt ? t + u : t];
+                raw[u] = *(const u32x4*)(dhid + (size_t)s_rid[ix][qq[u]] * hc + c0);
+            }
+#pragma unroll
+            for (int u = 0; u < 4; ++u) {
+                if (t + u < cnt) {
+                    const int ax = qq[u] >> 3, ay = qq[u] & 7;
+                    if (ax != cur) {
+                        if (cur >= 0) {
+                            const float wx = s_wx[ix][cur];
+#pragma unroll
+                            for (int i = 0; i < 8; ++i) { c[i] = fmaf(wx, v[i], c[i]); v[i] = 0.f; }
+                        }
+                        cur = ax;
+                    }
+                    const T* e = (const T*)&raw[u];
+                    const float wy = s_wy[ay];
+#pragma unroll
+                    for (int i = 0; i < 8; ++i) v[i] = fmaf(wy, to_f32(e[i]), v[i]);
+                }
+            }
+        }
+        if (cur >= 0) {
+            const float wx = s_wx[ix][cur];
+#pragma unroll
+            for (int i = 0; i < 8; ++i) c[i] = fmaf(wx, v[i], c[i]);
+        }
+        u32x4 o;
+        T* oe = (T*)&o;
+#pragma unroll
+        for (int i = 0; i < 8; ++i) oe[i] = from_f32<T>(c[i]);
+        *(u32x4*)(row + (size_t)ix * dg.ld + c0) = o;
+    }
+}
+
+extern "C" int64_t dbx_heads_sparse_work_bytes(int32_t dtype, int32_t cap, int32_t nh, int32_t w) {
+    if (cap < 0 || nh < 1 || nh > 4 || w < 1 || dtype == DBX_F32) return 0;
+    return (int64_t)(hsp::dhid_bytes(cap, 512 * nh) + (size_t)(nh < hsp::SPARSE_MAX ? nh : hsp::SPARSE_MAX) * hsp::chain_bytes(w) + 64);
+}
+extern "C" int dbx_heads_sparse_ok(int32_t dtype, const dbx_view* hid, const dbx_view* d_g44) {
+    if (!hid || !d_g44 || dtype == DBX_F32) return 0;
+    if (hid->c % 512 || hid->c / 512 < 1 || hid->c / 512 > 4 || d_g44->c != hid->c || d_g44->n != hid->n) return 0;
+    if (hid->h < 2 || hid->w < 2 || d_g44->h < 2 || d_g44->w < 2 || d_g44->w > 32 || hid->h > 64 || hid->h * hid->w > hsp::NPIX_MAX) return 0;
+    if (hid->w <= 32 || hid->w > 64) return 0;
+    const float sy = (float)(d_g44->h - 1) / (float)(hid->h - 1), sx = (float)(d_g44->w - 1) / (float)(hid->w - 1);
+    return sy > 0.45f && sy < 1.f && sx > 0.45f && sx < 1.f;
+}
+
+template <typename T>
+static int heads_sparse_head2_t(const dbx_view* dout, const dbx_view* hid, const float* const* w2, const int32_t* k, int nh, unsigned head_mask,
+                                int use_hash, unsigned seed, int cap, const void* rows, void* work, const dbx_view* d_g44, hipStream_t s) {
+    if constexpr (sizeof(T) != 2) {
+        dbx_set_error("heads_sparse_head2: 16-bit compute types only");
+        return DBX_ERR_DTYPE;
+    } else {
+        DBX_REQUIRE(dbx_heads_sparse_ok(DType<T>::id, hid, d_g44) == 1, "heads_sparse_head2: maps not supported (dbx_heads_sparse_ok)");
+        DBX_REQUIRE(nh == hid->c / 512 && dout->c % nh == 0 && dout->c / nh >= 8 && ((dout->c / nh) * sizeof(T)) % 16 == 0 &&
+                        (dout->ld * sizeof(T)) % 16 == 0 && ((size_t)dout->ptr % 16) == 0 && (dout->c_off * sizeof(T)) % 16 == 0,
+                    "heads_sparse_head2: d_out of nh 16-byte aligned slots >= 8 channels");
+        DBX_REQUIRE(dout->n == hid->n && dout->h == hid->h && dout->w == hid->w, "heads_sparse_head2: shape mismatch");
+        const dbx_view* vs[2] = {hid, d_g44};
+        for (const dbx_view* v : vs)
+            DBX_REQUIRE(((size_t)v->ptr % 16) == 0 && (v->ld * sizeof(T)) % 16 == 0 && (v->c_off * sizeof(T)) % 16 == 0, "heads_sparse_head2: 16-byte aligned views");
+        DBX_REQUIRE(cap >= 0 && ((size_t)work % 16) == 0 && ((size_t)rows % 16) == 0, "heads_sparse_head2: capacity / alignment");
+        HspHeads hs; hs.n = 0;
+        for (int i = 0; i < 4; ++i) hs.hd[i] = 0;
+        for (int i = 0; i < nh; ++i)
+            if ((head_mask >> i) & 1u) {
+                DBX_REQUIRE(k[i] >= 1 && k[i] <= 8 && w2[i], "heads_sparse_head2: k in 1..8, weights per head");
+                hs.hd[hs.n++] = i;
+            }
+        if (hs.n == 0) return DBX_OK;
+        const int hc = hid->c, hw = hid->h * hid->w;
+        const hsp::Rows R = hsp::rows_of((void*)rows, hid->n, (long long)hid->n * hw, cap);
+        T* const dhid_s = (T*)work;
+        const int tiles = (cap + 31) / 32;
+        if (tiles > 0) {
+            HspGenArgs g;
+            g.dout = make_geo<T>(dout);
+            for (int i = 0; i < 4; ++i) { g.w2[i] = i < nh ? w2[i] : w2[0]; g.k[i] = i < nh ? k[i] : 0; }
+            g.slot = dout->c / nh; g.use_hash = use_hash; g.seed = seed; g.hw = hw; g.w = hid->w; g.hc = hc; g.cap = cap; g.heads = hs;
+            hipLaunchKernelGGL(hsp_gen_kernel<T>, dim3(tiles, hs.n), dim3(256), 0, s, g, (const int*)R.hdr, (const int*)R.list, dhid_s);
+            DBX_LAUNCH_CHECK();
+        }
+        const float sy = (float)(d_g44->h - 1) / (float)(hid->h - 1), sx = (float)(d_g44->w - 1) / (float)(hid->w - 1);
+        hipLaunchKernelGGL(hsp_dg44_kernel<T>, dim3(d_g44->n * d_g44->h), dim3(256), 0, s, make_geo<T>(d_g44), hid->h, hid->w, sy, sx, hc,
+                           (const int*)R.rowid, (const T*)dhid_s, hs);
+        DBX_LAUNCH_CHECK();
+        return DBX_OK;
+    }
+}
+extern "C" int dbx_heads_sparse_head2(int32_t dtype, const dbx_view* d_out, const dbx_view* hid, const float* const* w2, const int32_t* k,
+                                      int32_t nh, uint32_t head_mask, int32_t use_hash, uint32_t drop_seed, int32_t cap, const void* rows,
+                                      void* work, const dbx_view* d_g44, void* stream) {
+    if (!d_out || !hid || !w2 || !k || !rows || !work || !d_g44) { dbx_set_error("heads_sparse_head2: null argument"); return DBX_ERR_ARG; }
+    if (nh < 1 || nh > 4) { dbx_set_error("heads_sparse_head2: nh in 1..4"); return DBX_ERR_ARG; }
+    DBX_DISPATCH_DTYPE(dtype, heads_sparse_head2_t, d_out, hid, w2, k, nh, (unsigned)head_mask, use_hash, (unsigned)drop_seed, cap, rows, work,
+                       d_g44, (hipStream_t)stream);
+}
diff --git a/densebox_amd/csrc/heads_sparse.hpp b/densebox_amd/csrc/heads_sparse.hpp
--- /dev/null
+++ b/densebox_amd/csrc/heads_sparse.hpp
@@ -0,0 +1,118 @@
+#pragma once
+#include "common.hpp"
+
+namespace hsp {
+constexpr int NPIX_MAX = 4096, HDR = 16, GMAX = 32, SPARSE_MAX = 2;
+struct Rows { int* hdr; int* pcount; int* rowid; int* list; };
+static inline size_t align16(size_t v) { return (v + 15) & ~(size_t)15; }
+static inline Rows rows_of(void* scratch, int n, long long nrows, int cap) {
+    Rows r; char* p = (char*)scratch;
+    r.hdr = (int*)p; p += HDR * 4;
+    r.pcount = (int*)p; p += align16((size_t)n * 4);
+    r.rowid = (int*)p; p += align16((size_t)nrows * 4);
+    r.list = (int*)p;
+    return r;
+}
+struct Chains { float* acc; float* bacc; int* flag; };
+static inline size_t dhid_bytes(int cap, int hc) { return align16((size_t)((cap + 31) / 32 * 32) * hc * 2); }
+static inline size_t chain_bytes(int w) { return align16((size_t)GMAX * w * (4096 + 8 + 1) * 4); }
+static inline Chains chains_of(void* work, int cap, int hc, int w, int ordinal) {
+    char* p = (char*)work + dhid_bytes(cap, hc) + (size_t)ordinal * chain_bytes(w);
+    Chains c;
+    c.acc = (float*)p; c.bacc = c.acc + (size_t)GMAX * w * 4096; c.flag = (int*)(c.bacc + (size_t)GMAX * w * 8);
+    return c;
+}
+}
+
+struct HspChainArgs {
+    FrameGeo dout, hid;
+    const int* rowid;
+    int H, W, n, G, hd, slot;
+    float* acc; float* bacc; int* flag;
+};
+template <typename T>
+__global__ __launch_bounds__(64) void hsp_chain_kernel(const HspChainArgs a) {
+    const int chain = blockIdx.x, lane = threadIdx.x;
+    const int grp = chain / a.W, px = chain - grp * a.W;
+    float acc[8][8], bs[8];
+#pragma unroll
+    for (int j = 0; j < 8; ++j) {
+        bs[j] = 0.f;
+#pragma unroll
+        for (int i = 0; i < 8; ++i) acc[j][i] = 0.f;
+    }
+    bool any = false;
+    for (int img0 = grp; img0 < a.n; img0 += 4 * a.G) {
+        int rid[4];
+#pragma unroll
+        for (int q = 0; q < 4; ++q) {
+            const int img = img0 + q * a.G;
+            rid[q] = -1;
+            if (lane < a.H && img < a.n) rid[q] = a.rowid[(img * a.H + lane) * a.W + px];
+        }
+#pragma unroll
+        for (int q = 0; q < 4; ++q) {
+            const int img = img0 + q * a.G;
+            unsigned long long mask = __ballot(rid[q] >= 0);
+            while (mask) {
+                const int y = __ffsll((long long)mask) - 1;
+                mask &= mask - 1;
+                any = true;
+                const u32x4 graw = *(const u32x4*)((const T*)a.dout.base + geo_pix(a.dout, img, y, px) + a.hd * a.slot);
+                const u32x4 hraw = *(const u32x4*)((const T*)a.hid.base + geo_pix(a.hid, img, y, px) + a.hd * 512 + lane * 8);
+                const T* ge = (const T*)&graw;
+                const T* he = (const T*)&hraw;
+#pragma unroll
+                for (int j = 0; j < 8; ++j) {
+                    const float g = to_f32(ge[j]);
+                    bs[j] += g;
+#pragma unroll
+                    for (int i = 0; i < 8; ++i) acc[j][i] = fmaf(g, to_f32(he[i]), acc[j][i]);
+                }
+            }
+        }
+    }
+    if (lane == 0) a.flag[chain] = any ? 1 : 0;
+    if (!any) return;
+#pragma unroll
+    for (int j = 0; j < 8; ++j) {
+        float* dst = a.acc + ((size_t)chain * 8 + j) * 512 + lane * 8;
+        *(f32x4*)dst = (f32x4){acc[j][0], acc[j][1], acc[j][2], acc[j][3]};
+        *(f32x4*)(dst + 4) = (f32x4){acc[j][4], acc[j][5], acc[j][6], acc[j][7]};
+    }
+    if (lane < 8) {
+        float b = bs[0];
+#pragma unroll
+        for (int j = 1; j < 8; ++j) b = lane == j ? bs[j] : b;
+        a.bacc[(size_t)chain * 8 + lane] = b;
+    }
+}
+struct HspTreeHalf { int px_lo, px_n, own_lo, own_hi; };
+struct HspTreeArgs {
+    const float* acc; const float* bacc; const int* flag;
+    int W, halves; HspTreeHalf h[2];
+    float* partial; float* bpartial;
+};
+static __global__ __launch_bounds__(256) void hsp_tree_kernel(const HspTreeArgs a) {
+    const int blk = blockIdx.x, e = blockIdx.y * 256 + threadIdx.x;
+    if (e >= 4096 + 8) return;
+    const bool bias = e >= 4096;
+    const int grp = blk / a.halves, half = blk - grp * a.halves;
+    const HspTreeHalf hf = half ? a.h[1] : a.h[0];
+    float o = 0.f;
+#pragma unroll
+    for (int w = 0; w < 4; ++w) {
+        float v[8];
+#pragma unroll
+        for (int p = 0; p < 8; ++p) {
+            const int pl = 8 * w + p, px = hf.px_lo + pl;
+            const bool own = pl < hf.px_n && px >= hf.own_lo && px < hf.own_hi;
+            const int chain = grp * a.W + (own ? px : 0);
+            v[p] = 0.f;
+            if (own && a.flag[chain]) v[p] = bias ? a.bacc[(size_t)chain * 8 + (e - 4096)] : a.acc[(size_t)chain * 4096 + e];
+        }
+        o += ((v[0] + v[1]) + (v[2] + v[3])) + ((v[4] + v[5]) + (v[6] + v[7]));
+    }
+    if (bias) a.bpartial[(size_t)blk * 32 + (e - 4096)] = o;
+    else a.partial[(size_t)blk * 4096 + e] = o;
+}
diff --git a/densebox_amd/csrc/loss.hip b/densebox_amd/csrc/loss.hip
--- a/densebox_amd/csrc/loss.hip
+++ b/densebox_amd/csrc/loss.hip
@@ -336,6 +336,7 @@
 extern "C" int64_t dbx_loss_scratch_bytes(int32_t n) {
     return (int64_t)n * LOSS_APPLY_BLOCKS * 8 + (int64_t)n * 5 * NPIX + 64;
 }
+extern "C" int64_t dbx_loss_mask_offset(int32_t n) { return (int64_t)n * LOSS_APPLY_BLOCKS * (int64_t)sizeof(double); }
 extern "C" int dbx_loss_forward_backward(const dbx_loss_desc* d, const dbx_loss_io* io, void* scratch, void* stream) {
     DBX_REQUIRE(d && io && scratch, "loss: null argument");
     DBX_REQUIRE(d->kind >= 0 && d->kind <= 2 && d->n > 0, "loss: bad kind/n");
diff --git a/densebox_amd/dist.py b/densebox_amd/dist.py
--- a/densebox_amd/dist.py
+++ b/densebox_amd/dist.py
@@ -253,6 +253,9 @@
             if net.KIND != 'DenseBox' and lm_rand_neg_indices is None:
                 lm_rand_neg_indices = np.stack([np.stack([rs.choice(3600, 1, replace=False) for _ in range(n)])
                                                 for _ in range(4)])
+            if 'rows_cap' not in loss_kw and not (torch.is_tensor(bbox) and bbox.is_cuda) and \
+                    not (torch.is_tensor(labels) and labels.is_cuda):
+                loss_kw['rows_cap'] = LB.cls_mask_bound(bbox, labels if net.KIND == 'DenseBoxLMLOC' else None, half)
             bbox, vertices, labels, rand_neg_indices, lm_rand_neg_indices = self._stage(
                 x.device, [(bbox, torch.float32), (vertices, torch.float32), (labels, torch.float32),
                            (rand_neg_indices, torch.int64), (lm_rand_neg_indices, torch.int64)])
diff --git a/densebox_amd/engine.py b/densebox_amd/engine.py
--- a/densebox_amd/engine.py
+++ b/densebox_amd/engine.py
@@ -56,12 +56,12 @@
     @staticmethod
     def env_flags():
         return tuple(os.environ.get(k, '1') != '0' for k in ('DBX_LIN_BWD', 'DBX_REFINE_LINEAR', 'DBX_POOL_IDX', 'DBX_HEADS_GEN')) + \
-            (os.environ.get('DBX_F32_LIN', '0') == '1',)
+            (os.environ.get('DBX_F32_LIN', '0') == '1', os.environ.get('DBX_HEADS_SPARSE', '1') != '0')
 
     def __init__(self, kind, n, h, w, dtype_id, device, train):
         self.kind, self.n, self.h, self.w, self.dtype_id, self.train = kind, n, h, w, dtype_id, train
         self.flags = Plan.env_flags()
-        lin_bwd, lin_refine, use_idx, heads_gen, f32_lin = self.flags
+        lin_bwd, lin_refine, use_idx, heads_gen, f32_lin, heads_sparse = self.flags
         lin_bwd = lin_bwd and (dtype_id != _lib.F32 or f32_lin)
         es = _lib.ESIZE[dtype_id]
         self.cin0 = 16 // es
@@ -113,6 +113,9 @@
                                       L.dbx_heads1_wgrad_gen_ok(dtype_id, C.byref(B['fusion'].view(512, 256)), nh))
             if not self.heads_gen or dtype_id == _lib.F32:
                 add('d_hid', h4, w4, 512 * nh, pad=1)
+            self.heads_sparse = bool(heads_sparse and self.heads_gen and dtype_id != _lib.F32 and h4 * w4 == 3600 and
+                                     L.dbx_heads_sparse_ok(dtype_id, C.byref(B['hid'].view()), C.byref(B['d_g44'].view())))
+            self.heads_path = None
             if rf_convs:
                 add('d_rfo', h4, w4, self.crf, pad=0)
                 add('d_rf_u', h4, w4, 64, pad=0)
@@ -128,6 +131,7 @@
         self.total = off
         if not train:
             self.heads_gen = False
+            self.heads_sparse = False
         self.drop_active = self.drop_hash = False
         self.frag = {}
         self.drop_seed = 0
@@ -892,6 +896,28 @@
     def _lin_bwd(self, dt):
         return (dt != _lib.F32 or os.environ.get('DBX_F32_LIN', '0') == '1') and os.environ.get('DBX_LIN_BWD', '1') != '0'
 
+    def _heads_sparse_mask(self, P, grad_outs, override, heads):
+        if not getattr(P, 'heads_sparse', False):
+            return 0, None
+        from . import loss as _loss
+        hint = _loss.rows_hint(P.ws.device)
+        if hint is None or hint['n'] != P.n:
+            return 0, None
+        frac = float(os.environ.get('DBX_HEADS_SPARSE_FRAC', 1.0 / 16))
+        if hint['bound'] > frac * P.n * P.h4 * P.w4:
+            return 0, None
+        mask = 0
+        confined = os.environ.get('DBX_HEADS_SPARSE_HEADS', 'lmloc').split(',')
+        for i, (stem, _) in enumerate(heads):
+            g = grad_outs.get(stem)
+            if stem in ('loc', 'lmloc') and stem in confined and override.get(stem) is None and (g is None or g.data_ptr() in hint['ok']):
+                mask |= 1 << i
+        return mask, hint
+
+    def heads_sparse_overflows(self):
+        from . import loss as _loss
+        return _loss.heads_sparse_overflows()
+
     def _d_hid(self, P):
         b = P.B.get('d_hid')
         if b is None:
@@ -1065,13 +1091,15 @@
         mask_p = C.c_void_p(P.mask_buf.data_ptr()) if (P.drop_active and not P.drop_hash) else None
         hash_on, hash_seed = (1 if P.drop_hash else 0), (P.drop_seed if P.drop_hash else 0)
         lin = self._lin_bwd(dt)
-        up_done = False
+        up_done = h2_profiled = False
         gen = bool(getattr(P, 'heads_gen', False) and lin and side is None and mask_p is None)
         if gen and dt != _lib.F32:
             dhid_v = View(None, hv.n, hv.h, hv.w, 1, 512 * nh, 0, 512 * nh)
         else:
             dhid_v = self._d_hid(P).view()
         w2p = (C.c_void_p * nh)(*[w.data_ptr() for w in w2s])
+        sparse_mask, hint = self._heads_sparse_mask(P, grad_outs, override, heads) if (gen and dt != _lib.F32) else (0, None)
+        P.heads_path = 'dense' if not sparse_mask else 'sparse:' + ','.join(st for i, (st, _) in enumerate(heads) if (sparse_mask >> i) & 1)
         if side is not None:
             def run_h2():
                 check(L.dbx_head2_wgrad(dt, C.byref(B['d_out'].view()), C.byref(hv), ks, nh,
@@ -1082,6 +1110,30 @@
             on_side(run_h2)
             check(L.dbx_head2_dgrad(dt, C.byref(B['d_out'].view()), (C.c_void_p * nh)(*[w.data_ptr() for w in w2s]), ks, nh,
                                     C.byref(dhid_v), mask_p, 512 * nh, hash_on, hash_seed, s))
+        elif lin and sparse_mask:
+            dw2p, db2p = (C.c_void_p * nh)(*[t.data_ptr() for t in dw2]), (C.c_void_p * nh)(*[t.data_ptr() for t in db2])
+            need = L.dbx_heads_sparse_work_bytes(dt, hint['cap'], nh, hv.w)
+            if getattr(self, '_hs_work', None) is None or self._hs_work.numel() < need:
+                self._hs_work = torch.empty(int(need), dtype=torch.uint8, device=dev)
+            check(L.dbx_head2_backward_up_heads(dt, C.byref(B['d_out'].view()), C.byref(hv), w2p, ks, nh, ((1 << nh) - 1) & ~sparse_mask,
+                                                C.byref(dhid_v), hash_on, hash_seed, dw2p, db2p, ptr(self._h2_scratch),
+                                                C.byref(B['d_g44'].view()), ptr(hint['rows']), hint['cap'], ptr(self._hs_work), s))
+            if prof is not None:
+                ev1.record()
+                kd = sum(k for i, (_, k) in enumerate(heads) if not (sparse_mask >> i) & 1)
+                prof.append({'kernel': 'head2_backward_up_kernel<%s>' % ('f16', 'bf16', 'f32')[dt],
+                             'flops': 2.0 * hv.n * hv.h * hv.w * 512 * kd * 2, 'start': ev0, 'end': ev1})
+                ev0, ev1 = torch.cuda.Event(enable_timing=True), torch.cuda.Event(enable_timing=True)
+                ev0.record()
+            check(L.dbx_heads_sparse_head2(dt, C.byref(B['d_out'].view()), C.byref(hv), w2p, ks, nh, sparse_mask, hash_on, hash_seed,
+                                           hint['cap'], ptr(hint['rows']), ptr(self._hs_work), C.byref(B['d_g44'].view()), s))
+            if prof is not None:
+                ev1.record()
+                ksp = sum(k for i, (_, k) in enumerate(heads) if (sparse_mask >> i) & 1)
+                prof.append({'kernel': 'heads_sparse_head2<%s>' % ('f16', 'bf16', 'f32')[dt],
+                             'flops': 2.0 * hint['bound'] * 512 * ksp * 2, 'start': ev0, 'end': ev1})
+                h2_profiled = True
+            up_done = True
         elif lin:
             check(L.dbx_head2_backward_up(dt, C.byref(B['d_out'].view()), C.byref(hv), (C.c_void_p * nh)(*[w.data_ptr() for w in w2s]), ks, nh,
                                           C.byref(dhid_v), mask_p, 512 * nh, hash_on, hash_seed,
@@ -1098,7 +1150,7 @@
                                        ptr(self._h2_scratch), s))
             if sink is not None:
                 sink.ready(h2_names)
-        if prof is not None:
+        if prof is not None and not h2_profiled:
             ev1.record()
             prof.append({'kernel': ('head2_backward_up_kernel<%s>' if up_done else 'head2_wgrad_kernel<%s>') % ('f16', 'bf16', 'f32')[dt],
                          'flops': 2.0 * hv.n * hv.h * hv.w * 512 * sum(k for _, k in heads) * (1 if side is not None else 2), 'start': ev0, 'end': ev1})
diff --git a/densebox_amd/labels.py b/densebox_amd/labels.py
--- a/densebox_amd/labels.py
+++ b/densebox_amd/labels.py
@@ -137,6 +137,32 @@
     return out
 
 
+def cls_mask_bound(bbox, labels, half):
+    b = np.asarray(torch.as_tensor(bbox).detach().cpu(), np.float32).reshape(-1, 4)
+    n = b.shape[0]
+    valid = np.ones(n, bool) if labels is None else \
+        np.asarray(torch.as_tensor(labels).detach().cpu(), np.float32).reshape(n) != 0.0
+
+    def norm(v):
+        return np.where(v < 0, np.maximum(v + HW, 0), np.minimum(v, HW))
+
+    area = {0: np.ones(n, np.int64), 2: np.ones(n, np.int64)}
+    for c0, c2 in ((b[:, 0], b[:, 2]), (b[:, 1], b[:, 3])):
+        centre = (c0 + c2).astype(np.float32).astype(np.float64) * 0.5
+        rw = (np.float32(0.3) * (c2 - c0).astype(np.float32)).astype(np.float32)
+        hf = (rw * np.float32(0.5)).astype(np.float32).astype(np.float64)
+        org = np.trunc(centre - hf + 0.5)
+        end = np.trunc(org + rw.astype(np.float64) + 0.5)
+        lo, hi = norm(org.astype(np.int64)), norm(end.astype(np.int64) + 1)
+        area[0] = area[0] * np.maximum(hi - lo, 0)
+        org = np.trunc(centre - hf - 2.0 + 0.5)
+        end = np.trunc(org + rw.astype(np.float64) + 4.0 + 0.5)
+        lo, hi = norm(org.astype(np.int64) + 2), norm(end.astype(np.int64) - 2 + 1)
+        area[2] = area[2] * np.maximum(hi - lo, 0)
+    per = np.where(valid, area[0] + area[2], 0) + 2 * int(half)
+    return int(np.minimum(per, HW * HW).sum())
+
+
 def neg_counts(positive_num, batch):
     neg_num = int(float(positive_num) / float(batch) + 0.5)
     return neg_num, int(neg_num * 0.5 + 0.5)
diff --git a/densebox_amd/loss.py b/densebox_amd/loss.py
--- a/densebox_amd/loss.py
+++ b/densebox_amd/loss.py
@@ -1,4 +1,5 @@
 import ctypes as C
+import os
 
 import numpy as np
 import torch
@@ -7,6 +8,21 @@
 from ._lib import LossDesc, LossIO, check, ptr, stream_ptr
 
 _KIND_ID = {'DenseBox': 0, 'DenseBoxLM': 1, 'DenseBoxLMLOC': 2}
+
+
+_ROWS = {}
+_OVERFLOW = {}
+
+
+def rows_hint(device):
+    return _ROWS.get(torch.device(device).index or 0)
+
+
+def heads_sparse_overflows(device=None):
+    if device is not None:
+        t = _OVERFLOW.get(torch.device(device).index or 0)
+        return int(t.item()) if t is not None else 0
+    return sum(int(t.item()) for t in _OVERFLOW.values())
 
 
 class _LossFn(torch.autograd.Function):
@@ -18,12 +34,19 @@
 
     @staticmethod
     def backward(ctx, g):
-        return (None, None) + tuple(d * g for d in ctx.grads) + (None,) * len(ctx.grads)
+        scaled = tuple(d * g for d in ctx.grads)
+        hint = getattr(ctx, 'rows', None)
+        if hint is not None:
+            for d, sd in zip(ctx.grads, scaled):
+                if d.data_ptr() in hint['ok']:
+                    hint['ok'].add(sd.data_ptr())
+                    hint['keep'].append(sd)
+        return (None, None) + scaled + (None,) * len(ctx.grads)
 
 
 def densebox_loss(kind, outputs, bbox, vertices=None, labels=None, rand_neg_indices=None, lm_rand_neg_indices=None,
                   lambda_loc=3.0, lambda_det=1.0, lambda_lm=0.5, batch_global=None, positive_num_global=None,
-                  return_debug=False, rng=None):
+                  return_debug=False, rng=None, rows_cap=None):
     kid = _KIND_ID[kind]
     if kind == 'DenseBox':
         score, loc = outputs
@@ -40,6 +63,9 @@
     P = int(LB.positive_count(bbox, labels if use_labels else None).sum()) if positive_num_global is None \
         else int(positive_num_global)
     _, half = LB.neg_counts(P, n if batch_global is None else batch_global)
+    if rows_cap is None and not (torch.is_tensor(bbox) and bbox.is_cuda) and \
+            not (use_labels and torch.is_tensor(labels) and labels.is_cuda):
+        rows_cap = LB.cls_mask_bound(bbox, labels if use_labels else None, half)
     rs = rng if rng is not None else np.random
     if rand_neg_indices is None:
         rand_neg_indices = np.stack([rs.choice(3600, half, replace=False) for _ in range(n)]) if half else \
@@ -77,11 +103,28 @@
                     ('pos_count', dbg.get('pos_count'))):
         setattr(io, name, t.data_ptr() if t is not None else None)
     check(_lib.lib().dbx_loss_forward_backward(C.byref(d), C.byref(io), ptr(scratch), stream_ptr()))
+    hint = None
+    if rows_cap is not None and os.environ.get('DBX_HEADS_SPARSE', '1') != '0':
+        L = _lib.lib()
+        cap = int(rows_cap)
+        rows = torch.empty(int(L.dbx_heads_sparse_rows_bytes(n, 3600, cap)), dtype=torch.uint8, device=dev)
+        di = dev.index or 0
+        if di not in _OVERFLOW:
+            _OVERFLOW[di] = torch.zeros(1, dtype=torch.int32, device=dev)
+        mask_off = int(L.dbx_loss_mask_offset(n))
+        check(L.dbx_heads_sparse_rows(C.c_void_p(scratch.data_ptr() + mask_off), n, 3600, 1, 5, cap, ptr(rows), ptr(_OVERFLOW[di]),
+                                      stream_ptr()))
+        confined = [gg for gg in (g[1], g[4]) if gg is not None]
+        hint = {'n': n, 'cap': cap, 'bound': int(rows_cap), 'rows': rows, 'ok': {gg.data_ptr() for gg in confined}, 'keep': confined + [scratch]}
+    _ROWS[dev.index or 0] = hint
     live = [(t, gg) for t, gg in zip((score, loc, lm, rf, lmloc), g) if t is not None]
     out = _LossFn.apply(loss[0], len(live), *[t for t, _ in live], *[gg for _, gg in live])
+    if out.grad_fn is not None:
+        out.grad_fn.rows = hint
     out._dbx_direct = ([t for t, _ in live], [gg for _, gg in live])
     if return_debug:
         dbg['half'] = half
+        dbg['rows'] = hint
         dbg['grads'] = {k: gg for k, gg in zip(('score', 'loc', 'lm', 'rf', 'lmloc'), g) if gg is not None}
         return out, dbg
     return out
diff --git a/include/densebox_hip.h b/include/densebox_hip.h
--- a/include/densebox_hip.h
+++ b/include/densebox_hip.h
@@ -114,6 +114,20 @@
                          float* db, void* scratch, void* stream);
 int dbx_heads1_dgrad_gen(int32_t dtype, const dbx_view* d_out, const float* const* w2, const int32_t* k, int32_t nh, int32_t use_hash,
                          uint32_t drop_seed, const void* w1t_frag, const dbx_view* y, const dbx_view* gate, void* stream);
+int64_t dbx_heads_sparse_rows_bytes(int32_t n, int32_t npix, int32_t cap);
+int dbx_heads_sparse_rows(const void* maskbuf, int32_t n, int32_t npix, int32_t planes, int32_t plane_stride, int32_t cap, void* rows,
+                          void* overflow, void* stream);
+int dbx_heads_sparse_rows_read(const void* rows, int32_t n, int32_t npix, int32_t cap, int32_t* count, int32_t* total, int32_t* list_out,
+                               int32_t* rowid_out, void* stream);
+int64_t dbx_heads_sparse_work_bytes(int32_t dtype, int32_t cap, int32_t nh, int32_t w);
+int dbx_heads_sparse_ok(int32_t dtype, const dbx_view* hid, const dbx_view* d_g44);
+int dbx_heads_sparse_head2(int32_t dtype, const dbx_view* d_out, const dbx_view* hid, const float* const* w2, const int32_t* k, int32_t nh,
+                           uint32_t head_mask, int32_t use_hash, uint32_t drop_seed, int32_t cap, const void* rows, void* work,
+                           const dbx_view* d_g44, void* stream);
+int dbx_head2_backward_up_heads(int32_t dtype, const dbx_view* d_out, const dbx_view* hid, const float* const* w2, const int32_t* k,
+                                int32_t nh, uint32_t head_mask, const dbx_view* d_hid, int32_t use_hash, uint32_t drop_seed,
+                                float* const* dw, float* const* db, void* scratch, const dbx_view* d_g44, const void* rows, int32_t cap,
+                                void* work, void* stream);
 
 int dbx_fold_heads(const float* w2, const float* b2, const float* w1, const float* b1, int32_t k, float* w_out,
                    float* b_out, void* stream);
@@ -189,6 +203,7 @@
 } dbx_loss_io;
 
 int64_t dbx_loss_scratch_bytes(int32_t n);
+int64_t dbx_loss_mask_offset(int32_t n);
 int dbx_loss_forward_backward(const dbx_loss_desc* d, const dbx_loss_io* io, void* scratch, void* stream);
 int dbx_count_positives(const float* bbox, const float* labels, int32_t n, int32_t* count_per_sample, void* stream);
 
```

Measured after the change: 7378 patches/s (median of 6 runs). Within noise of the previous version (+0.8%).
